# zsc/MOSS-TTSD

Measured on AMD Instinct MI355X. Metric: audio codec tokens/sec/node (decode, bf16, batch 32 @ 4k ctx), higher is better.
Workload: dtype bf16; 1 GPU; configs[2]: batch 32 synthetic dialogues/GPU, 4k-token KV context, top-k/top-p sampling on 8 channels, decode steps at full context; batch_per_gpu=32, context=4096, prompt=512, layers=28, hidden=2048, parallelism=dp1 (batch shard, no per-step collective)

## Files before the change

include/mtts.h:

```cpp
#ifndef MTTS_H
#define MTTS_H

#include <stdint.h>

#ifdef __cplusplus
extern "C" {
#endif

#define MTTS_OK 0
#define MTTS_EINVAL (-1)
#define MTTS_EHIP (-2)
#define MTTS_ENOMEM (-3)
#define MTTS_ESTATE (-4)

#define MTTS_CHANNELS 8

typedef struct MttsConfig {
    int32_t vocab_size;
    int32_t hidden_size;
    int32_t intermediate_size;
    int32_t num_hidden_layers;
    int32_t num_attention_heads;
    int32_t num_key_value_heads;
    int32_t head_dim;
// ... 13 lines not shown
#define MTTS_DTYPE_BF16 0
#define MTTS_DTYPE_F32 1
#define MTTS_DTYPE_F16 2

typedef struct MttsSamplerCfg {
    int32_t do_sample;
    int32_t top_k;
    float top_p;
    float one_minus_top_p;
    float temperature;
    float repetition_penalty;
} MttsSamplerCfg;

typedef struct MttsEngine MttsEngine;

const char* mtts_last_error(void);
int32_t mtts_version(void);

int32_t mtts_engine_create(const MttsConfig* cfg, int32_t device, MttsEngine** out);
int32_t mtts_engine_destroy(MttsEngine* e);

int32_t mtts_bind_weight(MttsEngine* e, const char* name, const void* dev_bf16,
                         int64_t rows, int64_t cols, void* stream);
int32_t mtts_bind_weight_lora(MttsEngine* e, const char* name, const void* dev_base, int64_t rows, int64_t cols,
                              const float* dev_lora_a, const float* dev_lora_b, int32_t r, float scaling, void* stream);
#define MTTS_MAX_ADAPTERS 16
#define MTTS_LORA_MAX_RANK 64
int32_t mtts_adapter_load(MttsEngine* e, int32_t adapter, const char* name, const float* dev_lora_a, const float* dev_lora_b,
                          int64_t rows, int64_t cols, int32_t r, float scaling, void* stream);
int32_t mtts_adapter_clear(MttsEngine* e, int32_t adapter);
int32_t mtts_set_row_adapters(MttsEngine* e, const int32_t* host_ids, int32_t n);
int32_t mtts_set_slot_adapter(MttsEngine* e, int32_t slot, int32_t adapter);
int32_t mtts_bind_rope(MttsEngine* e, const void* dev_cos_bf16, const void* dev_sin_bf16,
                       int32_t rows, void* stream);
int32_t mtts_weights_ready(MttsEngine* e);

int32_t mtts_generate(MttsEngine* e, const int64_t* host_input_ids, const uint8_t* host_attention_mask,
                      int32_t B, int32_t T, int32_t max_length,
                      const MttsSamplerCfg* sampler, uint64_t seed,
                      int64_t* host_out_ids, int32_t out_capacity, int32_t* out_len,
                      const int64_t* host_forced, int32_t forced_len, int64_t* host_decisions,
                      void* stream);

int32_t mtts_begin(MttsEngine* e, const int64_t* host_input_ids, const uint8_t* host_attention_mask,
                   int32_t B, int32_t T, int32_t max_length,
                   const MttsSamplerCfg* sampler, uint64_t seed, void* stream);
int32_t mtts_step(MttsEngine* e, int32_t n_steps, void* stream);
int32_t mtts_sync_state(MttsEngine* e, int32_t* steps_done, int32_t* all_finished, void* stream);
int32_t mtts_read_generated(MttsEngine* e, int64_t* host_gen, int32_t capacity_steps, int32_t* n_steps);
int32_t mtts_set_output_scores(MttsEngine* e, int32_t on);
int32_t mtts_read_scores(MttsEngine* e, float* host_lp, int32_t capacity_steps, int32_t* n_steps);
int32_t mtts_slot_read_scores(MttsEngine* e, int32_t slot, float* host_rows, int32_t capacity_steps, int32_t* n_steps);
int32_t mtts_score(MttsEngine* e, const int64_t* host_input_ids, const uint8_t* host_attention_mask,
                   const int64_t* host_labels, int32_t B, int32_t T, float* host_logp, void* stream);
#define MTTS_SCORE_MAX_TOPK 16
#define MTTS_SCORE_TOPK_ROWS 512
int32_t mtts_score_topk(MttsEngine* e, const int64_t* host_input_ids, const uint8_t* host_attention_mask,
                        const int64_t* host_labels, int32_t B, int32_t T, float* host_logp, int32_t k,
                        int32_t* host_top_ids, float* host_top_logp, void* stream);
int32_t mtts_read_logits(MttsEngine* e, uint16_t* host_logits0, uint16_t* host_logits17, void* stream);
int32_t mtts_read_logits_f32(MttsEngine* e, float* host_logits0, float* host_logits17, void* stream);
int32_t mtts_sched_open(MttsEngine* e, int32_t B, int32_t gen_cap, const MttsSamplerCfg* sampler, void* stream);
int32_t mtts_slot_submit(MttsEngine* e, int32_t slot, const int64_t* host_ids, int32_t T, int32_t max_length, uint64_t seed,
                         void* stream);
int32_t mtts_slot_submit_row(MttsEngine* e, int32_t slot, const int64_t* host_ids, int32_t T, int32_t max_length, uint64_t seed,
                             int32_t row_id, void* stream);
int32_t mtts_set_row_ids(MttsEngine* e, const int32_t* host_row_ids, int32_t n);
int32_t mtts_set_takes(MttsEngine* e, int32_t n);
int32_t mtts_slot_fork(MttsEngine* e, int32_t src_slot, int32_t dst_slot, uint64_t seed, int32_t row_id, void* stream);
int32_t mtts_slot_states(MttsEngine* e, int32_t* host_state, void* stream);
int32_t mtts_slot_read(MttsEngine* e, int32_t slot, int64_t* host_rows, int32_t capacity_steps, int32_t* n_steps);
int32_t mtts_read_seq_state(MttsEngine* e, int32_t* host_nas, int32_t* host_unfinished, int32_t* host_kv_len, void* stream);
int32_t mtts_slot_evict(MttsEngine* e, int32_t slot, void* stream);
int32_t mtts_kv_pool_state(MttsEngine* e, int32_t* total_pages, int32_t* free_pages, int32_t* max_pages_per_seq);
int32_t mtts_read_page_table(MttsEngine* e, int32_t* host_table, int32_t* host_n_pages);
int32_t mtts_set_forced_mode(MttsEngine* e, int32_t as_draw);
int32_t mtts_debug_read_device_page_table(MttsEngine* e, int32_t* host_table, void* stream);
int32_t mtts_export_codes(MttsEngine* e, int32_t first, int32_t n, int64_t* dev_codes, void* stream);
int32_t mtts_profile_enable(MttsEngine* e, int32_t on);
int32_t mtts_profile_read(MttsEngine* e, int32_t which, double* total_ms, int64_t* launches, int64_t* bytes);

int32_t mtts_debug_set_kv_len(MttsEngine* e, int32_t kv_len);
int32_t mtts_debug_kv_pack_stats(MttsEngine* e, int64_t* out6);
int32_t mtts_k_attn_bench(MttsEngine* e, int32_t phase, int32_t iters, float* avg_ms, int64_t* bytes_per_launch);
int32_t mtts_k_gemm_bench(int32_t N, int32_t K, int32_t epi, int32_t ksplit, int32_t waves, int32_t copies,
                          int32_t iters, float* avg_us);

int32_t mtts_k_gemm_bf16(const void* dev_w, const void* dev_x, void* dev_y,
                         int32_t M, int32_t N, int32_t K, int32_t ksplit, void* stream);
int64_t mtts_debug_gemm_depth_launches(void);
int64_t mtts_debug_attn_row_launches(void);
int32_t mtts_k_attn_section(const float* dev_slabs, int32_t ksplit, const void* dev_qnw, const void* dev_knw, const void* dev_cos,
                            const void* dev_sin, float eps, const void* dev_k, const void* dev_v, const int32_t* host_lens,
                            const int32_t* host_page_table, int32_t R, int32_t Lmax, int32_t nq, int32_t nkv, int32_t sealed,
                            int32_t path, void* dev_out, void* dev_kcache, void* dev_vcache, void* dev_kpack, void* dev_vpack,
                            void* stream);
int32_t mtts_k_attn_prefill(const float* dev_slabs, int32_t ksplit, const void* dev_qnw, const void* dev_knw, const void* dev_cos,
                            const void* dev_sin, float eps, const void* dev_k, const void* dev_v, const int32_t* host_lens,
                            const int32_t* host_cached, const int32_t* host_page_table, int32_t B, int32_t Lmax, int32_t nq,
                            int32_t nkv, void* dev_out, void* dev_q, void* dev_kcache, void* dev_vcache, void* stream);
int32_t mtts_k_gemm_swiglu_bf16(const void* dev_w, const void* dev_x, void* dev_y,
                                int32_t M, int32_t N, int32_t K, void* stream);
int32_t mtts_k_rmsnorm(const void* dev_x, const void* dev_w, void* dev_y,
                       int32_t rows, int32_t n, float eps, void* stream);
int32_t mtts_k_embed_norm(const int32_t* host_tokens, const int32_t* host_seq, const void* const* host_tables,
                          const int32_t* host_vocab, const void* dev_norm_w, int32_t R, int32_t H, float eps,
                          void* dev_x, void* dev_xn, void* stream);
int32_t mtts_k_resid_norm(const float* dev_slabs, int32_t ksplit, int32_t Npad, void* dev_x, const void* dev_norm_w,
                          const int32_t* host_seq, const int32_t* host_last, int32_t R, int32_t H, int32_t nseq, float eps,
                          void* dev_xn, void* dev_hlast, void* stream);
int32_t mtts_k_gemv_small(int32_t epi, int32_t pro, const void* dev_w, int32_t rows, int32_t N, int32_t K, int32_t want_ksplit,
                          const void* dev_x_in, const float* dev_slabs, int32_t slab_ksplit, const void* dev_norm_w, float eps,
                          void* dev_x_out, const float* dev_opart, const int32_t* host_seq, const int32_t* host_pos, int32_t nq,
                          int32_t nchunks_max, const void* dev_xrows, void* dev_y, int32_t* out_plan, void* stream);
int32_t mtts_k_gemm_tile(int32_t epi, const void* dev_w, const void* dev_x, void* dev_y, int32_t M, int32_t N, int32_t K,
                         int32_t ksplit, void* stream);
int32_t mtts_k_rope_kvwrite(const void* dev_qkv, const int32_t* host_pos, const void* dev_qnorm, const void* dev_knorm,
                            const void* dev_cos, const void* dev_sin, int32_t R, int32_t nq, int32_t nkv, float eps,
                            void* dev_q, void* dev_k, void* dev_v, void* stream);
int32_t mtts_k_paged_attn_decode(const void* dev_q, const void* dev_k, const void* dev_v, const int32_t* host_lens,
                                 const int32_t* host_page_table, int32_t R, int32_t Lmax, int32_t nq, int32_t nkv,
                                 void* dev_out, void* stream);
int32_t mtts_k_kv_seal(const void* dev_pages, int32_t npages, void* dev_sealed, int32_t as_k, void* stream);
int32_t mtts_k_head_ce(const void* dev_w, const void* dev_x, const int32_t* host_labels, int32_t M, int32_t N, int32_t K,
                       int32_t n_valid, int32_t segments, float* dev_logp, void* stream);
int32_t mtts_k_head_topk(const void* dev_w, const void* dev_x, int32_t M, int32_t N, int32_t K, int32_t n_valid,
                         int32_t segments, int32_t k, int32_t* dev_ids, float* dev_logp, void* stream);
int32_t mtts_k_lora_pack(const void* dev_base, int32_t rows, int32_t cols, const float* dev_lora_a, const float* dev_lora_b,
                         int32_t r, float scaling, int32_t rows_pad, int32_t row_mul, int32_t row_off, int32_t dtype,
                         void* dev_out, void* stream);
int32_t mtts_k_lora_delta(const void* dev_x, int32_t R, int32_t K, int32_t Npad, int32_t nseg, const int32_t* host_segs,
                          int32_t n_adapters, const void* const* host_a, const void* const* host_b, const int32_t* host_r,
                          const float* host_scaling, const int32_t* host_row_adapter, float* dev_slabs, int32_t ks, void* stream);
int32_t mtts_k_swiglu_slabs(const void* dev_w, const void* dev_x, const float* dev_delta, void* dev_y, float* dev_slab0_out,
                            int32_t M, int32_t N, int32_t K, void* stream);
int32_t mtts_k_sample(const void* dev_logits_bf16, int32_t rows, int32_t vocab,
                      const void* dev_history_bitmap, const MttsSamplerCfg* cfg,
                      int32_t mask_id, uint64_t seed, int32_t step, int32_t channel,
                      int32_t* dev_tokens, void* stream);
int32_t mtts_k_sample_scores(const void* dev_logits_bf16, int32_t rows, int32_t vocab,
                             const void* dev_history_bitmap, const MttsSamplerCfg* cfg,
                             int32_t mask_id, uint64_t seed, int32_t step, int32_t channel,
                             int32_t* dev_tokens, float* dev_logp, void* stream);

typedef struct MttsCodecConfig {
    int32_t nq, codebook_size, rvq_dim, quant_out_dim;
    int32_t adapter_layers, adapter_dim, adapter_heads, adapter_ffn, adapter_max_pos;
    int32_t up_stride;
    int32_t dec_layers, dec_dim, dec_heads, dec_ffn, dec_max_pos, mel_bins;
    int32_t voc_dim, voc_inter, voc_layers, n_fft, hop;
    int32_t mel_n_fft, mel_hop, mel_frames;
    int32_t enc_layers, enc_dim, enc_heads, enc_ffn, enc_max_pos;
    int32_t sem_adapter_layers, pre_rvq_layers, down_pool;
} MttsCodecConfig;

typedef struct MttsCodec MttsCodec;
const char* mtts_codec_last_error(void);
int32_t mtts_codec_create(const MttsCodecConfig* cfg, int32_t device, MttsCodec** out);
int32_t mtts_codec_destroy(MttsCodec* c);
int32_t mtts_codec_bind(MttsCodec* c, const char* role, const float* dev_f32, int64_t n, void* stream);
int32_t mtts_codec_detokenize(MttsCodec* c, const int64_t* dev_codes, const int32_t* host_lens, int32_t B, int32_t T,
                              float* dev_wav, void* stream);
int32_t mtts_codec_detokenize_async(MttsCodec* c, const int64_t* dev_codes, const int32_t* host_lens, int32_t B, int32_t T,
                                    float* dev_wav, void* stream);
int32_t mtts_codec_check(MttsCodec* c, void* stream);
int32_t mtts_codec_tokenize(MttsCodec* c, const float* dev_wav, const int32_t* host_lens, int32_t B, int32_t nsamp,
// ... 11 lines not shown
```

moss-ttsd_amd/csrc/attn.hip:

```cpp
#include "launch.h"
#include <algorithm>
#include <atomic>
#include <cstdlib>
#ifndef MTTS_PK_WAVES
#define MTTS_PK_WAVES 0
#endif
#if MTTS_PK_WAVES
#define PK_OCC(PK) __attribute__((amdgpu_waves_per_eu((PK) ? MTTS_PK_WAVES : 1, (PK) ? MTTS_PK_WAVES : 8)))
#else
#define PK_OCC(PK)
#endif

__device__ __forceinline__ uint32_t u4c(const u32x4_t& v, int c) { return c == 0 ? v.x : c == 1 ? v.y : c == 2 ? v.z : v.w; }
__device__ __forceinline__ void pk_unit(const u32x4_t* pk, int j, uint32_t w[4]) {
    const uint32_t L0 = u4c(pk[j >> 1], 2 * (j & 1)), L1 = u4c(pk[j >> 1], 2 * (j & 1) + 1);
    const uint32_t N = u4c(pk[8 + (j >> 2)], j & 3);
    const uint32_t lo = pk[12].x, hi = pk[12].y;
    const uint32_t HA = ((N & 0x08080808u) << 4) | __builtin_amdgcn_perm(hi, lo, N & 0x07070707u);
    const uint32_t HB = (N & 0x80808080u) | __builtin_amdgcn_perm(hi, lo, (N >> 4) & 0x07070707u);
    w[0] = __builtin_amdgcn_perm(HA, L0, 0x05010400u);
    w[1] = __builtin_amdgcn_perm(HA, L0, 0x07030602u);
    w[2] = __builtin_amdgcn_perm(HB, L1, 0x05010400u);
    w[3] = __builtin_amdgcn_perm(HB, L1, 0x07030602u);
}
// ... 109 lines not shown
                }
                out |= b << (16 * h);
            }
            w[c] = out;
        }
        v[j] = u32x4_t{w[0], w[1], w[2], w[3]};
    }
    return seal_encode(v, pk, ((uint32_t)s0 & 0xffu) | (((uint32_t)s1 & 0xffu) << 8), unfit);
}
__device__ bool seal_lane_v(const u32x4_t* __restrict__ raw, u32x4_t* __restrict__ pk, uint8_t* __restrict__ lds, int lane) {
    u32x4_t v[16];
#pragma unroll
    for (int j = 0; j < 16; ++j) v[j] = raw[j * 64];
    const int sub = lane >> 5;
    __builtin_amdgcn_wave_barrier();
    uint32_t* row = (uint32_t*)(lds + lane * 128);
#pragma unroll
    for (int it = 0; it < 16; ++it)
#pragma unroll
        for (int h = 0; h < 2; ++h) {
            uint32_t sum = 0u, cnt = 0u;
#pragma unroll
            for (int c = 0; c < 4; ++c) {
                const uint32_t e = (u4c(v[it], c) >> (7 + 16 * h)) & 0xffu;
                sum += e;
                cnt += e ? 1u : 0u;
            }
            row[2 * it + h] = sum | (cnt << 16);
        }
    __builtin_amdgcn_wave_barrier();
    int mean;
    {
        const int t = lane, st = (t >> 1) & 1, j = 2 * (t >> 2) + (t & 1);
        uint32_t tot = 0u, cn = 0u;
        for (int d = 0; d < 32; ++d) {
            const uint32_t w = ((const uint32_t*)(lds + (st * 32 + d) * 128))[j];
            tot += w & 0xffffu;
            cn += w >> 16;
        }
        mean = cn ? (int)((tot + cn / 2) / cn) : 0;
    }
    int* means = (int*)(lds + 8192);
    int8_t* sv = (int8_t*)(lds + 8192 + 256);
    means[lane] = mean;
    __builtin_amdgcn_wave_barrier();
    int ref = 255;
    for (int t = 0; t < 64; ++t) { const int m = means[t]; if (m > 0) ref = min(ref, m); }
    const int s_own = mean > 0 ? min((mean - ref) & ~1, 126) : 0;
    sv[lane] = (int8_t)s_own;
    __builtin_amdgcn_wave_barrier();
    bool unfit = false;
#pragma unroll
    for (int it = 0; it < 16; ++it) {
        const int s0 = sv[4 * it + 2 * sub], s1 = sv[4 * it + 2 * sub + 1];
        uint32_t w[4] = {v[it].x, v[it].y, v[it].z, v[it].w};
#pragma unroll
        for (int c = 0; c < 4; ++c) {
            uint32_t out = 0u;
#pragma unroll
            for (int h = 0; h < 2; ++h) {
                uint32_t b = (w[c] >> (16 * h)) & 0xffffu;
                const int sft = h ? s1 : s0;
                const int e = (int)((b >> 7) & 0xffu);
                if (e == 0) {
                    if ((b & 0x7fu) && sft) unfit = true;
                } else {
                    const int e2 = e - sft;
                    if (e == 255 ? sft != 0 : e2 < 1) unfit = true;
                    else b = (b - ((uint32_t)sft << 7)) & 0xffffu;
                }
                out |= b << (16 * h);
            }
            w[c] = out;
        }
        v[it] = u32x4_t{w[0], w[1], w[2], w[3]};
    }
    return seal_encode(v, pk, (uint32_t)s_own & 0xffu, unfit);
}
__device__ __forceinline__ void seal_count(bool fit, unsigned long long* __restrict__ cnt, int layer, int wave, int lane) {
    const bool all = !__any(!fit);
    if (cnt && lane == 0) atomicAdd(cnt + layer * 4 + wave * 2 + (all ? 0 : 1), 1ull);
}

__global__ __launch_bounds__(128) void kv_seal_scan_kernel(const u32x4_t* __restrict__ kcache, const u32x4_t* __restrict__ vcache,
                                                           u32x4_t* __restrict__ kpack, u32x4_t* __restrict__ vpack,
                                                           const int32_t* __restrict__ page_table, const RowMeta* __restrict__ meta, int R,
                                                           int max_pages, int total_pages, size_t raw_layer, size_t pk_layer,
                                                           unsigned long long* __restrict__ cnt) {
    __shared__ __attribute__((aligned(16))) uint8_t klds[8192 + 128];
    __shared__ __attribute__((aligned(16))) uint8_t vlds[8192 + 320];
    const int kvh = blockIdx.y, layer = blockIdx.z, wave = threadIdx.x >> 6, lane = threadIdx.x & 63;
    const int r = blockIdx.x * 64 + lane;
    RowMeta m{-1, 0, 0, 0};
    if (r < R) m = meta[r];
    unsigned long long todo = __ballot(m.seq >= 0 && (m.pos & 63) == 63);
    while (todo) {
        const int i = __ffsll((long long)todo) - 1;
        todo &= todo - 1;
        const int seq = __shfl(m.seq, i, 64), pos = __shfl(m.pos, i, 64);
        const int page = page_table[(size_t)seq * max_pages + (pos >> 6)];
        const size_t pi = (size_t)kvh * total_pages + page;
        const bool fit = wave ? seal_lane_v(vcache + layer * raw_layer + pi * (MTTS_PAGE * MTTS_HD / 8) + lane,
                                            vpack + layer * pk_layer + pi * (MTTS_PKU * 64) + lane, vlds, lane)
                              : seal_lane_k(kcache + layer * raw_layer + pi * (MTTS_PAGE * MTTS_HD / 8) + lane,
                                            kpack + layer * pk_layer + pi * (MTTS_PKU * 64) + lane, klds, lane);
        seal_count(fit, cnt, layer, wave, lane);
    }
}
__global__ __launch_bounds__(128) void kv_seal_all_kernel(const u32x4_t* __restrict__ kcache, const u32x4_t* __restrict__ vcache,
                                                          u32x4_t* __restrict__ kpack, u32x4_t* __restrict__ vpack, int total_pages,
                                                          size_t raw_layer, size_t pk_layer, unsigned long long* __restrict__ cnt) {
    __shared__ __attribute__((aligned(16))) uint8_t klds[8192 + 128];
    __shared__ __attribute__((aligned(16))) uint8_t vlds[8192 + 320];
    const int kvh = blockIdx.y, layer = blockIdx.z, wave = threadIdx.x >> 6, lane = threadIdx.x & 63;
    const size_t pi = (size_t)kvh * total_pages + blockIdx.x;
    const bool fit = wave ? seal_lane_v(vcache + layer * raw_layer + pi * (MTTS_PAGE * MTTS_HD / 8) + lane,
                                        vpack + layer * pk_layer + pi * (MTTS_PKU * 64) + lane, vlds, lane)
                          : seal_lane_k(kcache + layer * raw_layer + pi * (MTTS_PAGE * MTTS_HD / 8) + lane,
                                        kpack + layer * pk_layer + pi * (MTTS_PKU * 64) + lane, klds, lane);
    seal_count(fit, cnt, layer, wave, lane);
}
__global__ __launch_bounds__(64) void kv_seal_pages_kernel(const u32x4_t* __restrict__ raw, u32x4_t* __restrict__ pk, int as_k) {
    __shared__ __attribute__((aligned(16))) uint8_t klds[8192 + 320];
    const u32x4_t* src = raw + (size_t)blockIdx.x * (MTTS_PAGE * MTTS_HD / 8) + threadIdx.x;
    u32x4_t* dst = pk + (size_t)blockIdx.x * (MTTS_PKU * 64) + threadIdx.x;
    if (as_k == 1) seal_lane_k(src, dst, klds, threadIdx.x);
    else if (as_k == 2) seal_lane_v(src, dst, klds, threadIdx.x);
    else seal_lane(src, dst);
}
void launch_kv_seal_pages(const void* raw, void* pk, int npages, int as_k, hipStream_t st) {
    hipLaunchKernelGGL(kv_seal_pages_kernel, dim3(npages), dim3(64), 0, st, (const u32x4_t*)raw, (u32x4_t*)pk, as_k);
}
__global__ __launch_bounds__(64) void kv_pack_count_kernel(const u32x4_t* __restrict__ kpack, const u32x4_t* __restrict__ vpack,
                                                           const int32_t* __restrict__ page_table, const int32_t* __restrict__ complete,
                                                           int max_pages, int total_pages, size_t pk_layer, unsigned long long* __restrict__ out) {
    const int b = blockIdx.x, kvh = blockIdx.y, layer = blockIdx.z, lane = threadIdx.x;
    unsigned long long n = 0, dk = 0, dv = 0;
    for (int pg = 0; pg < complete[b]; ++pg) {
        const size_t pi = (size_t)kvh * total_pages + page_table[(size_t)b * max_pages + pg];
        const u32x4_t fk = kpack[layer * pk_layer + pi * (MTTS_PKU * 64) + 12 * 64 + lane];
        const u32x4_t fv = vpack[layer * pk_layer + pi * (MTTS_PKU * 64) + 12 * 64 + lane];
        n += 1;
        dk += __any(fk.w != 0u) ? 1 : 0;
        dv += __any(fv.w != 0u) ? 1 : 0;
    }
    if (lane == 0 && n) {
        atomicAdd(out + 0, n); atomicAdd(out + 1, dk); atomicAdd(out + 2, n); atomicAdd(out + 3, dv);
    }
}
void launch_kv_pack_count(const void* kpack, const void* vpack, const int32_t* page_table, const int32_t* complete, int B, int max_pages,
                          int total_pages, int nkv, int L, unsigned long long* out, hipStream_t st) {
    const size_t pk_layer = (size_t)total_pages * nkv * (MTTS_PKU * 64);
    hipLaunchKernelGGL(kv_pack_count_kernel, dim3(B, nkv, L), dim3(64), 0, st, (const u32x4_t*)kpack, (const u32x4_t*)vpack, page_table,
                       complete, max_pages, total_pages, pk_layer, out);
}
void launch_kv_seal_rows(const void* kcache, const void* vcache, void* kpack, void* vpack, const int32_t* page_table,
                         const RowMeta* meta, int R, int max_pages, int total_pages, int nkv, int L, unsigned long long* cnt, hipStream_t st) {
    const size_t raw_layer = (size_t)total_pages * nkv * (MTTS_PAGE * MTTS_HD / 8), pk_layer = (size_t)total_pages * nkv * (MTTS_PKU * 64);
    hipLaunchKernelGGL(kv_seal_scan_kernel, dim3((R + 63) / 64, nkv, L), dim3(128), 0, st, (const u32x4_t*)kcache, (const u32x4_t*)vcache,
                       (u32x4_t*)kpack, (u32x4_t*)vpack, page_table, meta, R, max_pages, total_pages, raw_layer, pk_layer, cnt);
}
void launch_kv_seal_all(const void* kcache, const void* vcache, void* kpack, void* vpack, int total_pages, int nkv, int L,
                        unsigned long long* cnt, hipStream_t st) {
    const size_t raw_layer = (size_t)total_pages * nkv * (MTTS_PAGE * MTTS_HD / 8), pk_layer = (size_t)total_pages * nkv * (MTTS_PKU * 64);
    hipLaunchKernelGGL(kv_seal_all_kernel, dim3(total_pages, nkv, L), dim3(128), 0, st, (const u32x4_t*)kcache, (const u32x4_t*)vcache,
                       (u32x4_t*)kpack, (u32x4_t*)vpack, total_pages, raw_layer, pk_layer, cnt);
}


__device__ __forceinline__ void fuse_reduce(const QkvFuse& f, int r, int col, int lane, float& a, float& b) {
    const size_t kstride = (size_t)MTTS_PFCAP * f.Npad;
    const float* p0 = f.partial + (size_t)r * f.Npad + col + lane;
    a = 0.f; b = 0.f;
    for (int k0 = 0; k0 < f.ksplit; k0 += 8) {
        float ta[8], tb[8];
#pragma unroll
        for (int j = 0; j < 8; ++j) {
            const float* pk = p0 + (size_t)min(k0 + j, f.ksplit - 1) * kstride;
            ta[j] = pk[0];
            tb[j] = pk[64];
        }
        if (k0 == 0) { a = ta[0]; b = tb[0]; }
#pragma unroll
        for (int j = 0; j < 8; ++j)
            if (k0 + j < f.ksplit && k0 + j > 0) { a += ta[j]; b += tb[j]; }
    }
    a = rbf(a);
    b = rbf(b);
}

__device__ __forceinline__ void fuse_reduce_request(const QkvFuse& f, int r, int col, int lane, float (&ta)[8], float (&tb)[8]) {
    const size_t kstride = (size_t)MTTS_PFCAP * f.Npad;
    const float* p0 = f.partial + (size_t)r * f.Npad + col + lane;
#pragma unroll
    for (int j = 0; j < 8; ++j) {
        const float* pk = p0 + (size_t)min(j, f.ksplit - 1) * kstride;
        ta[j] = pk[0];
        tb[j] = pk[64];
    }
}
__device__ __forceinline__ void fuse_reduce_sum(const QkvFuse& f, const float (&ta)[8], const float (&tb)[8], float& a, float& b) {
    a = ta[0]; b = tb[0];
#pragma unroll
    for (int j = 1; j < 8; ++j)
        if (j < f.ksplit) { a += ta[j]; b += tb[j]; }
    a = rbf(a);
    b = rbf(b);
}

struct FuseVec { float w0, w1, c, s; };
__device__ __forceinline__ FuseVec fuse_load_vec(const QkvFuse& f, const uint16_t* __restrict__ nw, int pos, int lane) {
    FuseVec v;
    v.w0 = bf2f(nw[lane]);
    v.w1 = bf2f(nw[lane + 64]);
    v.c = bf2f(f.rope_cos[(size_t)pos * 64 + lane]);
    v.s = bf2f(f.rope_sin[(size_t)pos * 64 + lane]);
    return v;
}
__device__ __forceinline__ void fuse_norm_rope(const QkvFuse& f, const FuseVec& v, float a, float b, float& o1, float& o2) {
    const float ss = wave_sum(a * a + b * b);
    const float inv = 1.0f / sqrtf(ss / (float)MTTS_HD + f.eps);
    a = rbf(v.w0 * rbf(a * inv));
    b = rbf(v.w1 * rbf(b * inv));
    o1 = rbf(rbf(a * v.c) + rbf(-b * v.s));
    o2 = rbf(rbf(b * v.c) + rbf(a * v.s));
}

template <int G, bool FUSED, bool PK>
__global__ __launch_bounds__(256) PK_OCC(PK) void attn_scores_kernel(
    const uint16_t* __restrict__ qbuf, u32x4_t* __restrict__ kcache, const int32_t* __restrict__ page_table,
    const RowMeta* __restrict__ meta, uint16_t* __restrict__ scores, float* __restrict__ stats, int max_pages,
    int total_pages, int nq, int nkv, float scale, QkvFuse f, const u32x4_t* __restrict__ kpack) {
    __shared__ __attribute__((aligned(16))) uint32_t qs[G][MTTS_HD / 2];
    __shared__ __attribute__((aligned(16))) uint16_t knew[MTTS_HD];
    __shared__ __attribute__((aligned(16))) uint32_t qw[PK ? 4 : 1][G][MTTS_HD / 2];
    const int r = blockIdx.z, kvh = blockIdx.y;
    const RowMeta m = meta[r];
    if (m.seq < 0) return;
    const int len = m.pos + 1;
    const int npages = (len + MTTS_PAGE - 1) / MTTS_PAGE;
    if ((int)blockIdx.x * 4 >= npages) return;
    const int wave = __builtin_amdgcn_readfirstlane(threadIdx.x >> 6), lane = threadIdx.x & 63;
    const int pg = blockIdx.x * 4 + wave;
// ... 1009 lines not shown
```

moss-ttsd_amd/csrc/engine.h:

```cpp
#pragma once
#include <hip/hip_runtime.h>

#include <algorithm>
#include <cstdarg>
#include <cstdio>
#include <cstdlib>
#include <cstring>
#include <memory>
#include <string>
#include <vector>

#include "launch.h"

#define MTTS_LOCAL __attribute__((visibility("hidden")))
extern MTTS_LOCAL thread_local char g_err[512];
MTTS_LOCAL int fail(int code, const char* fmt, ...) __attribute__((format(printf, 2, 3)));
#define HIPCHK(x)                                                                          \
    do {                                                                                   \
        hipError_t _e = (x);                                                               \
        if (_e != hipSuccess) return fail(MTTS_EHIP, "%s: %s (%s:%d)", #x, hipGetErrorString(_e), __FILE__, __LINE__); \
    } while (0)
#define TRY(x)             \
    do {                   \
        int _r = (x);      \
// ... 108 lines not shown
    uint16_t *rope_cos = nullptr, *rope_sin = nullptr;
    int rope_rows = 0;
    int emb_bound = 0, norm_bound = 0;
    const uint16_t** d_tables = nullptr;
    GemmPlan p_qkv, p_o, p_gu, p_d, p_h0, p_h17;
    float* partial = nullptr;
    float* partial2 = nullptr;
    void *x2 = nullptr, *act_rm = nullptr;
    int small_rows = SMALL_RP;
    int gemm_depth = 1;
    void *x = nullptr, *xn = nullptr, *attn_p = nullptr, *act_p = nullptr, *qbuf = nullptr, *hlast = nullptr, *xh = nullptr;
    void *logits0 = nullptr, *logits17 = nullptr, *join_logits0 = nullptr, *join_logits17 = nullptr;
    void* scores = nullptr;
    float *stats = nullptr, *opart = nullptr;
    void *kcache = nullptr, *vcache = nullptr;
    size_t layer_stride = 0;
    int total_pages = 0, max_pages = 0, nchunks_max = 0;
    int32_t* d_page_table = nullptr;
    std::vector<int32_t> h_page_table;
    std::vector<int32_t> free_pages;
    std::vector<int32_t> n_pages;
    std::vector<int32_t> page_owners;
    std::vector<char> slot_live;
    PageEdits pending_edits;
    int forced_draw = 0;
    std::vector<int32_t> next_row_ids;
    int next_takes = 1;
    int takes = 1;
    bool f32 = false;
    int h16 = 0;
    struct LayerF32 { float *wqkv = nullptr, *wo = nullptr, *wgu = nullptr, *wd = nullptr, *ln_in = nullptr, *ln_post = nullptr, *qn = nullptr, *kn = nullptr; };
    std::vector<LayerF32> lf;
    float* embf[8] = {nullptr};
    const float** d_tables_f = nullptr;
    float *final_norm_f = nullptr, *rope_cos_f = nullptr, *rope_sin_f = nullptr;
    float *kcache_f = nullptr, *vcache_f = nullptr;
    float *xf = nullptr, *xnf = nullptr, *qkvf = nullptr, *qbuf_f = nullptr, *attnf = nullptr, *yf = nullptr, *guf = nullptr,
          *actf = nullptr, *hlast_f = nullptr, *scores_f = nullptr;
    SeqState* d_seqs = nullptr;
    RowMeta* d_meta = nullptr;
    LoopState* d_ls = nullptr;
    LoopState* h_ls = nullptr;
    SeqState* h_seqs = nullptr;
    int32_t *d_decisions = nullptr, *d_cur = nullptr, *d_gen = nullptr, *d_declog = nullptr, *d_forced = nullptr,
            *d_tf = nullptr;
    uint32_t* d_bitmaps = nullptr;
    int bm_words = 0;
    MttsSamplerCfg* d_scfg = nullptr;
    SampleScratch sscr;
    int ch0_sampled = 0;
    float* d_lp = nullptr;
    int lp_cap = 0;
    int scores_next = 0;
    int scores_on = 0;
    bool run_open = false;
    int32_t* d_sc_labels = nullptr;
    float* d_sc_logp = nullptr;
    size_t sc_cap_rows = 0;
    float* sc_part = nullptr;
    float* sc_logits = nullptr;
    int32_t* d_sc_top_ids = nullptr;
    float* d_sc_top_logp = nullptr;
    size_t sc_top_cap = 0;
    uint32_t* sc_cand = nullptr;
    std::vector<LoraEnt> bank;
    LoraEnt* d_bank = nullptr;
    int bank_pairs[MTTS_MAX_ADAPTERS] = {0};
    int32_t* d_seq_adapter = nullptr;
    std::vector<int32_t> seq_adapter = std::vector<int32_t>(MTTS_RCAP, -1);
    std::vector<int32_t> next_slot_adapter = std::vector<int32_t>(MTTS_RCAP, -1);
    std::vector<int32_t> next_row_adapters;
    bool row_adapters_pending = false;
    int32_t* d_pf_tokens = nullptr;
    RowMeta* d_pf_meta = nullptr;
    size_t pf_cap_rows = 0;
    int gen_cap = 0;
    int B = 0, T = 0, base_length = 0, max_length = 0, max_steps = 0, steps_issued = 0;
    bool continuous = false;
    std::vector<int> join_step;
    std::vector<int> n_real;
    int max_real = 0;
    uint64_t seed = 0;
    bool began = false, has_forced = false;
    struct StepGraph { int B, pages, forced, ch0, scores, row, lora; hipGraphExec_t exec; };
    std::vector<StepGraph> graphs;
    hipStream_t cap_stream = nullptr;
    bool use_graphs = true;
    int kv_pack = 1;
    void *kpack = nullptr, *vpack = nullptr;
    size_t pk_layer_stride = 0;
    unsigned long long *d_seal_cnt = nullptr, *h_seal_cnt = nullptr;
    std::vector<char> pack_k_on, pack_v_on;
    int pack_min_work = 512;
    int fuse_qkv_max = 2560;
    int attn_row = 1;
    int n_cus = 0;
    int pf_mfma_pages = 0;
    bool prof = false;
    std::vector<std::pair<hipEvent_t, hipEvent_t>> ev[PROF_N];
    int64_t prof_bytes[PROF_N] = {0, 0, 0, 0, 0};
};

static inline bool attn_row_auto(int rows, int nkv, int pages_bound, int n_cus) {
    (void)pages_bound;
    return n_cus > 0 && rows * nkv >= n_cus;
}
static inline bool attn_row_shape(const MttsEngine* e, int pages_bound) {
    if (e->attn_row == 0 || e->f32) return false;
    return e->attn_row == 2 || attn_row_auto(e->B, e->nkv, pages_bound, e->n_cus);
}

static inline KvPack layer_pack(MttsEngine* e, int n, int pages_bound) {
    KvPack pk{nullptr, nullptr};
    if (e->B * pages_bound < e->pack_min_work) return pk;
    if (e->kpack && e->pack_k_on[n]) pk.k = (uint8_t*)e->kpack + e->pk_layer_stride * n;
    if (e->vpack && e->pack_v_on[n]) pk.v = (uint8_t*)e->vpack + e->pk_layer_stride * n;
    return pk;
}
```

moss-ttsd_amd/csrc/engine.hip:

```cpp
#include "engine.h"

#define FLUSH_STEPS 7
#define LINGER_STEPS 14
static inline int linger_bound(int B) { return 6 * B + 8; }

thread_local char g_err[512] = "";
int fail(int code, const char* fmt, ...) {
    va_list ap;
    va_start(ap, fmt);
    vsnprintf(g_err, sizeof(g_err), fmt, ap);
    va_end(ap);
    return code;
}

const char* mtts_last_error(void) { return g_err; }
int32_t mtts_version(void) { return 202; }

static void pool_reset(MttsEngine* e) {
    e->free_pages.resize(e->total_pages);
    for (int i = 0; i < e->total_pages; ++i) e->free_pages[i] = e->total_pages - 1 - i;
    if (const char* g = getenv("MTTS_PAGE_SHUFFLE")) {
        uint64_t x = 0x9E3779B97F4A7C15ull ^ (uint64_t)atoll(g);
        for (int i = e->total_pages - 1; i > 0; --i) {
            x = x * 6364136223846793005ull + 1442695040888963407ull;
// ... 73 lines not shown
    HIPCHK(hipMemcpy((void*)e->d_tables_f, e->embf, 8 * sizeof(void*), hipMemcpyHostToDevice));
    const size_t P = MTTS_PF32CAP;
    TRY(e->mem.get(&e->xf, P * H)); TRY(e->mem.get(&e->xnf, P * H)); TRY(e->mem.get(&e->yf, P * H));
    TRY(e->mem.get(&e->qkvf, P * e->qkv_rows)); TRY(e->mem.get(&e->qbuf_f, P * e->nq * D)); TRY(e->mem.get(&e->attnf, P * e->nq * D));
    TRY(e->mem.get(&e->guf, P * 2 * I)); TRY(e->mem.get(&e->actf, P * I));
    TRY(e->mem.get(&e->hlast_f, (size_t)MTTS_RCAP * H));
    TRY(e->mem.get((float**)&e->logits0, (size_t)MTTS_RCAP * e->V0_pad));
    TRY(e->mem.get((float**)&e->logits17, (size_t)MTTS_RCAP * 7 * e->Vs_pad));
    return 0;
}

static int forward_rows_f32(MttsEngine* e, const int32_t* d_tokens, const RowMeta* d_meta, int R, int heads, hipStream_t st) {
    const int H = e->H, I = e->I, nq = e->nq, nkv = e->nkv;
    const float eps = e->cfg.rms_norm_eps, scale = 1.0f / sqrtf((float)MTTS_HD);
    const int Lmax = e->max_pages * MTTS_PAGE, h16 = e->h16;
    const bool dec = heads == 1;
    launch_f32_embed_norm(d_tokens, d_meta, e->d_tables_f, e->lf[0].ln_in, e->xf, e->xnf, R, H, eps, h16, st);
    for (int n = 0; n < e->L; ++n) {
        auto& l = e->lf[n];
        float* kc = e->kcache_f + e->layer_stride * n;
        float* vc = e->vcache_f + e->layer_stride * n;
        launch_f32_linear(l.wqkv, e->xnf, e->qkvf, R, e->qkv_rows, H, e->qkv_rows, h16, dec, st);
        launch_f32_qkv_post(e->qkvf, e->qkv_rows, d_meta, l.qn, l.kn, e->rope_cos_f, e->rope_sin_f, e->qbuf_f, kc, vc,
                            e->d_page_table, e->max_pages, e->total_pages, R, nq, nkv, eps, h16, st);
        launch_f32_attn(e->qbuf_f, kc, vc, e->d_page_table, d_meta, e->scores_f, e->attnf, R, e->max_pages, e->total_pages, nq,
                        nkv, scale, Lmax, h16, st);
        launch_f32_linear(l.wo, e->attnf, e->yf, R, H, nq * MTTS_HD, H, h16, dec, st);
        launch_f32_resid_norm(e->yf, e->xf, l.ln_post, e->xnf, nullptr, d_meta, R, H, eps, h16, st);
        launch_f32_linear(l.wgu, e->xnf, e->guf, R, 2 * I, H, 2 * I, h16, dec, st);
        launch_f32_swiglu(e->guf, e->actf, R, I, h16, st);
        launch_f32_linear(l.wd, e->actf, e->yf, R, H, I, H, h16, dec, st);
        const bool lastl = n == e->L - 1;
        launch_f32_resid_norm(e->yf, e->xf, lastl ? e->final_norm_f : e->lf[n + 1].ln_in, e->xnf, lastl ? e->hlast_f : nullptr,
                              d_meta, R, H, eps, h16, st);
    }
    if (heads) {
        const float* xin = heads == 1 ? e->xnf : e->hlast_f;
        launch_f32_linear(e->embf[0], xin, (float*)e->logits0, e->B, e->V0, H, e->V0_pad, h16, true, st);
        for (int c = 1; c < 8; ++c)
            launch_f32_linear(e->embf[c], xin, (float*)e->logits17 + (size_t)(c - 1) * e->Vs_pad, e->B, e->Vs, H, 7 * e->Vs_pad, h16, true, st);
    }
    HIPCHK(hipGetLastError());
    return MTTS_OK;
}

static void drop_graphs(MttsEngine* e) {
    for (auto& g : e->graphs) hipGraphExecDestroy(g.exec);
    e->graphs.clear();
}

int32_t mtts_engine_create(const MttsConfig* c, int32_t device, MttsEngine** out) {
    if (!c || !out) return fail(MTTS_EINVAL, "null argument");
    if (c->head_dim != MTTS_HD) return fail(MTTS_EINVAL, "head_dim must be 128 (got %d)", c->head_dim);
    if (c->channels != 8) return fail(MTTS_EINVAL, "channels must be 8");
    if (c->hidden_size % 16 || c->intermediate_size % 16) return fail(MTTS_EINVAL, "hidden/intermediate must be multiples of 16");
    if (c->hidden_size > 8192) return fail(MTTS_EINVAL, "hidden_size > 8192 not built (resid_norm keeps a row in registers)");
    if (c->num_attention_heads % c->num_key_value_heads) return fail(MTTS_EINVAL, "bad GQA ratio");
    int G = c->num_attention_heads / c->num_key_value_heads;
    if (G != 1 && G != 2 && G != 4) return fail(MTTS_EINVAL, "GQA group %d not built (1,2,4)", G);
    if (c->max_batch < 1 || c->max_batch > MTTS_RCAP) return fail(MTTS_EINVAL, "max_batch must be 1..128");
    if (c->vocab_size <= 152694 || c->speech_vocab_size <= 1024)
        return fail(MTTS_EINVAL, "vocab too small for the reference's hard-coded mask ids 152694 / 1024");
    if (c->dtype != MTTS_DTYPE_BF16 && c->dtype != MTTS_DTYPE_F32 && c->dtype != MTTS_DTYPE_F16)
        return fail(MTTS_EINVAL, "dtype %d not built (bf16 = 0, fp32 = 1, fp16 = 2)", c->dtype);
    if (c->kv_pool_pages < 0) return fail(MTTS_EINVAL, "kv_pool_pages must be >= 0");
    HIPCHK(hipSetDevice(device));
    struct Destroy {
        void operator()(MttsEngine* p) const {
            const std::string keep = g_err;
            mtts_engine_destroy(p);
            snprintf(g_err, sizeof(g_err), "%s", keep.c_str());
        }
    };
    std::unique_ptr<MttsEngine, Destroy> holder(new MttsEngine());
    MttsEngine* e = holder.get();
    DevBufs& m = e->mem;
    e->cfg = *c;
    e->device = device;
    if (const char* g = getenv("MTTS_GRAPHS")) e->use_graphs = atoi(g) != 0;
    if (const char* g = getenv("MTTS_FUSE_QKV_MAX")) e->fuse_qkv_max = atoi(g);
    if (const char* g = getenv("MTTS_KV_PACK")) e->kv_pack = atoi(g);
    if (const char* g = getenv("MTTS_KV_PACK_MIN")) e->pack_min_work = atoi(g);
    if (const char* g = getenv("MTTS_PREFILL_MFMA_PAGES")) e->pf_mfma_pages = atoi(g);
    if (const char* g = getenv("MTTS_ATTN_ROW")) e->attn_row = std::min(std::max(atoi(g), 0), 2);
    HIPCHK(hipDeviceGetAttribute(&e->n_cus, hipDeviceAttributeMultiprocessorCount, device));
    if (e->attn_row && attn_row_prepare()) {
        if (e->attn_row == 2) return fail(MTTS_EINVAL, "attn_row_kernel: the dynamic LDS limit could not be raised");
        e->attn_row = 0;
    }
    if (const char* g = getenv("MTTS_SMALL_ROWS")) e->small_rows = std::min(std::max(atoi(g), 0), SMALL_RP);
    e->gemm_depth = gemm_depth_env();
    e->H = c->hidden_size; e->I = c->intermediate_size; e->L = c->num_hidden_layers;
    e->nq = c->num_attention_heads; e->nkv = c->num_key_value_heads;
    e->V0 = c->vocab_size; e->Vs = c->speech_vocab_size;
    e->V0_pad = round_up(e->V0, 32); e->Vs_pad = round_up(e->Vs, 32);
    e->qkv_rows = (e->nq + 2 * e->nkv) * MTTS_HD;
    e->layers.resize(e->L);
    const int H = e->H, I = e->I;
    e->f32 = c->dtype != MTTS_DTYPE_BF16;
    e->h16 = c->dtype == MTTS_DTYPE_F16;
    if (e->f32) TRY(create_f32(e));
    if (!e->f32) {
        for (auto& l : e->layers) {
            TRY(m.get((uint16_t**)&l.wqkv, (size_t)e->qkv_rows * H));
            TRY(m.get((uint16_t**)&l.wo, (size_t)H * e->nq * MTTS_HD));
            TRY(m.get((uint16_t**)&l.wgu, (size_t)2 * I * H));
            TRY(m.get((uint16_t**)&l.wd, (size_t)round_up(H, 32) * I));
            TRY(m.get((uint16_t**)&l.ln_in, (size_t)H));
            TRY(m.get((uint16_t**)&l.ln_post, (size_t)H));
            TRY(m.get((uint16_t**)&l.qn, (size_t)MTTS_HD));
            TRY(m.get((uint16_t**)&l.kn, (size_t)MTTS_HD));
        }
        TRY(m.get((uint16_t**)&e->emb[0], (size_t)e->V0 * H, false));
        for (int ch = 1; ch < 8; ++ch) TRY(m.get((uint16_t**)&e->emb[ch], (size_t)e->Vs * H, false));
        TRY(m.get((uint16_t**)&e->head0, (size_t)e->V0_pad * H));
        TRY(m.get((uint16_t**)&e->heads17, (size_t)7 * e->Vs_pad * H));
        TRY(m.get((uint16_t**)&e->final_norm, (size_t)H));
        TRY(m.get(&e->d_tables, 8));
        HIPCHK(hipMemcpy((void*)e->d_tables, e->emb, 8 * sizeof(void*), hipMemcpyHostToDevice));
    }
    e->p_qkv = mtts_plan_gemm(e->qkv_rows, H, 0);
    e->p_o = mtts_plan_gemm(round_up(H, 32), e->nq * MTTS_HD, 0);
    e->p_gu = mtts_plan_gemm(2 * I, H, 1);
    e->p_d = mtts_plan_gemm(round_up(H, 32), I, 0);
    e->p_h0 = mtts_plan_gemm(e->V0_pad, H, 1);
    e->p_h17 = mtts_plan_gemm(7 * e->Vs_pad, H, 1);
    for (GemmPlan* p : {&e->p_qkv, &e->p_o, &e->p_gu, &e->p_d, &e->p_h0, &e->p_h17}) p->depth = e->gemm_depth;
    size_t pmax = (size_t)8 * std::max(e->qkv_rows, round_up(H, 32));
    if (!e->f32) {
        TRY(m.get(&e->partial, pmax * MTTS_PFCAP));
        TRY(m.get(&e->partial2, (size_t)8 * round_up(H, 32) * MTTS_PFCAP));
        TRY(m.get((uint16_t**)&e->x2, (size_t)MTTS_MAXR * H));
        TRY(m.get((uint16_t**)&e->act_rm, (size_t)MTTS_MAXR * I));
        TRY(m.get((uint16_t**)&e->x, (size_t)MTTS_PFCAP * H));
        TRY(m.get((uint16_t**)&e->xn, (size_t)MTTS_PFCAP * H));
        TRY(m.get((uint16_t**)&e->xh, (size_t)MTTS_RCAP * H));
        TRY(m.get((uint16_t**)&e->hlast, (size_t)MTTS_RCAP * H));
        TRY(m.get((uint16_t**)&e->attn_p, (size_t)MTTS_PFCAP * e->nq * MTTS_HD));
        TRY(m.get((uint16_t**)&e->act_p, (size_t)MTTS_PFCAP * I));
        TRY(m.get((uint16_t**)&e->qbuf, (size_t)MTTS_PFCAP * e->nq * MTTS_HD));
        TRY(m.get((uint16_t**)&e->logits0, (size_t)MTTS_RCAP * e->V0_pad));
        TRY(m.get((uint16_t**)&e->logits17, (size_t)MTTS_RCAP * 7 * e->Vs_pad));
        TRY(m.get((uint16_t**)&e->join_logits0, (size_t)MTTS_MAXR * e->V0_pad));
        TRY(m.get((uint16_t**)&e->join_logits17, (size_t)MTTS_MAXR * 7 * e->Vs_pad));
    }
    e->max_pages = (c->max_seq_len + MTTS_PAGE - 1) / MTTS_PAGE + 1;
    e->total_pages = c->kv_pool_pages > 0 ? c->kv_pool_pages : e->max_pages * c->max_batch;
    e->nchunks_max = (e->max_pages + ATT_PB - 1) / ATT_PB;
    e->layer_stride = (size_t)e->total_pages * e->nkv * MTTS_PAGE * MTTS_HD;
    if (e->f32) {
        TRY(m.get(&e->kcache_f, e->layer_stride * e->L));
        TRY(m.get(&e->vcache_f, e->layer_stride * e->L));
        TRY(m.get(&e->scores_f, (size_t)MTTS_PF32CAP * e->nq * e->max_pages * MTTS_PAGE, false));
    } else {
        TRY(m.get((uint16_t**)&e->kcache, e->layer_stride * e->L));
        TRY(m.get((uint16_t**)&e->vcache, e->layer_stride * e->L));
        if (e->kv_pack) {
            e->pk_layer_stride = (size_t)e->total_pages * e->nkv * MTTS_PKU * 64 * 16;
            size_t free_b = 0, total_b = 0;
            const size_t need = 2 * e->pk_layer_stride * e->L;
            if (hipMemGetInfo(&free_b, &total_b) != hipSuccess || need + ((size_t)8 << 30) > free_b) {
                fprintf(stderr, "mtts: sealed KV pages off: %.1f GB needed, %.1f GB free (8 GB kept for the run)\n", need / 1e9, free_b / 1e9);
                e->kv_pack = 0;
            }
        }
        if (e->kv_pack) {
// ... 324 lines not shown
}
static void prof_end(MttsEngine* e, hipStream_t st, hipEvent_t a) {
    if (!e->prof) return;
    hipEventRecord(a, st);
}

static int pack_policy_reset(MttsEngine* e, hipStream_t st) {
    if (!e->d_seal_cnt) return 0;
    HIPCHK(hipMemsetAsync(e->d_seal_cnt, 0, (size_t)e->L * 4 * sizeof(unsigned long long), st));
    bool changed = false;
    for (int n = 0; n < e->L; ++n) { changed |= !e->pack_k_on[n] || !e->pack_v_on[n]; e->pack_k_on[n] = 1; e->pack_v_on[n] = 1; }
    if (changed) drop_graphs(e);
    return 0;
}
static int attend_layer(MttsEngine* e, int n, const RowMeta* d_meta, int R, int pages_bound, int ks_qkv, int nphases, bool prefill,
                        bool fused, bool sealed, hipStream_t st, int64_t kv_tokens_hint) {
    static const AttnPhase decode_ph[3] = {ATTN_SCORES, ATTN_PV, ATTN_COMBINE}, prefill_ph[3] = {ATTN_PF_SCORES, ATTN_PF_PV, ATTN_PF_COMBINE};
    Layer& l = e->layers[n];
    const float eps = e->cfg.rms_norm_eps, scale = 1.0f / sqrtf((float)MTTS_HD);
    uint16_t* kc = (uint16_t*)e->kcache + e->layer_stride * n;
    uint16_t* vc = (uint16_t*)e->vcache + e->layer_stride * n;
    const QkvFuse fz{e->partial, ks_qkv, e->qkv_rows, (const uint16_t*)l.qn, (const uint16_t*)l.kn, e->rope_cos, e->rope_sin, eps};
    const KvPack pk = layer_pack(e, n, pages_bound);
    const KvPack* pkp = (sealed && (pk.k || pk.v)) ? &pk : nullptr;
    if (!prefill && sealed && nphases == 3 && attn_row_shape(e, pages_bound) && attn_row_fits(e->nq / e->nkv, &fz, pkp, pages_bound)) {
        hipEvent_t ev = nullptr;
        prof_begin(e, PROF_SCORES, st, &ev);
        if (const int rc = launch_attn(e->qbuf, kc, vc, e->d_page_table, d_meta, e->scores, e->stats, e->opart, e->attn_p, R, pages_bound,
                                       e->max_pages, e->total_pages, e->nchunks_max, e->nq, e->nkv, scale, &fz, ATTN_ROW, st, pkp))
            return fail(MTTS_EINVAL, rc == -2 ? "the whole-row attention kernel does not take this launch" : "attention group size not built");
        prof_end(e, st, ev);
        if (e->prof) e->prof_bytes[PROF_SCORES] += 2 * kv_tokens_hint * e->nkv * MTTS_HD * 2;
        return 0;
    }
    if (!fused)
        launch_qkv_post(e->partial, ks_qkv, e->qkv_rows, d_meta, l.qn, l.kn, e->rope_cos, e->rope_sin, e->qbuf,
                        kc, vc, e->d_page_table, e->max_pages, e->total_pages, R, e->nq, e->nkv, eps, st);
    for (int i = 0; i < nphases; ++i) {
        hipEvent_t ev = nullptr;
        if (i < 2) prof_begin(e, i == 0 ? PROF_SCORES : PROF_PV, st, &ev);
        if (launch_attn(e->qbuf, kc, vc, e->d_page_table, d_meta, e->scores, e->stats, e->opart, e->attn_p, R,
                        pages_bound, e->max_pages, e->total_pages, e->nchunks_max, e->nq, e->nkv, scale,
                        fused ? &fz : nullptr, (prefill ? prefill_ph : decode_ph)[i], st, pkp))
            return fail(MTTS_EINVAL, "attention group size not built");
        if (i < 2) prof_end(e, st, ev);
    }
    if (e->prof) {
        e->prof_bytes[PROF_SCORES] += kv_tokens_hint * e->nkv * MTTS_HD * 2;
        e->prof_bytes[PROF_PV] += kv_tokens_hint * e->nkv * MTTS_HD * 2;
    }
    return 0;
}
static bool small_path_fits(MttsEngine* e) {
    const int H = e->H;
    if (H > 8192 || H % 8 || e->I % 8) return false;
    const int lim = 64 * 1024 - 33 * 1024;
    return mtts_small_lds_bytes(e->p_qkv, H, PRO_NORM) <= lim && mtts_small_lds_bytes(e->p_d, e->I, PRO_ROWS) <= lim &&
           mtts_small_lds_bytes(e->p_o, e->nq * MTTS_HD, PRO_COMBINE) <= lim;
}
static int forward_small(MttsEngine* e, const RowMeta* d_meta, int pages_bound, hipStream_t st, int64_t kv_tokens_hint) {
    const int H = e->H, I = e->I, nq = e->nq, nkv = e->nkv, Hp = round_up(H, 32), R = MTTS_MAXR;
    const float eps = e->cfg.rms_norm_eps;
    uint16_t* xa = (uint16_t*)e->x;
    uint16_t* xb = (uint16_t*)e->x2;
    SmallPro base{};
    base.rows = e->B; base.eps = eps; base.slab_npad = Hp;
    for (int n = 0; n < e->L; ++n) {
        Layer& l = e->layers[n];
        SmallPro pq = base;
        pq.x_in = xa; pq.x_out = xb; pq.slabs = e->partial2; pq.ksplit = n ? e->p_d.ksplit : 0; pq.norm_w = (const uint16_t*)l.ln_in;
        launch_gemv_small(EPI_PARTIAL, PRO_NORM, e->p_qkv, l.wqkv, H, e->qkv_rows, e->qkv_rows, e->partial, nullptr, pq, st);
        TRY(attend_layer(e, n, d_meta, R, pages_bound, e->p_qkv.ksplit, 2, false, e->B * pages_bound <= e->fuse_qkv_max, true, st,
                         kv_tokens_hint));
        SmallPro po = base;
        po.opart = e->opart; po.meta = d_meta; po.nchunks_max = e->nchunks_max; po.nq = nq; po.pages_per_chunk = ATT_PB;
        launch_gemv_small(EPI_PARTIAL, PRO_COMBINE, e->p_o, l.wo, nq * MTTS_HD, Hp, Hp, e->partial2, nullptr, po, st);
        SmallPro pg = base;
        pg.x_in = xb; pg.x_out = xa; pg.slabs = e->partial2; pg.ksplit = e->p_o.ksplit; pg.norm_w = (const uint16_t*)l.ln_post;
        launch_gemv_small(EPI_SILU_RM, PRO_NORM, e->p_gu, l.wgu, H, 2 * I, 2 * I, nullptr, (uint16_t*)e->act_rm, pg, st);
        SmallPro pd = base;
        pd.xrows = (const uint16_t*)e->act_rm;
        launch_gemv_small(EPI_PARTIAL, PRO_ROWS, e->p_d, l.wd, I, Hp, Hp, e->partial2, nullptr, pd, st);
    }
    if (e->kpack)
        launch_kv_seal_rows(e->kcache, e->vcache, e->kpack, e->vpack, e->d_page_table, d_meta, R, e->max_pages, e->total_pages, nkv, e->L, e->d_seal_cnt, st);
    SmallPro ph = base;
    ph.x_in = xa; ph.x_out = nullptr; ph.slabs = e->partial2; ph.ksplit = e->p_d.ksplit; ph.norm_w = (const uint16_t*)e->final_norm;
    launch_gemv_small(EPI_BF16, PRO_NORM, e->p_h0, e->head0, H, e->V0_pad, e->V0, nullptr, (uint16_t*)e->logits0, ph, st);
    launch_gemv_small(EPI_BF16, PRO_NORM, e->p_h17, e->heads17, H, 7 * e->Vs_pad, 7 * e->Vs_pad, nullptr, (uint16_t*)e->logits17, ph, st);
    HIPCHK(hipGetLastError());
    return MTTS_OK;
}

static int forward_rows(MttsEngine* e, const int32_t* d_tokens, const RowMeta* d_meta, int R, int pages_bound,
                        int heads, bool lora, hipStream_t st, int64_t kv_tokens_hint) {
    const int H = e->H, I = e->I, nq = e->nq, nkv = e->nkv;
    const float eps = e->cfg.rms_norm_eps;
    const int Hp = round_up(H, 32);
    const int mb = (R + 31) / 32;
    const bool tiled = heads != 1;
    if (e->f32) return forward_rows_f32(e, d_tokens, d_meta, heads == 1 ? e->B : R, heads, st);
    launch_embed_norm(d_tokens, d_meta, e->d_tables, e->layers[0].ln_in, e->x, e->xn, R, H, eps, st);
    if (heads == 1 && !lora && e->B <= e->small_rows && small_path_fits(e)) return forward_small(e, d_meta, pages_bound, st, kv_tokens_hint);
    if (lora && !e->d_bank) return fail(MTTS_ESTATE, "a pass with adapters on an engine without a bank");
    const int QD = nq * MTTS_HD, KD = nkv * MTTS_HD, EL = e->L * 7;
    const LoraJob j_qkv{3, e->qkv_rows, H, EL, {{0, QD, 1, 0}, {QD, KD, 1, 1}, {QD + KD, KD, 1, 2}}};
    const LoraJob j_o{1, Hp, QD, EL, {{0, H, 1, 3}}}, j_gu{2, 2 * I, H, EL, {{0, I, 2, 4}, {1, I, 2, 5}}}, j_d{1, Hp, I, EL, {{0, H, 1, 6}}};
    for (int n = 0; n < e->L; ++n) {
        Layer& l = e->layers[n];
        auto delta = [&](const LoraJob& job, const void* xp, int ks) {
            launch_lora_delta(xp, d_meta, e->d_seq_adapter, e->d_bank + (size_t)n * 7, job, e->partial + (size_t)ks * MTTS_PFCAP * job.Npad, R, st);
        };
        const int ex = lora ? 1 : 0;
        const int ks_qkv = tiled ? mtts_tile_ksplit(e->qkv_rows, H, 1024) : e->p_qkv.ksplit;
        const int ks_o = tiled ? mtts_tile_ksplit(Hp, nq * MTTS_HD, 1024) : e->p_o.ksplit;
        const int ks_d = tiled ? mtts_tile_ksplit(Hp, I, 1024) : e->p_d.ksplit;
        if (tiled) launch_gemm_tile(EPI_PARTIAL, R, ks_qkv, l.wqkv, e->xn, H, e->qkv_rows, e->qkv_rows, e->partial, nullptr, st);
        else launch_gemm(EPI_PARTIAL, mb, e->p_qkv, l.wqkv, e->xn, H, e->qkv_rows, e->qkv_rows, e->partial, nullptr, st);
        if (lora) delta(j_qkv, e->xn, ks_qkv);
        TRY(attend_layer(e, n, d_meta, R, pages_bound, ks_qkv + ex, 3, heads != 1 && pages_bound >= e->pf_mfma_pages,
                         heads == 1 && e->B * pages_bound <= e->fuse_qkv_max, heads == 1, st, kv_tokens_hint));
        if (tiled) launch_gemm_tile(EPI_PARTIAL, R, ks_o, l.wo, e->attn_p, nq * MTTS_HD, Hp, Hp, e->partial, nullptr, st);
        else launch_gemm(EPI_PARTIAL, mb, e->p_o, l.wo, e->attn_p, nq * MTTS_HD, Hp, Hp, e->partial, nullptr, st);
        if (lora) delta(j_o, e->attn_p, ks_o);
        launch_resid_norm(e->partial, ks_o + ex, Hp, e->x, l.ln_post, e->xn, nullptr, d_meta, R, H, eps, st);
        const int gu_epi = lora ? EPI_PARTIAL : EPI_SILU;
        float* gu_slab = lora ? e->partial : nullptr;
        if (tiled) launch_gemm_tile(gu_epi, R, 1, l.wgu, e->xn, H, 2 * I, 2 * I, gu_slab, (uint16_t*)e->act_p, st);
        else launch_gemm(gu_epi, mb, e->p_gu, l.wgu, e->xn, H, 2 * I, 2 * I, gu_slab, (uint16_t*)e->act_p, st);
        if (lora) {
            delta(j_gu, e->xn, 1);
            launch_swiglu_slabs(e->partial, e->partial + (size_t)MTTS_PFCAP * 2 * I, e->act_p, mb * 32, I, st);
        }
        if (tiled) launch_gemm_tile(EPI_PARTIAL, R, ks_d, l.wd, e->act_p, I, Hp, Hp, e->partial, nullptr, st);
        else launch_gemm(EPI_PARTIAL, mb, e->p_d, l.wd, e->act_p, I, Hp, Hp, e->partial, nullptr, st);
        if (lora) delta(j_d, e->act_p, ks_d);
        const bool lastl = (n == e->L - 1);
        const void* nw = lastl ? e->final_norm : e->layers[n + 1].ln_in;
        launch_resid_norm(e->partial, ks_d + ex, Hp, e->x, nw, e->xn, lastl ? e->hlast : nullptr, d_meta, R, H, eps, st);
    }
    if (e->kpack)
        launch_kv_seal_rows(e->kcache, e->vcache, e->kpack, e->vpack, e->d_page_table, d_meta, R, e->max_pages, e->total_pages, nkv, e->L, e->d_seal_cnt, st);
    if (heads) {
        const void* xin = e->xn;
        int hmb = mb;
        if (heads == 2) {
            hmb = (e->B + 31) / 32;
            launch_pack_rows(e->hlast, e->xh, e->B, H, hmb, st);
            xin = e->xh;
        }
        launch_gemm(EPI_BF16, hmb, e->p_h0, e->head0, xin, H, e->V0_pad, e->V0, nullptr, (uint16_t*)e->logits0, st);
        launch_gemm(EPI_BF16, hmb, e->p_h17, e->heads17, xin, H, 7 * e->Vs_pad, 7 * e->Vs_pad, nullptr, (uint16_t*)e->logits17, st);
    }
    HIPCHK(hipGetLastError());
    return MTTS_OK;
}

static int prefill_staged(MttsEngine* e, size_t Mpad, int pages_bound, int last_heads, bool lora, hipStream_t st) {
    const size_t pfcap = e->f32 ? MTTS_PF32CAP : MTTS_PFCAP;
    for (size_t off = 0; off < Mpad; off += pfcap) {
        const int rows = (int)std::min<size_t>(pfcap, Mpad - off);
        TRY(forward_rows(e, e->d_pf_tokens + off * 8, e->d_pf_meta + off, rows, pages_bound, off + rows >= Mpad ? last_heads : 0, lora, st, 0));
    }
    return 0;
}

static int ensure_gen_storage(MttsEngine* e, int steps) {
    if (steps <= e->gen_cap) return 0;
    e->mem.release(e->d_gen); e->mem.release(e->d_declog); e->mem.release(e->d_forced);
    drop_graphs(e);
    e->gen_cap = steps;
    const size_t n = (size_t)e->cfg.max_batch * steps * 8;
    TRY(e->mem.get(&e->d_gen, n));
    TRY(e->mem.get(&e->d_declog, n));
    TRY(e->mem.get(&e->d_forced, n, false));
    return 0;
}

static int start_scores(MttsEngine* e, hipStream_t st) {
    e->scores_on = e->scores_next;
    if (!e->scores_on) return 0;
    if (!e->sscr.lp) {
        drop_graphs(e);
        TRY(alloc_lp_scratch(e->mem, e->sscr, e->cfg.max_batch));
    }
    const size_t n = (size_t)e->cfg.max_batch * e->gen_cap * 8;
    if (!e->d_lp || e->lp_cap != e->gen_cap) {
        e->mem.release(e->d_lp);
        drop_graphs(e);
        TRY(e->mem.get(&e->d_lp, n, false));
        e->lp_cap = e->gen_cap;
    }
    HIPCHK(hipMemsetAsync(e->d_lp, 0xff, n * sizeof(float), st));
    return 0;
}

static int grow_prefill_staging(MttsEngine* e, size_t rows) {
    if (rows <= e->pf_cap_rows) return 0;
    e->mem.release(e->d_pf_tokens); e->mem.release(e->d_pf_meta);
    e->pf_cap_rows = 0;
    TRY(e->mem.get(&e->d_pf_tokens, rows * 8, false));
    TRY(e->mem.get(&e->d_pf_meta, rows, false));
    e->pf_cap_rows = rows;
    return 0;
}

static const SeqState IDLE_SEQ{-1, 0, 0, 0, 0, 0, 0, 0, 0};
static int reset_run_state(MttsEngine* e, const std::vector<SeqState>& seqs, bool continuous, const MttsSamplerCfg* sampler, hipStream_t st) {
    HIPCHK(hipMemcpyAsync(e->d_seqs, seqs.data(), seqs.size() * sizeof(SeqState), hipMemcpyHostToDevice, st));
    if (continuous) e->forced_draw = 0;
    LoopState ls{0, 0, continuous ? 1 : 0, e->B, 0, e->gen_cap, e->forced_draw, e->f32 ? 1 : 0};
    e->continuous = continuous;
    e->join_step.assign(MTTS_RCAP, 0);
    HIPCHK(hipMemcpyAsync(e->d_ls, &ls, sizeof(ls), hipMemcpyHostToDevice, st));
    *e->h_ls = ls;
    std::vector<RowMeta> dm(MTTS_RCAP, RowMeta{-1, 0, 0, 0});
    HIPCHK(hipMemcpyAsync(e->d_meta, dm.data(), dm.size() * sizeof(RowMeta), hipMemcpyHostToDevice, st));
    HIPCHK(hipMemcpyAsync(e->d_scfg, sampler, 8 * sizeof(MttsSamplerCfg), hipMemcpyHostToDevice, st));
    e->ch0_sampled = sampler[0].do_sample ? 1 : 0;
    HIPCHK(hipMemsetAsync(e->sscr.hist, 0, (size_t)e->cfg.max_batch * 2048 * 4, st));
    HIPCHK(hipMemsetAsync(e->sscr.cand_n, 0, (size_t)e->cfg.max_batch * 4, st));
    HIPCHK(hipMemsetAsync(e->sscr.overflow, 0, (size_t)e->cfg.max_batch * 4, st));
    HIPCHK(hipStreamSynchronize(st));
    return 0;
}

static int launch_fork_job(MttsEngine* e, ForkJob& job, bool state_rows, hipStream_t st) {
    const int ew = e->f32 ? 4 : 2;
    job.narr = 0;
    auto arr = [&](void* base, size_t stride, size_t bytes) {
        job.base[job.narr] = (uint8_t*)base; job.stride[job.narr] = (int64_t)stride; job.bytes[job.narr++] = (int64_t)bytes;
    };
    arr(e->logits0, (size_t)e->V0_pad * ew, (size_t)e->V0_pad * ew);
    arr(e->logits17, (size_t)7 * e->Vs_pad * ew, (size_t)7 * e->Vs_pad * ew);
    if (state_rows) {
// ... 82 lines not shown
    for (int b = 0; b < B; ++b) Mtot += (size_t)round_up(e->n_real[b * takes], MTTS_MAXR);
    size_t Mpad = (Mtot + MTTS_RCAP - 1) / MTTS_RCAP * MTTS_RCAP;
    std::vector<int32_t> toks(Mpad * 8, 0);
    std::vector<RowMeta> metas(Mpad, RowMeta{-1, 0, 0, 0});
    size_t r = 0;
    for (int b = 0; b < B; r = (r + MTTS_MAXR - 1) / MTTS_MAXR * MTTS_MAXR, ++b)
        for (int i = 0; i < e->n_real[b * takes]; ++i, ++r) {
            const int64_t* src = ids + ((size_t)b * T + pad[b] + i) * 8;
            for (int c = 0; c < 8; ++c) {
                int64_t t = src[c];
                int64_t V = c == 0 ? e->V0 : e->Vs;
                if (t < 0 || t >= V) return fail(MTTS_EINVAL, "token %lld out of range on channel %d", (long long)t, c);
                toks[r * 8 + c] = (int32_t)t;
            }
            metas[r] = RowMeta{b * takes, i, i == e->n_real[b * takes] - 1 ? 1 : 0, 0};
        }
    TRY(grow_prefill_staging(e, Mpad));
    HIPCHK(hipMemcpyAsync(e->d_pf_tokens, toks.data(), Mpad * 8 * 4, hipMemcpyHostToDevice, st));
    HIPCHK(hipMemcpyAsync(e->d_pf_meta, metas.data(), Mpad * sizeof(RowMeta), hipMemcpyHostToDevice, st));
    {
        std::vector<uint32_t> bm((size_t)MTTS_RCAP * 8 * e->bm_words, 0u);
        for (int rw = 0; rw < R; ++rw)
            for (int t = 0, b = rw / takes; t < base; ++t)
                for (int c = 0; c < 8; ++c) {
                    int64_t tk = ids[((size_t)b * T + t) * 8 + c];
                    if (tk >= 0 && tk < (int64_t)e->bm_words * 32) bm[((size_t)rw * 8 + c) * e->bm_words + (tk >> 5)] |= 1u << (tk & 31);
                }
        HIPCHK(hipMemcpyAsync(e->d_bitmaps, bm.data(), bm.size() * 4, hipMemcpyHostToDevice, st));
        std::vector<int32_t> tf((size_t)MTTS_RCAP * 7 * 8, 0);
        for (int rw = 0; rw < R; ++rw)
            for (int s = 0, b = rw / takes; s < 7; ++s)
                for (int c = 0; c < 8; ++c) {
                    int64_t tk = ids[((size_t)b * T + base + s) * 8 + c];
                    if (tk < 0 || tk >= (c == 0 ? e->V0 : e->Vs)) return fail(MTTS_EINVAL, "token %lld out of range on channel %d (delayed tail)", (long long)tk, c);
                    tf[((size_t)rw * 7 + s) * 8 + c] = (int32_t)tk;
                }
        HIPCHK(hipMemcpyAsync(e->d_tf, tf.data(), tf.size() * 4, hipMemcpyHostToDevice, st));
        std::vector<SeqState> ss(MTTS_RCAP, IDLE_SEQ);
        if (!e->next_row_ids.empty() && (int)e->next_row_ids.size() != R)
            return fail(MTTS_EINVAL, "mtts_set_row_ids gave %d ids, the batch has %d rows", (int)e->next_row_ids.size(), R);
        for (int b = 0; b < R; ++b)
            ss[b] = SeqState{-1, 1, e->n_real[b], 0, base, max_length, e->next_row_ids.empty() ? b : e->next_row_ids[b], 1, seed};
        e->next_row_ids.clear();
        for (int b = 0; b < MTTS_RCAP; ++b) e->seq_adapter[b] = (b < R && !row_adapters.empty()) ? row_adapters[b / takes] : -1;
        if (e->d_seq_adapter) HIPCHK(hipMemcpyAsync(e->d_seq_adapter, e->seq_adapter.data(), MTTS_RCAP * sizeof(int32_t), hipMemcpyHostToDevice, st));
        TRY(reset_run_state(e, ss, false, sampler, st));
    }
    TRY(prefill_staged(e, Mpad, (e->max_real + MTTS_PAGE - 1) / MTTS_PAGE, 2, lora, st));
    if (fork.nr) TRY(launch_fork_job(e, fork, false, st));
    e->began = true;
    e->run_open = true;
    return MTTS_OK;
}

int32_t mtts_set_takes(MttsEngine* e, int32_t n) {
    if (!e) return fail(MTTS_EINVAL, "null engine");
    if (n < 1 || n > MTTS_RCAP) return fail(MTTS_EINVAL, "takes must be 1..%d (got %d)", MTTS_RCAP, n);
    e->next_takes = n;
    return MTTS_OK;
}

int32_t mtts_begin(MttsEngine* e, const int64_t* ids, const uint8_t* mask, int32_t B, int32_t T, int32_t max_length,
                   const MttsSamplerCfg* sampler, uint64_t seed, void* stream) {
    if (!e) return fail(MTTS_EINVAL, "null argument");
    const int takes = e->next_takes;
    e->next_takes = 1;
    const std::vector<int32_t> row_adapters = take_row_adapters(e);
    return begin_run(e, ids, mask, B, T, max_length, sampler, seed, takes, row_adapters, stream);
}

static int step_body(MttsEngine* e, int pages_bound, hipStream_t st, int64_t kvtok) {
    launch_sample(e->logits0, e->logits17, e->V0, e->Vs, e->Vs_pad, e->d_bitmaps, e->bm_words, e->d_scfg, e->d_ls,
                  e->d_seqs, e->seed, e->d_decisions, &e->d_ls->error, e->B, e->sscr, e->ch0_sampled,
                  full_cap_for(e->V0), e->scores_on, st);
    launch_update(e->d_decisions, e->d_declog, e->has_forced ? e->d_forced : nullptr, e->d_tf, e->d_gen, e->d_cur,
                  e->d_seqs, e->d_meta, e->d_bitmaps, e->bm_words, e->d_ls, e->cfg.eos_token_id,
                  e->cfg.speech_pad_token, e->cfg.speech_range_lo, e->cfg.speech_range_hi,
                  e->scores_on ? e->sscr.lp : nullptr, e->scores_on ? e->d_lp : nullptr, st);
    return forward_rows(e, e->d_cur, e->d_meta, round_up(e->B, 32), pages_bound, 1, rows_carry_adapters(e), st, kvtok);
}

static int step_graph(MttsEngine* e, int pages, hipGraphExec_t* out) {
    const int forced = e->has_forced ? 1 : 0, row = attn_row_shape(e, pages) ? 1 : 0, lora = rows_carry_adapters(e) ? 1 : 0;
    for (auto& g : e->graphs)
        if (g.B == e->B && g.pages == pages && g.forced == forced && g.ch0 == e->ch0_sampled && g.scores == e->scores_on && g.row == row &&
            g.lora == lora) {
            *out = g.exec;
            return MTTS_OK;
        }
    if (e->graphs.size() >= 256) drop_graphs(e);
    if (!e->cap_stream) HIPCHK(hipStreamCreateWithFlags(&e->cap_stream, hipStreamNonBlocking));
    hipGraph_t g = nullptr;
    HIPCHK(hipStreamBeginCapture(e->cap_stream, hipStreamCaptureModeRelaxed));
    int rc = step_body(e, pages, e->cap_stream, 0);
    hipError_t ce = hipStreamEndCapture(e->cap_stream, &g);
    if (rc) { if (g) hipGraphDestroy(g); return rc; }
    HIPCHK(ce);
    hipGraphExec_t exec = nullptr;
    hipError_t ie = hipGraphInstantiate(&exec, g, nullptr, nullptr, 0);
    hipGraphDestroy(g);
    HIPCHK(ie);
    e->graphs.push_back({e->B, pages, forced, e->ch0_sampled, e->scores_on, row, lora, exec});
    *out = exec;
    return MTTS_OK;
}

static int issue_steps(MttsEngine* e, int n, hipStream_t st) {
    for (int i = 0; i < n; ++i) {
        if (e->steps_issued >= e->max_steps) break;
        int len_bound = 1;
        for (int b = 0; b < e->B; ++b) {
            if (!e->slot_live[b]) continue;
            const int len = e->n_real[b] + e->steps_issued + 1;
            len_bound = std::max(len_bound, len);
            TRY(pool_grow(e, b, (len + MTTS_PAGE - 1) / MTTS_PAGE, st));
        }
        TRY(pool_flush(e, st));
        const int pages_bound = (len_bound + MTTS_PAGE - 1) / MTTS_PAGE;
        if (e->use_graphs && !e->prof) {
            hipGraphExec_t exec = nullptr;
            TRY(step_graph(e, std::min(round_up(pages_bound, ATT_PB), e->max_pages), &exec));
            HIPCHK(hipGraphLaunch(exec, st));
        } else {
            hipEvent_t ev = nullptr;
            prof_begin(e, PROF_STEP, st, &ev);
            int64_t kvtok = 0;
            for (int b = 0; b < e->B; ++b) if (e->slot_live[b]) kvtok += e->n_real[b] + e->steps_issued + 1;
            TRY(step_body(e, pages_bound, st, kvtok));
            prof_end(e, st, ev);
        }
        e->steps_issued++;
    }
    return MTTS_OK;
}

int32_t mtts_step(MttsEngine* e, int32_t n_steps, void* stream) {
    if (!e || !e->began) return fail(MTTS_ESTATE, "mtts_begin has not run");
    HIPCHK(hipSetDevice(e->device));
    return issue_steps(e, n_steps, S(stream));
}

int32_t mtts_sync_state(MttsEngine* e, int32_t* steps_done, int32_t* all_finished, void* stream) {
    if (!e || !e->began) return fail(MTTS_ESTATE, "mtts_begin has not run");
    HIPCHK(hipSetDevice(e->device));
    HIPCHK(hipMemcpyAsync(e->h_ls, e->d_ls, sizeof(LoopState), hipMemcpyDeviceToHost, S(stream)));
    if (!e->continuous) HIPCHK(hipMemcpyAsync(e->h_seqs, e->d_seqs, e->B * sizeof(SeqState), hipMemcpyDeviceToHost, S(stream)));
    if (e->d_seal_cnt) HIPCHK(hipMemcpyAsync(e->h_seal_cnt, e->d_seal_cnt, (size_t)e->L * 4 * sizeof(unsigned long long), hipMemcpyDeviceToHost, S(stream)));
    HIPCHK(hipStreamSynchronize(S(stream)));
    if (e->d_seal_cnt && e->kv_pack == 1) {
        bool changed = false;
        for (int n = 0; n < e->L; ++n) {
            const unsigned long long* c = e->h_seal_cnt + (size_t)n * 4;
            const bool k_on = c[0] + c[1] < 16 || c[1] * 8 <= c[0] + c[1], v_on = c[2] + c[3] < 16 || c[3] * 8 <= c[2] + c[3];
            changed |= (k_on != (bool)e->pack_k_on[n]) || (v_on != (bool)e->pack_v_on[n]);
            e->pack_k_on[n] = k_on; e->pack_v_on[n] = v_on;
        }
        if (changed) drop_graphs(e);
    }
    if (e->h_ls->error) return fail(MTTS_EINVAL, "device sampler error %d: more than 4096 candidate tokens (set top_k so that the k-th score's radix bin holds <= 4096 tokens)", e->h_ls->error);
    if (!e->continuous) {
        const SeqState* ss = e->h_seqs;
        for (int b = 0; b < e->B; ++b)
            if (e->slot_live[b] && ss[b].step > 0 && !ss[b].unfinished && ss[b].active != 2) { e->slot_live[b] = 0; pool_release(e, b); }
    }
    if (steps_done) *steps_done = e->h_ls->step;
    if (all_finished) *all_finished = e->h_ls->done;
    if (e->h_ls->done && !e->continuous) e->run_open = false;
    return MTTS_OK;
}

template <typename Src, typename Dst>
static int read_slots(MttsEngine* e, const Src* d_src, int slot0, int nslots, int steps, Dst* host) {
    std::vector<Src> tmp((size_t)std::max(steps, 1) * 8);
    for (int b = 0; b < nslots; ++b) {
        if (steps) HIPCHK(hipMemcpy(tmp.data(), d_src + (size_t)(slot0 + b) * e->gen_cap * 8, (size_t)steps * 8 * sizeof(Src), hipMemcpyDeviceToHost));
        for (int s = 0; s < steps; ++s)
            for (int c = 0; c < 8; ++c) host[((size_t)s * nslots + b) * 8 + c] = tmp[(size_t)s * 8 + c];
    }
    return MTTS_OK;
}
template <typename Src, typename Dst>
static int read_rows(MttsEngine* e, const Src* d_src, Dst* host, int capacity_steps, int* n_steps) {
    const int steps = e->h_ls->step;
    if (steps > capacity_steps) return fail(MTTS_EINVAL, "output buffer holds %d steps, need %d", capacity_steps, steps);
    TRY(read_slots(e, d_src, 0, e->B, steps, host));
    if (n_steps) *n_steps = steps;
    return MTTS_OK;
}
template <typename Src, typename Dst>
static int slot_read(MttsEngine* e, const Src* d_src, int slot, Dst* host_rows, int capacity_steps, int* n_steps) {
    HIPCHK(hipSetDevice(e->device));
    HIPCHK(hipDeviceSynchronize());
    SeqState cur;
    HIPCHK(hipMemcpy(&cur, e->d_seqs + slot, sizeof(cur), hipMemcpyDeviceToHost));
    if (cur.step > capacity_steps) return fail(MTTS_EINVAL, "buffer holds %d steps, need %d", capacity_steps, cur.step);
    TRY(read_slots(e, d_src, slot, 1, cur.step, host_rows));
    if (n_steps) *n_steps = cur.step;
    return MTTS_OK;
}
template <typename T>
// ... 355 lines not shown
    e->B = B; e->steps_issued = 0; e->has_forced = false; e->continuous = true;
    e->max_steps = 1 << 30;
    e->n_real.assign(B, 0);
    e->max_real = 0;
    HIPCHK(hipStreamSynchronize(st));
    for (int b = 0; b < e->cfg.max_batch; ++b) { pool_release(e, b); e->slot_live[b] = 0; }
    e->pending_edits.n = 0;
    TRY(pack_policy_reset(e, st));
    std::fill(e->seq_adapter.begin(), e->seq_adapter.end(), -1);
    if (e->d_seq_adapter) HIPCHK(hipMemsetAsync(e->d_seq_adapter, 0xff, MTTS_RCAP * sizeof(int32_t), st));
    TRY(reset_run_state(e, std::vector<SeqState>(MTTS_RCAP, IDLE_SEQ), true, sampler, st));
    e->began = true;
    e->run_open = true;
    return MTTS_OK;
}

int32_t mtts_slot_submit(MttsEngine* e, int32_t slot, const int64_t* ids, int32_t T, int32_t max_length, uint64_t seed,
                         void* stream) {
    return mtts_slot_submit_row(e, slot, ids, T, max_length, seed, 0, stream);
}

int32_t mtts_set_row_ids(MttsEngine* e, const int32_t* host_row_ids, int32_t n) {
    if (!e || (n > 0 && !host_row_ids) || n < 0 || n > MTTS_RCAP) return fail(MTTS_EINVAL, "set_row_ids: bad argument");
    e->next_row_ids.assign(host_row_ids, host_row_ids + n);
    return MTTS_OK;
}

int32_t mtts_slot_submit_row(MttsEngine* e, int32_t slot, const int64_t* ids, int32_t T, int32_t max_length, uint64_t seed,
                             int32_t row_id, void* stream) {
    if (!e || !e->began || !e->continuous || !ids) return fail(MTTS_ESTATE, "mtts_sched_open has not run");
    HIPCHK(hipSetDevice(e->device));
    hipStream_t st = S(stream);
    if (slot < 0 || slot >= e->B) return fail(MTTS_EINVAL, "slot %d out of range", slot);
    const int adapter = e->next_slot_adapter[slot];
    e->next_slot_adapter[slot] = -1;
    TRY(adapter_id_check(e, adapter, "slot", slot));
    if (T < 8) return fail(MTTS_EINVAL, "T must be >= 8");
    const int base = T - 7, n = base;
    if (max_length <= base) return fail(MTTS_EINVAL, "max_length leaves no room to generate");
    const int max_new = max_length - base + FLUSH_STEPS;
    if (max_new > e->gen_cap) return fail(MTTS_EINVAL, "dialogue may run %d steps, slot storage holds %d", max_new, e->gen_cap);
    if ((n + max_new + MTTS_PAGE - 1) / MTTS_PAGE > e->max_pages) return fail(MTTS_ENOMEM, "dialogue needs more KV pages than a sequence may hold");
    if (n + max_new > e->rope_rows) return fail(MTTS_EINVAL, "rope table too short");
    HIPCHK(hipStreamSynchronize(st));
    {
        SeqState cur;
        HIPCHK(hipMemcpy(&cur, e->d_seqs + slot, sizeof(cur), hipMemcpyDeviceToHost));
        if (cur.active) return fail(MTTS_ESTATE, "slot %d is occupied", slot);
    }
    if (e->slot_live[slot]) { e->slot_live[slot] = 0; pool_release(e, slot); }
    if ((int)e->free_pages.size() < (n + 1 + MTTS_PAGE - 1) / MTTS_PAGE)
        return fail(MTTS_ENOMEM, "KV page pool: %d pages free, the prompt needs %d", (int)e->free_pages.size(), (n + 1 + MTTS_PAGE - 1) / MTTS_PAGE);
    TRY(pool_grow(e, slot, (n + MTTS_PAGE - 1) / MTTS_PAGE, st));
    TRY(pool_flush(e, st));
    const size_t Mpad = ((size_t)n + MTTS_RCAP - 1) / MTTS_RCAP * MTTS_RCAP;
    std::vector<int32_t> toks(Mpad * 8, 0);
    std::vector<RowMeta> metas(Mpad, RowMeta{-1, 0, 0, 0});
    std::vector<uint32_t> bm((size_t)8 * e->bm_words, 0u);
    std::vector<int32_t> tf(7 * 8, 0);
    for (int i = 0; i < T; ++i)
        for (int c = 0; c < 8; ++c) {
            int64_t t = ids[(size_t)i * 8 + c];
            if (t < 0 || t >= (c == 0 ? e->V0 : e->Vs)) return fail(MTTS_EINVAL, "token %lld out of range on channel %d", (long long)t, c);
            if (i < n) { toks[(size_t)i * 8 + c] = (int32_t)t; bm[(size_t)c * e->bm_words + (t >> 5)] |= 1u << (t & 31); }
            else tf[(i - n) * 8 + c] = (int32_t)t;
        }
    for (int i = 0; i < n; ++i) metas[i] = RowMeta{slot, i, i == n - 1 ? 1 : 0, 0};
    TRY(grow_prefill_staging(e, Mpad));
    HIPCHK(hipMemcpy(e->d_pf_tokens, toks.data(), Mpad * 8 * 4, hipMemcpyHostToDevice));
    HIPCHK(hipMemcpy(e->d_pf_meta, metas.data(), Mpad * sizeof(RowMeta), hipMemcpyHostToDevice));
    HIPCHK(hipMemcpy(e->d_bitmaps + (size_t)slot * 8 * e->bm_words, bm.data(), bm.size() * 4, hipMemcpyHostToDevice));
    HIPCHK(hipMemcpy(e->d_tf + (size_t)slot * 7 * 8, tf.data(), tf.size() * 4, hipMemcpyHostToDevice));
    TRY(set_seq_adapter(e, slot, adapter, st));
    TRY(prefill_staged(e, Mpad, (n + MTTS_PAGE - 1) / MTTS_PAGE, 0, adapter >= 0, st));
    if (e->f32) {
        const float* xin = e->hlast_f + (size_t)slot * e->H;
        launch_f32_linear(e->embf[0], xin, (float*)e->logits0 + (size_t)slot * e->V0_pad, 1, e->V0, e->H, e->V0_pad, e->h16, true, st);
        for (int c = 1; c < 8; ++c)
            launch_f32_linear(e->embf[c], xin, (float*)e->logits17 + (size_t)slot * 7 * e->Vs_pad + (size_t)(c - 1) * e->Vs_pad, 1, e->Vs,
                              e->H, 7 * e->Vs_pad, e->h16, true, st);
    } else {
    HIPCHK(hipMemsetAsync(e->xh, 0, (size_t)MTTS_MAXR * e->H * 2, st));
    launch_pack_rows((const uint16_t*)e->hlast + (size_t)slot * e->H, e->xh, 1, e->H, 1, st);
    launch_gemm(EPI_BF16, 1, e->p_h0, e->head0, e->xh, e->H, e->V0_pad, e->V0, nullptr, (uint16_t*)e->join_logits0, st);
    launch_gemm(EPI_BF16, 1, e->p_h17, e->heads17, e->xh, e->H, 7 * e->Vs_pad, 7 * e->Vs_pad, nullptr, (uint16_t*)e->join_logits17, st);
    HIPCHK(hipMemcpyAsync((uint16_t*)e->logits0 + (size_t)slot * e->V0_pad, e->join_logits0, (size_t)e->V0 * 2, hipMemcpyDeviceToDevice, st));
    HIPCHK(hipMemcpyAsync((uint16_t*)e->logits17 + (size_t)slot * 7 * e->Vs_pad, e->join_logits17, (size_t)7 * e->Vs_pad * 2, hipMemcpyDeviceToDevice, st));
    }
    SeqState ns{-1, 1, n, 0, base, max_length, row_id, 1, seed};
    HIPCHK(hipMemcpyAsync(e->d_seqs + slot, &ns, sizeof(ns), hipMemcpyHostToDevice, st));
    int32_t zero = 0;
    HIPCHK(hipMemcpyAsync(&e->d_ls->done, &zero, 4, hipMemcpyHostToDevice, st));
    HIPCHK(hipStreamSynchronize(st));
    e->n_real[slot] = n - e->steps_issued;
    e->join_step[slot] = e->steps_issued;
    e->slot_live[slot] = 1;
    return MTTS_OK;
}

int32_t mtts_slot_fork(MttsEngine* e, int32_t src, int32_t dst, uint64_t seed, int32_t row_id, void* stream) {
    if (!e || !e->began || !e->continuous) return fail(MTTS_ESTATE, "mtts_sched_open has not run");
    if (src < 0 || src >= e->B || dst < 0 || dst >= e->B || src == dst) return fail(MTTS_EINVAL, "fork: slots %d -> %d out of range", src, dst);
    HIPCHK(hipSetDevice(e->device));
    hipStream_t st = S(stream);
    if (!e->slot_live[src] || e->join_step[src] != e->steps_issued)
        return fail(MTTS_ESTATE, "fork: slot %d holds no dialogue submitted since the last step", src);
    HIPCHK(hipMemcpyAsync(e->h_seqs, e->d_seqs, (size_t)e->B * sizeof(SeqState), hipMemcpyDeviceToHost, st));
    HIPCHK(hipStreamSynchronize(st));
    if (!e->h_seqs[src].active || e->h_seqs[src].step) return fail(MTTS_ESTATE, "fork: slot %d has stepped", src);
    if (e->h_seqs[dst].active) return fail(MTTS_ESTATE, "fork: slot %d is occupied", dst);
    if (e->slot_live[dst]) { e->slot_live[dst] = 0; pool_release(e, dst); }
    const int len = e->n_real[src] + e->steps_issued, full = len / MTTS_PAGE, tail = len % MTTS_PAGE != 0;
    if ((int)e->free_pages.size() < tail)
        return fail(MTTS_ENOMEM, "KV page pool: no free page for the take's copy of the last prompt page");
    ForkJob job;
    job.np = 0; job.nr = 1;
    job.rsrc[0] = src; job.rdst[0] = dst;
    int rc = pool_share(e, src, dst, full, st);
    if (!rc && tail) {
        rc = pool_grow(e, dst, full + 1, st);
        job.psrc[0] = e->h_page_table[(size_t)src * e->max_pages + full];
        job.pdst[0] = e->h_page_table[(size_t)dst * e->max_pages + full];
        job.np = 1;
    }
    if (!rc) rc = pool_flush(e, st);
    if (!rc) rc = launch_fork_job(e, job, true, st);
    if (rc) { pool_release(e, dst); return rc; }
    SeqState ns = e->h_seqs[src];
    ns.row_id = row_id; ns.seed = seed;
    e->h_seqs[dst] = ns;
    TRY(set_seq_adapter(e, dst, e->seq_adapter[src], st));
    HIPCHK(hipMemcpyAsync(e->d_seqs + dst, e->h_seqs + dst, sizeof(SeqState), hipMemcpyHostToDevice, st));
    HIPCHK(hipStreamSynchronize(st));
    e->n_real[dst] = e->n_real[src];
    e->join_step[dst] = e->steps_issued;
    e->slot_live[dst] = 1;
    return MTTS_OK;
}

int32_t mtts_slot_states(MttsEngine* e, int32_t* host_state, void* stream) {
    if (!e || !e->began || !host_state) return fail(MTTS_ESTATE, "engine not started");
    HIPCHK(hipSetDevice(e->device));
    std::vector<SeqState> ss(MTTS_RCAP);
    HIPCHK(hipMemcpyAsync(ss.data(), e->d_seqs, ss.size() * sizeof(SeqState), hipMemcpyDeviceToHost, S(stream)));
    HIPCHK(hipStreamSynchronize(S(stream)));
    for (int b = 0; b < e->B; ++b) {
        host_state[b * 4 + 0] = ss[b].active; host_state[b * 4 + 1] = ss[b].unfinished;
        host_state[b * 4 + 2] = ss[b].step; host_state[b * 4 + 3] = ss[b].kv_len;
        if (e->continuous && e->slot_live[b] && !ss[b].active) { e->slot_live[b] = 0; pool_release(e, b); e->seq_adapter[b] = -1; }
    }
    return MTTS_OK;
}

int32_t mtts_slot_evict(MttsEngine* e, int32_t slot, void* stream) {
    if (!e || !e->began || !e->continuous) return fail(MTTS_ESTATE, "mtts_sched_open has not run");
    if (slot < 0 || slot >= e->B) return fail(MTTS_EINVAL, "slot %d out of range", slot);
    HIPCHK(hipSetDevice(e->device));
    HIPCHK(hipStreamSynchronize(S(stream)));
    SeqState cur;
    HIPCHK(hipMemcpy(&cur, e->d_seqs + slot, sizeof(cur), hipMemcpyDeviceToHost));
    cur.active = 0; cur.unfinished = 0;
    HIPCHK(hipMemcpy(e->d_seqs + slot, &cur, sizeof(cur), hipMemcpyHostToDevice));
    RowMeta idle{-1, 0, 0, 0};
    HIPCHK(hipMemcpy(e->d_meta + slot, &idle, sizeof(idle), hipMemcpyHostToDevice));
    if (e->slot_live[slot]) { e->slot_live[slot] = 0; pool_release(e, slot); }
    e->seq_adapter[slot] = -1;
    return MTTS_OK;
}
// ... 80 lines not shown
```

moss-ttsd_amd/csrc/gemm.hip:

```cpp
#include "launch.h"


template <int WAVES, int EPI, int MB>
__global__ __launch_bounds__(WAVES * 64) void gemm_skinny_kernel(
    const u32x4_t* __restrict__ Wp, const u32x4_t* __restrict__ Xp, int KT, int kt_per_split,
    int kt_per_wave, float* __restrict__ partial, uint16_t* __restrict__ out, int Npad, int n_valid) {
    __shared__ float red[WAVES][16][64];
    const int nt = blockIdx.x, ks = blockIdx.y;
    const int wave = threadIdx.x >> 6, lane = threadIdx.x & 63;
    int kt0 = ks * kt_per_split + wave * kt_per_wave;
    int kt1 = min(min(kt0 + kt_per_wave, (ks + 1) * kt_per_split), KT);
    f32x16_t acc[MB];
#pragma unroll
    for (int mb = 0; mb < MB; ++mb)
#pragma unroll
        for (int i = 0; i < 16; ++i) acc[mb][i] = 0.f;
    const u32x4_t* wp = Wp + ((size_t)nt * KT + kt0) * 64 + lane;
    const u32x4_t* xp = Xp + (size_t)kt0 * 64 + lane;
    const size_t xtile = (size_t)KT * 64;
    constexpr int U = (MB == 1) ? 8 : 4;
    int n = kt1 - kt0;
    int i = 0;
    for (; i + U <= n; i += U) {
        u32x4_t a[U], b[U][MB];
#pragma unroll
        for (int u = 0; u < U; ++u) a[u] = __builtin_nontemporal_load(wp + (size_t)(i + u) * 64);
#pragma unroll
        for (int u = 0; u < U; ++u)
#pragma unroll
            for (int mb = 0; mb < MB; ++mb) b[u][mb] = xp[(size_t)(i + u) * 64 + mb * xtile];
#pragma unroll
        for (int u = 0; u < U; ++u)
#pragma unroll
            for (int mb = 0; mb < MB; ++mb)
                acc[mb] = __builtin_amdgcn_mfma_f32_32x32x16_bf16(*(bf16x8_t*)&a[u], *(bf16x8_t*)&b[u][mb], acc[mb], 0, 0, 0);
    }
    for (; i < n; ++i) {
        u32x4_t a = __builtin_nontemporal_load(wp + (size_t)i * 64);
#pragma unroll
        for (int mb = 0; mb < MB; ++mb) {
            u32x4_t b = xp[(size_t)i * 64 + mb * xtile];
            acc[mb] = __builtin_amdgcn_mfma_f32_32x32x16_bf16(*(bf16x8_t*)&a, *(bf16x8_t*)&b, acc[mb], 0, 0, 0);
        }
    }
    const int l2 = threadIdx.x & 63;
#pragma unroll
    for (int mb = 0; mb < MB; ++mb) {
        if (mb) __syncthreads();
#pragma unroll
        for (int r = 0; r < 16; ++r) red[wave][r][lane] = acc[mb][r];
        __syncthreads();
        for (int q = threadIdx.x >> 6; q < 4; q += WAVES) {
            float v[4];
#pragma unroll
            for (int j = 0; j < 4; ++j) {
                float s = red[0][4 * q + j][l2];
#pragma unroll
                for (int w = 1; w < WAVES; ++w) s += red[w][4 * q + j][l2];
                v[j] = s;
            }
            const int row = mb * 32 + (l2 & 31);
            const int nl = 8 * q + 4 * (l2 >> 5);
            const int n0 = nt * 32 + nl;
            if (EPI == EPI_PARTIAL) {
                float4 o = make_float4(v[0], v[1], v[2], v[3]);
                *(float4*)(partial + ((size_t)ks * MTTS_PFCAP + row) * Npad + n0) = o;
            } else if (EPI == EPI_BF16) {
                uint16_t* o = out + (size_t)row * Npad + n0;
                if (n0 + 3 < n_valid) *(u32x2_t*)o = u32x2_t{pack2(v[0], v[1]), pack2(v[2], v[3])};
                else {
#pragma unroll
                    for (int j = 0; j < 4; ++j)
                        if (n0 + j < n_valid) o[j] = f2bf(v[j]);
                }
            } else {
#pragma unroll
                for (int j = 0; j < 2; ++j) {
                    float g = rbf(v[2 * j]), u = rbf(v[2 * j + 1]);
                    float a = rbf(g / (1.0f + expf(-g)));
                    int idx = (n0 >> 1) + j;
                    out[xpack_off(row, idx, Npad >> 1)] = f2bf(a * u);
                }
            }
        }
    }
}

template <int EPI>
__device__ __forceinline__ void skinny_store(const float (&v)[4], int row, int n0, int ks, float* __restrict__ partial,
                                             uint16_t* __restrict__ out, int Npad, int n_valid) {
    if (EPI == EPI_PARTIAL) {
        *(float4*)(partial + ((size_t)ks * MTTS_PFCAP + row) * Npad + n0) = make_float4(v[0], v[1], v[2], v[3]);
    } else if (EPI == EPI_BF16) {
        uint16_t* o = out + (size_t)row * Npad + n0;
        if (n0 + 3 < n_valid) *(u32x2_t*)o = u32x2_t{pack2(v[0], v[1]), pack2(v[2], v[3])};
        else {
#pragma unroll
            for (int j = 0; j < 4; ++j)
                if (n0 + j < n_valid) o[j] = f2bf(v[j]);
        }
    } else {
#pragma unroll
        for (int j = 0; j < 2; ++j) {
            float g = rbf(v[2 * j]), u = rbf(v[2 * j + 1]);
            float a = rbf(g / (1.0f + expf(-g)));
            out[xpack_off(row, (n0 >> 1) + j, Npad >> 1)] = f2bf(a * u);
        }
    }
}

template <int WAVES, int KTW, int EPI>
__global__ __launch_bounds__(WAVES * 64) void gemm_depth_kernel(
    const u32x4_t* __restrict__ Wp, const u32x4_t* __restrict__ Xp, int KT, float* __restrict__ partial,
    uint16_t* __restrict__ out, int Npad, int n_valid) {
    __shared__ float red[WAVES][16][64];
    const int nt = blockIdx.x, ks = blockIdx.y;
    const int wave = threadIdx.x >> 6, lane = threadIdx.x & 63;
    const int kt0 = (ks * WAVES + wave) * KTW;
    const u32x4_t* wp = Wp + ((size_t)nt * KT + kt0) * 64 + lane;
    const u32x4_t* xp = Xp + (size_t)kt0 * 64 + lane;
    u32x4_t a[KTW], b[KTW];
#pragma unroll
    for (int u = 0; u < KTW; ++u) b[u] = xp[(size_t)u * 64];
    __builtin_amdgcn_sched_barrier(0);
#pragma unroll
    for (int u = 0; u < KTW; ++u) {
        a[u] = __builtin_nontemporal_load(wp + (size_t)u * 64);
        __builtin_amdgcn_sched_barrier(0);
    }
    f32x16_t acc;
#pragma unroll
    for (int i = 0; i < 16; ++i) acc[i] = 0.f;
#pragma unroll
    for (int u = 0; u < KTW; ++u)
        acc = __builtin_amdgcn_mfma_f32_32x32x16_bf16(*(bf16x8_t*)&a[u], *(bf16x8_t*)&b[u], acc, 0, 0, 0);
#pragma unroll
    for (int r = 0; r < 16; ++r) red[wave][r][lane] = acc[r];
    __syncthreads();
    for (int q = wave; q < 4; q += WAVES) {
        float v[4];
#pragma unroll
        for (int j = 0; j < 4; ++j) {
            float s = red[0][4 * q + j][lane];
#pragma unroll
            for (int w = 1; w < WAVES; ++w) s += red[w][4 * q + j][lane];
            v[j] = s;
        }
        skinny_store<EPI>(v, lane & 31, nt * 32 + 8 * q + 4 * (lane >> 5), ks, partial, out, Npad, n_valid);
    }
}

template <int WAVES, int KTW>
__global__ __launch_bounds__(WAVES * 64) void gemm_gateup48_kernel(
    const u32x4_t* __restrict__ Wp, const u32x4_t* __restrict__ Xp, int KT, uint16_t* __restrict__ out, int Npad) {
    __shared__ float red[WAVES][24][64];
    const int p = blockIdx.x >> 1, o = blockIdx.x & 1;
    const int tf = 3 * p + 2 * o, th = 3 * p + 1;
    const int wave = threadIdx.x >> 6, lane = threadIdx.x & 63;
    const int kt0 = wave * KTW;
    const int hl = (((lane >> 4) & 1) == o) ? lane : (lane ^ 16);
    const u32x4_t* wp = Wp + ((size_t)tf * KT + kt0) * 64 + lane;
    const u32x4_t* hp = Wp + ((size_t)th * KT + kt0) * 64 + hl;
    const u32x4_t* xp = Xp + (size_t)kt0 * 64 + lane;
    u32x4_t a[KTW], h[KTW], b[KTW];
#pragma unroll
// ... 334 lines not shown
    int KT = K / 16, ntiles = Npad / 32;
    int ks = want_ksplit;
    if (ks <= 0) {
        ks = 1;
        while (ntiles * ks < 256 && ks < 8 && KT / (ks * 2) >= 16) ks *= 2;
    }
    p.ksplit = ks;
    p.kt_per_split = (KT + ks - 1) / ks;
    int w = 8;
    while (w > 1 && p.kt_per_split / w < 4) w >>= 1;
    p.waves = w;
    p.kt_per_wave = (p.kt_per_split + w - 1) / w;
    p.depth = 1;
    return p;
}

template <int EPI, int MB>
static void launch_gemm_epi(const GemmPlan& p, const void* Wp, const void* Xp, int K, int Npad, int n_valid,
                            float* partial, uint16_t* out, hipStream_t st) {
    dim3 grid(Npad / 32, p.ksplit);
    int KT = K / 16;
#define MTTS_GEMM_CASE(WV)                                                                            \
    case WV:                                                                                          \
        hipLaunchKernelGGL((gemm_skinny_kernel<WV, EPI, MB>), grid, dim3(WV * 64), 0, st,             \
                           (const u32x4_t*)Wp, (const u32x4_t*)Xp, KT, p.kt_per_split, p.kt_per_wave, \
                           partial, out, Npad, n_valid);                                              \
        break;
    switch (p.waves) {
        MTTS_GEMM_CASE(8)
        MTTS_GEMM_CASE(4)
        MTTS_GEMM_CASE(2)
        MTTS_GEMM_CASE(1)
    }
#undef MTTS_GEMM_CASE
}

template <int EPI>
static void launch_gemm_mb(int mb, const GemmPlan& p, const void* Wp, const void* Xp, int K, int Npad, int n_valid,
                           float* partial, uint16_t* out, hipStream_t st) {
    if (mb <= 1) launch_gemm_epi<EPI, 1>(p, Wp, Xp, K, Npad, n_valid, partial, out, st);
    else if (mb == 2) launch_gemm_epi<EPI, 2>(p, Wp, Xp, K, Npad, n_valid, partial, out, st);
    else launch_gemm_epi<EPI, 4>(p, Wp, Xp, K, Npad, n_valid, partial, out, st);
}

static long long g_depth_launches = 0;
long long mtts_gemm_depth_launches() { return g_depth_launches; }
static bool launch_gemm_depth(int epi, int mb, const GemmPlan& p, const void* Wp, const void* Xp, int K, int Npad,
                              int n_valid, float* partial, uint16_t* out, hipStream_t st) {
    const int KT = K / 16;
    if (!p.depth || mb > 1 || p.waves != 8 || K % 16 || KT != p.ksplit * 8 * p.kt_per_wave || p.kt_per_split != 8 * p.kt_per_wave)
        return false;
    if (epi == EPI_PARTIAL) {
        dim3 grid(Npad / 32, p.ksplit);
#define MTTS_DEPTH_CASE(KTW)                                                                                        \
    case KTW:                                                                                                       \
        hipLaunchKernelGGL((gemm_depth_kernel<8, KTW, EPI_PARTIAL>), grid, dim3(512), 0, st, (const u32x4_t*)Wp,    \
                           (const u32x4_t*)Xp, KT, partial, out, Npad, n_valid);                                    \
        ++g_depth_launches;                                                                                         \
        return true;
        switch (p.kt_per_wave) {
            MTTS_DEPTH_CASE(4)
            MTTS_DEPTH_CASE(12)
        }
#undef MTTS_DEPTH_CASE
        return false;
    }
    if (epi == EPI_SILU && p.ksplit == 1 && p.kt_per_wave == 16 && Npad % 96 == 0 && n_valid == Npad) {
        hipLaunchKernelGGL((gemm_gateup48_kernel<8, 16>), dim3(Npad / 48), dim3(512), 0, st, (const u32x4_t*)Wp,
                           (const u32x4_t*)Xp, KT, out, Npad);
        ++g_depth_launches;
        return true;
    }
    return false;
}

void launch_gemm(int epi, int mb, const GemmPlan& p, const void* Wp, const void* Xp, int K, int Npad, int n_valid,
                 float* partial, uint16_t* out, hipStream_t st) {
    if (launch_gemm_depth(epi, mb, p, Wp, Xp, K, Npad, n_valid, partial, out, st)) return;
    if (epi == EPI_PARTIAL) launch_gemm_mb<EPI_PARTIAL>(mb, p, Wp, Xp, K, Npad, n_valid, partial, out, st);
    else if (epi == EPI_BF16) launch_gemm_mb<EPI_BF16>(mb, p, Wp, Xp, K, Npad, n_valid, partial, out, st);
    else launch_gemm_mb<EPI_SILU>(mb, p, Wp, Xp, K, Npad, n_valid, partial, out, st);
}


int mtts_small_lds_bytes(const GemmPlan& p, int K, int pro) {
    const int kts = pro == PRO_NORM ? K / 16 : p.kt_per_split;
    return kts * 2 * SMALL_RP * 16;
}
template <int EPI, int PRO>
static void launch_small_epi(const GemmPlan& p0, const void* Wp, int K, int Npad, int n_valid, float* partial, uint16_t* out,
                             const SmallPro& pr, hipStream_t st) {
    GemmPlan p = p0;
    if (p.waves < 4) { p.waves = 4; p.kt_per_wave = (p.kt_per_split + 3) / 4; }
    dim3 grid(Npad / 32, p.ksplit);
    const int KT = K / 16;
    const size_t lds = (size_t)mtts_small_lds_bytes(p, K, PRO);
    if (p.waves == 8)
        hipLaunchKernelGGL((gemv_small_kernel<8, EPI, PRO>), grid, dim3(512), lds, st, (const u32x4_t*)Wp, KT, p.kt_per_split,
                           p.kt_per_wave, partial, out, Npad, n_valid, pr);
    else
        hipLaunchKernelGGL((gemv_small_kernel<4, EPI, PRO>), grid, dim3(256), lds, st, (const u32x4_t*)Wp, KT, p.kt_per_split,
                           p.kt_per_wave, partial, out, Npad, n_valid, pr);
}
void launch_gemv_small(int epi, int pro, const GemmPlan& p, const void* Wp, int K, int Npad, int n_valid, float* partial,
                       uint16_t* out, const SmallPro& pr, hipStream_t st) {
    if (epi == EPI_PARTIAL && pro == PRO_NORM) launch_small_epi<EPI_PARTIAL, PRO_NORM>(p, Wp, K, Npad, n_valid, partial, out, pr, st);
    else if (epi == EPI_PARTIAL && pro == PRO_COMBINE) launch_small_epi<EPI_PARTIAL, PRO_COMBINE>(p, Wp, K, Npad, n_valid, partial, out, pr, st);
    else if (epi == EPI_PARTIAL && pro == PRO_ROWS) launch_small_epi<EPI_PARTIAL, PRO_ROWS>(p, Wp, K, Npad, n_valid, partial, out, pr, st);
    else if (epi == EPI_SILU_RM && pro == PRO_NORM) launch_small_epi<EPI_SILU_RM, PRO_NORM>(p, Wp, K, Npad, n_valid, partial, out, pr, st);
    else if (epi == EPI_BF16 && pro == PRO_NORM) launch_small_epi<EPI_BF16, PRO_NORM>(p, Wp, K, Npad, n_valid, partial, out, pr, st);
}

int mtts_tile_ksplit(int Npad, int K, int R) {
    int blocks = ((Npad + 127) / 128) * ((R + 127) / 128), ks = 1;
    while (blocks * ks < 512 && ks < 8 && (K / 16) / (ks * 2) >= 16) ks *= 2;
    return ks;
}
void launch_gemm_tile(int epi, int R, int ksplit, const void* Wp, const void* Xp, int K, int Npad, int n_valid,
                      float* partial, uint16_t* out, hipStream_t st) {
    const int KT = K / 16, ntiles = Npad / 32, rtiles = (R + 31) / 32;
    const int kps = (KT + ksplit - 1) / ksplit;
    dim3 grid((ntiles + 3) / 4, (rtiles + 3) / 4, ksplit);
#define MTTS_TILE_CASE(E)                                                                                     \
    hipLaunchKernelGGL((gemm_tile_kernel<E>), grid, dim3(256), 0, st, (const u32x4_t*)Wp, (const u32x4_t*)Xp, \
                       KT, kps, ntiles, rtiles, partial, out, Npad, n_valid)
    if (epi == EPI_PARTIAL) MTTS_TILE_CASE(EPI_PARTIAL);
    else if (epi == EPI_BF16) MTTS_TILE_CASE(EPI_BF16);
    else MTTS_TILE_CASE(EPI_SILU);
#undef MTTS_TILE_CASE
}

GemmPlan mtts_plan_gemm(int Npad, int K, int want_ksplit) { return plan_gemm(Npad, K, want_ksplit); }
GemmPlan mtts_plan_gemm_forced(int Npad, int K, int ksplit, int waves) {
    GemmPlan p;
    int KT = K / 16;
    p.ksplit = ksplit;
    p.kt_per_split = (KT + ksplit - 1) / ksplit;
    p.waves = waves;
    p.kt_per_wave = (p.kt_per_split + waves - 1) / waves;
    p.depth = 1;
    return p;
}

void launch_pack_weight(const void* src, void* dst, int rows, int cols, int rows_pad, int row_mul, int row_off, hipStream_t st) {
    size_t total = (size_t)rows_pad * cols / 8;
    int blocks = (int)((total + 255) / 256);
    if (blocks > 4096) blocks = 4096;
    hipLaunchKernelGGL(pack_weight_kernel, dim3(blocks), dim3(256), 0, st, (const uint16_t*)src, (uint16_t*)dst, rows,
                       cols, rows_pad, row_mul, row_off);
}
void launch_pack_rows(const void* src, void* dst, int R, int K, int tiles, hipStream_t st) {
    int total = (K / 16) * 64 * tiles;
    hipLaunchKernelGGL(pack_rows_kernel, dim3((total + 255) / 256), dim3(256), 0, st, (const uint16_t*)src,
                       (uint16_t*)dst, R, K, tiles);
}
void launch_reduce_partial_bf16(const float* partial, void* out, int ksplit, int Npad, int n_valid, int R, hipStream_t st) {
    int total = R * n_valid;
    hipLaunchKernelGGL(reduce_partial_bf16_kernel, dim3((total + 255) / 256), dim3(256), 0, st, partial,
                       (uint16_t*)out, ksplit, Npad, n_valid, R);
}
```

moss-ttsd_amd/csrc/hooks.hip:

```cpp
#include "engine.h"

int32_t mtts_k_gemm_bf16(const void* w, const void* x, void* y, int32_t M, int32_t N, int32_t K, int32_t ksplit, void* stream) {
    if (!w || !x || !y || M < 1 || M > MTTS_PFCAP || K % 16 || N < 1) return fail(MTTS_EINVAL, "gemm: need 1<=M<=MTTS_PFCAP, K%%16==0");
    hipStream_t st = S(stream);
    int Npad = round_up(N, 32);
    void *wp = nullptr, *xp = nullptr;
    float* part = nullptr;
    GemmPlan p = mtts_plan_gemm(Npad, K, ksplit);
    p.depth = gemm_depth_env();
    DevBufs hb;
    TRY(hb.get((uint16_t**)&wp, (size_t)Npad * K));
    const bool tiled = M > MTTS_RCAP;
    const int ks = tiled ? (ksplit > 0 ? ksplit : mtts_tile_ksplit(Npad, K, M)) : p.ksplit;
    TRY(hb.get((uint16_t**)&xp, (size_t)MTTS_PFCAP * K));
    TRY(hb.get(&part, (size_t)ks * MTTS_PFCAP * Npad));
    launch_pack_weight(w, wp, N, K, Npad, 1, 0, st);
    const int tiles = (M + 31) / 32;
    launch_pack_rows(x, xp, M, K, tiles == 3 ? 4 : tiles, st);
    if (tiled) launch_gemm_tile(EPI_PARTIAL, M, ks, wp, xp, K, Npad, Npad, part, nullptr, st);
    else launch_gemm(EPI_PARTIAL, tiles, p, wp, xp, K, Npad, Npad, part, nullptr, st);
    launch_reduce_partial_bf16(part, y, ks, Npad, N, M, st);
    HIPCHK(hipGetLastError());
    HIPCHK(hipStreamSynchronize(st));
    return MTTS_OK;
// ... 576 lines not shown
    std::vector<char> seen(total_pages, 0);
    for (size_t i = 0; i < hpt.size(); ++i) {
        hpt[i] = host_page_table ? host_page_table[i] : (int32_t)i;
        if (hpt[i] < 0 || hpt[i] >= total_pages || seen[hpt[i]]) return fail(MTTS_EINVAL, "page table must be a permutation of 0..%d", total_pages - 1);
        seen[hpt[i]] = 1;
    }
    const int R = round_up((int)M, MTTS_RCAP);
    std::vector<RowMeta> hm(R, RowMeta{-1, 0, 0, 0});
    {
        int r = 0;
        for (int b = 0; b < B; r = round_up(r, MTTS_MAXR), ++b)
            for (int i = host_cached[b]; i < host_lens[b]; ++i, ++r) hm[r] = RowMeta{b, i, i == host_lens[b] - 1 ? 1 : 0, 0};
    }
    hipStream_t st = S(stream);
    RowMeta* meta = nullptr; int32_t *pt = nullptr, *lens = nullptr; uint16_t *kc = nullptr, *vc = nullptr, *qbuf = nullptr, *scores = nullptr, *outp = nullptr;
    float *stats = nullptr, *opart = nullptr, *slabs = nullptr;
    const size_t cache_n = (size_t)total_pages * nkv * MTTS_PAGE * MTTS_HD;
    const size_t q_n = (size_t)R * nq * MTTS_HD, sc_n = (size_t)R * nq * max_pages * MTTS_PAGE, st_n = (size_t)R * nq * max_pages * 2;
    const size_t op_n = (size_t)R * nq * nch_pf * MTTS_HD, sl_n = (size_t)ksplit * MTTS_PFCAP * Npad;
    DevBufs hb;
    TRY(hb.get(&meta, (size_t)R, false)); TRY(hb.get(&pt, hpt.size(), false)); TRY(hb.get(&lens, (size_t)B, false));
    TRY(hb.get(&kc, cache_n)); TRY(hb.get(&vc, cache_n));
    TRY(hb.get(&qbuf, q_n, false)); TRY(hb.get(&scores, sc_n, false)); TRY(hb.get(&stats, st_n, false)); TRY(hb.get(&opart, op_n, false));
    TRY(hb.get(&outp, q_n, false)); TRY(hb.get(&slabs, sl_n, false));
    HIPCHK(hipMemsetAsync(qbuf, 0xff, q_n * 2, st)); HIPCHK(hipMemsetAsync(scores, 0xff, sc_n * 2, st));
    HIPCHK(hipMemsetAsync(stats, 0xff, st_n * 4, st)); HIPCHK(hipMemsetAsync(opart, 0xff, op_n * 4, st));
    HIPCHK(hipMemsetAsync(outp, 0xff, q_n * 2, st)); HIPCHK(hipMemsetAsync(slabs, 0xff, sl_n * 4, st));
    std::vector<int32_t> full(B, Lmax);
    HIPCHK(hipMemcpyAsync(meta, hm.data(), hm.size() * sizeof(RowMeta), hipMemcpyHostToDevice, st));
    HIPCHK(hipMemcpyAsync(pt, hpt.data(), hpt.size() * 4, hipMemcpyHostToDevice, st));
    HIPCHK(hipMemcpyAsync(lens, full.data(), (size_t)B * 4, hipMemcpyHostToDevice, st));
    for (int k = 0; k < ksplit; ++k)
        HIPCHK(hipMemcpyAsync(slabs + (size_t)k * MTTS_PFCAP * Npad, dev_slabs + (size_t)k * M * Npad, (size_t)M * Npad * 4, hipMemcpyDeviceToDevice, st));
    launch_pack_kv_pages(dev_k, dev_v, kc, vc, pt, lens, B, Lmax, nkv, max_pages, total_pages, st);
    const float scale = 1.0f / sqrtf((float)MTTS_HD);
    launch_qkv_post(slabs, ksplit, Npad, meta, dev_qnw, dev_knw, dev_cos, dev_sin, qbuf, kc, vc, pt, max_pages, total_pages, R, nq, nkv, eps, st);
    static const AttnPhase prefill_ph[3] = {ATTN_PF_SCORES, ATTN_PF_PV, ATTN_PF_COMBINE};
    for (int i = 0; i < 3; ++i)
        if (launch_attn(qbuf, kc, vc, pt, meta, scores, stats, opart, outp, R, pages_bound, max_pages, total_pages, nch, nq, nkv, scale,
                        nullptr, prefill_ph[i], st, nullptr))
            return fail(MTTS_EINVAL, "attention group size not built (1, 2, 4)");
    launch_unpack_rows(outp, dev_out, (int)M, nq * MTTS_HD, st);
    HIPCHK(hipGetLastError());
    HIPCHK(hipMemcpyAsync(dev_q, qbuf, (size_t)M * nq * MTTS_HD * 2, hipMemcpyDeviceToDevice, st));
    HIPCHK(hipMemcpyAsync(dev_kcache, kc, cache_n * 2, hipMemcpyDeviceToDevice, st));
    HIPCHK(hipMemcpyAsync(dev_vcache, vc, cache_n * 2, hipMemcpyDeviceToDevice, st));
    HIPCHK(hipStreamSynchronize(st));
    return MTTS_OK;
}

int32_t mtts_k_kv_seal(const void* dev_pages, int32_t npages, void* dev_sealed, int32_t as_k, void* stream) {
    if (!dev_pages || !dev_sealed || npages < 1) return fail(MTTS_EINVAL, "kv_seal: bad argument");
    launch_kv_seal_pages(dev_pages, dev_sealed, npages, as_k, S(stream));
    HIPCHK(hipGetLastError());
    HIPCHK(hipStreamSynchronize(S(stream)));
    return MTTS_OK;
}

int32_t mtts_debug_kv_pack_stats(MttsEngine* e, int64_t* out6) {
    if (!e || !out6) return fail(MTTS_EINVAL, "null argument");
    if (!e->kpack) return fail(MTTS_ESTATE, "the engine keeps no sealed pages (fp32 / fp16 engine, or MTTS_KV_PACK=0)");
    HIPCHK(hipSetDevice(e->device));
    HIPCHK(hipDeviceSynchronize());
    std::vector<SeqState> ss(MTTS_RCAP);
    HIPCHK(hipMemcpy(ss.data(), e->d_seqs, ss.size() * sizeof(SeqState), hipMemcpyDeviceToHost));
    std::vector<int32_t> complete(e->B, 0);
    for (int b = 0; b < e->B; ++b)
        if (e->slot_live[b]) complete[b] = std::min(ss[b].kv_len >> 6, e->n_pages[b]);
    DevBufs hb;
    int32_t* dc = nullptr; unsigned long long* dout = nullptr;
    TRY(hb.get(&dc, e->B)); TRY(hb.get(&dout, 4));
    HIPCHK(hipMemcpy(dc, complete.data(), e->B * 4, hipMemcpyHostToDevice));
    HIPCHK(hipMemset(dout, 0, 32));
    launch_kv_pack_count(e->kpack, e->vpack, e->d_page_table, dc, e->B, e->max_pages, e->total_pages, e->nkv, e->L, dout, nullptr);
    HIPCHK(hipGetLastError());
    unsigned long long h[4];
    HIPCHK(hipMemcpy(h, dout, 32, hipMemcpyDeviceToHost));
    for (int i = 0; i < 4; ++i) out6[i] = (int64_t)h[i];
    out6[4] = out6[5] = 0;
    for (int n = 0; n < e->L; ++n) { out6[4] += e->pack_k_on[n]; out6[5] += e->pack_v_on[n]; }
    return MTTS_OK;
}

int32_t mtts_debug_set_kv_len(MttsEngine* e, int32_t kv_len) {
    if (!e || !e->began) return fail(MTTS_ESTATE, "mtts_begin has not run");
    if (e->f32) return fail(MTTS_EINVAL, "measurement hook of the bf16 engine");
    HIPCHK(hipSetDevice(e->device));
    HIPCHK(hipDeviceSynchronize());
    const int cap = std::min(e->max_pages * MTTS_PAGE, e->rope_rows);
    const int limit = cap - MTTS_PAGE;
    if (kv_len < 1 || kv_len > limit) return fail(MTTS_EINVAL, "kv_len %d outside 1..%d", kv_len, limit);
    e->max_steps = std::min(e->max_steps, e->steps_issued + cap - kv_len);
    std::vector<SeqState> ss(MTTS_RCAP);
    HIPCHK(hipMemcpy(ss.data(), e->d_seqs, ss.size() * sizeof(SeqState), hipMemcpyDeviceToHost));
    for (int b = 0; b < e->B; ++b) { ss[b].kv_len = kv_len; e->n_real[b] = kv_len - e->steps_issued; }
    e->max_real = kv_len - e->steps_issued;
    HIPCHK(hipMemcpy(e->d_seqs, ss.data(), ss.size() * sizeof(SeqState), hipMemcpyHostToDevice));
    launch_fill_random_bf16(e->kcache, e->layer_stride * e->L, 0x1234u, nullptr);
    launch_fill_random_bf16(e->vcache, e->layer_stride * e->L, 0x9876u, nullptr);
    if (e->kpack) launch_kv_seal_all(e->kcache, e->vcache, e->kpack, e->vpack, e->total_pages, e->nkv, e->L, nullptr, nullptr);
    HIPCHK(hipDeviceSynchronize());
    return MTTS_OK;
}

int32_t mtts_k_attn_bench(MttsEngine* e, int32_t phase, int32_t iters, float* avg_ms, int64_t* bytes_per_launch) {
    if (!e || !e->began || phase < ATTN_ALL || phase > ATTN_ROW || iters < 1 || !avg_ms) return fail(MTTS_EINVAL, "attn_bench: bad argument");
    if (e->f32) return fail(MTTS_EINVAL, "measurement hook of the bf16 engine");
    HIPCHK(hipSetDevice(e->device));
    HIPCHK(hipDeviceSynchronize());
    const float scale = 1.0f / sqrtf((float)MTTS_HD);
    const int R = round_up(e->B, 32);
    const int len_bound = e->max_real + e->steps_issued + 1;
    const int pages_bound = (len_bound + MTTS_PAGE - 1) / MTTS_PAGE;
    if (phase == ATTN_ROW) {
        if (attn_row_prepare()) return fail(MTTS_EINVAL, "attn_row_kernel: the dynamic LDS limit could not be raised");
        const QkvFuse f0{e->partial, e->p_qkv.ksplit, e->qkv_rows, nullptr, nullptr, nullptr, nullptr, 0.f};
        for (int n = 0; n < e->L; ++n) {
            const KvPack pk = layer_pack(e, n, pages_bound);
            if (!attn_row_fits(e->nq / e->nkv, &f0, (pk.k || pk.v) ? &pk : nullptr, pages_bound))
                return fail(MTTS_EINVAL, "attn_bench: the whole-row kernel does not take this shape");
        }
    }
    hipEvent_t e0, e1;
    hipEventCreate(&e0); hipEventCreate(&e1);
    auto run = [&](int n) {
        for (int i = 0; i < n; ++i) {
            const int layer = i % e->L;
            uint16_t* kc = (uint16_t*)e->kcache + e->layer_stride * layer;
            uint16_t* vc = (uint16_t*)e->vcache + e->layer_stride * layer;
            const QkvFuse fz{e->partial, e->p_qkv.ksplit, e->qkv_rows, (const uint16_t*)e->layers[layer].qn,
                             (const uint16_t*)e->layers[layer].kn, e->rope_cos, e->rope_sin, e->cfg.rms_norm_eps};
            const KvPack pk = layer_pack(e, layer, pages_bound);
            launch_attn(e->qbuf, kc, vc, e->d_page_table, e->d_meta, e->scores, e->stats, e->opart, e->attn_p, R, pages_bound,
                        e->max_pages, e->total_pages, e->nchunks_max, e->nq, e->nkv, scale, (phase == ATTN_ROW || e->B * pages_bound <= e->fuse_qkv_max) ? &fz : nullptr, (AttnPhase)phase, nullptr,
                        (pk.k || pk.v) ? &pk : nullptr);
        }
    };
    run(e->L);
    hipEventRecord(e0, nullptr);
    run(iters);
    hipEventRecord(e1, nullptr);
    HIPCHK(hipEventSynchronize(e1));
    float ms = 0;
    hipEventElapsedTime(&ms, e0, e1);
    *avg_ms = ms / iters;
    if (bytes_per_launch) {
        std::vector<RowMeta> m(MTTS_RCAP);
        HIPCHK(hipMemcpy(m.data(), e->d_meta, m.size() * sizeof(RowMeta), hipMemcpyDeviceToHost));
        int64_t tok = 0;
        for (int b = 0; b < R; ++b) if (m[b].seq >= 0) tok += m[b].pos + 1;
        *bytes_per_launch = phase == ATTN_COMBINE ? 0 : tok * e->nkv * MTTS_HD * 2 * ((phase == ATTN_ALL || phase == ATTN_ROW) ? 2 : 1);
    }
    hipEventDestroy(e0); hipEventDestroy(e1);
    return MTTS_OK;
}

int32_t mtts_k_gemm_bench(int32_t N, int32_t K, int32_t epi, int32_t ksplit, int32_t waves, int32_t copies,
                                     int32_t iters, float* avg_us) {
    if (N % 32 || K % 16 || copies < 1 || iters < 1 || !avg_us) return fail(MTTS_EINVAL, "gemm_bench: bad argument");
    const int tile_rows = waves < 0 ? -waves : 0;
    if (tile_rows > MTTS_PFCAP) return fail(MTTS_EINVAL, "gemm_bench: at most MTTS_PFCAP rows");
    GemmPlan p = (ksplit > 0 && waves > 0) ? mtts_plan_gemm_forced(N, K, ksplit, waves) : mtts_plan_gemm(N, K, tile_rows ? std::max(ksplit, 1) : ksplit);
    if (tile_rows) p.ksplit = std::max(ksplit, 1);
    p.depth = gemm_depth_env();
    DevBufs hb;
    std::vector<uint16_t*> w(copies, nullptr);
// ... 26 lines not shown
```

moss-ttsd_amd/csrc/launch.h:

```cpp
#pragma once
#include <type_traits>

#include "../../include/mtts.h"
#include "common.h"

enum { EPI_PARTIAL = 0, EPI_BF16 = 1, EPI_SILU = 2,
       EPI_SILU_RM = 3 };
struct GemmPlan {
    int waves, ksplit, kt_per_split, kt_per_wave;
    int depth;
};
GemmPlan mtts_plan_gemm(int Npad, int K, int want_ksplit);
GemmPlan mtts_plan_gemm_forced(int Npad, int K, int ksplit, int waves);
void launch_gemm(int epi, int mb, const GemmPlan& p, const void* Wp, const void* Xp, int K, int Npad, int n_valid,
                 float* partial, uint16_t* out, hipStream_t st);
int mtts_tile_ksplit(int Npad, int K, int R);
void launch_gemm_tile(int epi, int R, int ksplit, const void* Wp, const void* Xp, int K, int Npad, int n_valid,
                      float* partial, uint16_t* out, hipStream_t st);
int mtts_small_lds_bytes(const GemmPlan& p, int K, int pro);
void launch_gemv_small(int epi, int pro, const GemmPlan& p, const void* Wp, int K, int Npad, int n_valid, float* partial,
                       uint16_t* out, const SmallPro& pr, hipStream_t st);
long long mtts_gemm_depth_launches();
void launch_pack_weight(const void* src, void* dst, int rows, int cols, int rows_pad, int row_mul, int row_off, hipStream_t st);
void launch_pack_rows(const void* src, void* dst, int R, int K, int tiles, hipStream_t st);
void launch_reduce_partial_bf16(const float* partial, void* out, int ksplit, int Npad, int n_valid, int R, hipStream_t st);

struct PageEdits { int32_t n; int32_t idx[31]; int32_t val[31]; };
static_assert(sizeof(PageEdits) == 252, "PageEdits is a kernel argument: one 32-bit count + 31 (index, value) pairs");
void launch_embed_norm(const int32_t* tokens, const RowMeta* meta, const uint16_t* const* tables, const void* norm_w,
                       void* x, void* xn_packed, int R, int H, float eps, hipStream_t st);
void launch_resid_norm(const float* partial, int ksplit, int Npad, void* x, const void* norm_w, void* xn_packed,
                       void* hlast, const RowMeta* meta, int R, int H, float eps, hipStream_t st);
void launch_qkv_post(const float* partial, int ksplit, int Npad, const RowMeta* meta, const void* qnw, const void* knw,
                     const void* cosb, const void* sinb, void* qbuf, void* kcache, void* vcache,
                     const int32_t* page_table, int max_pages, int total_pages, int R, int nq, int nkv, float eps,
                     hipStream_t st);
void launch_rmsnorm_rows(const void* x, const void* w, void* y, int rows, int n, float eps, hipStream_t st);
void launch_fill_random_bf16(void* p, size_t n, uint32_t seed, hipStream_t st);
void launch_set_pages(int32_t* table, const PageEdits& ed, hipStream_t st);
void launch_fork(void* kc, void* vc, size_t layer_bytes, size_t head_bytes, int blk_bytes, int L, int nkv, const ForkJob& job,
                 hipStream_t st);
void launch_pack_kv_pages(const void* K, const void* V, void* kcache, void* vcache, const int32_t* page_table, const int32_t* lens,
                          int S, int Lmax, int nkv, int max_pages, int total_pages, hipStream_t st);
void launch_bf16_to_f32(const void* a, float* b, size_t n, hipStream_t st);
void launch_unpack_rows(const void* packed, void* out, int R, int K, hipStream_t st);

enum AttnPhase { ATTN_ALL = 0, ATTN_SCORES = 1, ATTN_PV = 2, ATTN_COMBINE = 3,
                 ATTN_ROW = 4,
                 ATTN_PF_SCORES = 11, ATTN_PF_PV = 12, ATTN_PF_COMBINE = 13 };
int launch_attn(const void* qbuf, void* kcache, void* vcache, const int32_t* page_table,
                const RowMeta* meta, void* scores, float* stats, float* opart, void* out_packed, int R,
                int pages_bound, int max_pages, int total_pages, int nchunks_max, int nq, int nkv, float scale,
                const QkvFuse* fuse, AttnPhase phase, hipStream_t st, const KvPack* pack = nullptr);
bool attn_row_fits(int G, const QkvFuse* fuse, const KvPack* pack, int pages_bound);
int attn_row_prepare();
int attn_row_lds_limit();
long long mtts_attn_row_launches();
void launch_kv_seal_rows(const void* kcache, const void* vcache, void* kpack, void* vpack, const int32_t* page_table,
                         const RowMeta* meta, int R, int max_pages, int total_pages, int nkv, int L, unsigned long long* cnt, hipStream_t st);
void launch_kv_seal_all(const void* kcache, const void* vcache, void* kpack, void* vpack, int total_pages, int nkv, int L,
                        unsigned long long* cnt, hipStream_t st);
void launch_kv_seal_pages(const void* raw, void* pk, int npages, int as_k, hipStream_t st);
void launch_kv_pack_count(const void* kpack, const void* vpack, const int32_t* page_table, const int32_t* complete, int B, int max_pages,
                          int total_pages, int nkv, int L, unsigned long long* out, hipStream_t st);

struct SeqState {
    int32_t nas;
    int32_t unfinished;
    int32_t kv_len;
    int32_t step;
    int32_t base_length;
    int32_t max_length;
    int32_t row_id;
    int32_t active;
    uint64_t seed;
};

struct LoopState {
    int32_t step;
    int32_t done;
    int32_t continuous;
    int32_t B;
    int32_t error;
    int32_t gen_cap;
    int32_t forced_draw;
    int32_t logits_f32;
};
static_assert(sizeof(SeqState) == 40 && std::is_trivially_copyable<SeqState>::value, "SeqState layout");
static_assert(sizeof(LoopState) == 32 && std::is_trivially_copyable<LoopState>::value, "LoopState layout");

#define SAMP_CAND 4096
#define SAMP_NS 32
struct SampleScratch {
    uint32_t* hist = nullptr;
    float* slice_val = nullptr;
    int32_t* slice_idx = nullptr;
    float* cand_val = nullptr;
    int32_t* cand_idx = nullptr;
// ... 70 lines not shown
```

moss-ttsd_amd/csrc/sampler.hip:

```cpp
#include "launch.h"

__device__ __forceinline__ void philox4x32_10(uint32_t c0, uint32_t c1, uint32_t c2, uint32_t c3, uint32_t k0,
                                              uint32_t k1, uint32_t* out) {
#pragma unroll
    for (int i = 0; i < 10; ++i) {
        uint64_t p0 = (uint64_t)0xD2511F53u * c0;
        uint64_t p1 = (uint64_t)0xCD9E8D57u * c2;
        uint32_t n0 = (uint32_t)(p1 >> 32) ^ c1 ^ k0;
        uint32_t n1 = (uint32_t)p1;
        uint32_t n2 = (uint32_t)(p0 >> 32) ^ c3 ^ k1;
        uint32_t n3 = (uint32_t)p0;
        c0 = n0; c1 = n1; c2 = n2; c3 = n3;
        k0 += 0x9E3779B9u;
        k1 += 0xBB67AE85u;
    }
    out[0] = c0; out[1] = c1; out[2] = c2; out[3] = c3;
}

__device__ __forceinline__ uint32_t fkey(float f) {
    uint32_t u = __float_as_uint(f);
    return (u & 0x80000000u) ? ~u : (u | 0x80000000u);
}

struct LogitsPtr { const void* p; int f32; };
__device__ __forceinline__ float proc_score(LogitsPtr logits, int i, int mask_id,
                                            const uint32_t* __restrict__ bitmap, float penalty, float temperature) {
    if (i == mask_id) return -INFINITY;
    float s = logits.f32 ? ((const float*)logits.p)[i] : bf2f(((const uint16_t*)logits.p)[i]);
    if (penalty > 0.f && (bitmap[i >> 5] >> (i & 31)) & 1u) s = (s < 0.f) ? s * penalty : s / penalty;
    if (temperature > 0.f) s = s / temperature;
    return s;
}

#define SAMP_T 256

struct SampleCtx {
    LogitsPtr lg;
    const uint32_t* bm;
    int V, mask_id, step, c;
    float penalty, temp;
    uint64_t seed;
    uint32_t row_id;
};

__device__ __forceinline__ bool sample_ctx(SampleCtx& x, int b, int c_in, const uint16_t* logits0,
                                           const uint16_t* logits17, int V0, int Vs, int Vs_pad,
                                           const uint32_t* bitmaps, int bm_words, const MttsSamplerCfg* cfgs,
                                           const LoopState* ls, const SeqState* seqs, int single_vocab, int single_mask,
                                           int single_step, int single_channel) {
    if (single_vocab > 0) {
        x.c = single_channel; x.step = single_step; x.V = single_vocab; x.mask_id = single_mask;
        x.seed = 0; x.row_id = (uint32_t)b;
        x.lg = LogitsPtr{logits0 + (size_t)b * x.V, 0};
        x.bm = bitmaps ? bitmaps + (size_t)b * bm_words : nullptr;
    } else {
        if (ls->done) return false;
        const SeqState sq = seqs[b];
        if (!sq.active || !(sq.unfinished || sq.active == 2)) return false;
        x.c = c_in; x.step = sq.step;
        x.seed = sq.seed; x.row_id = (uint32_t)sq.row_id;
        x.V = (x.c == 0) ? V0 : Vs;
        {
            const size_t off = (x.c == 0) ? (size_t)b * ((V0 + 31) & ~31) : ((size_t)b * 7 + (x.c - 1)) * Vs_pad;
            const char* base = (const char*)((x.c == 0) ? logits0 : logits17);
            x.lg = LogitsPtr{base + off * (ls->logits_f32 ? 4 : 2), ls->logits_f32};
        }
        x.mask_id = -1;
        if (x.c != 0 && x.step >= x.c) x.mask_id = 1024;
        if (x.c == 0 && x.step <= 6) x.mask_id = 152694;
        x.bm = bitmaps ? bitmaps + ((size_t)b * 8 + x.c) * bm_words : nullptr;
    }
    const MttsSamplerCfg cfg = cfgs[x.c];
    x.penalty = (x.bm && cfg.repetition_penalty > 0.f) ? cfg.repetition_penalty : 0.f;
    x.temp = cfg.temperature;
    return true;
}

__device__ __forceinline__ void argmax_merge(float& bv, int& bi, float ov, int oi) {
    if (ov > bv || (ov == bv && oi < bi)) { bv = ov; bi = oi; }
}

__device__ __forceinline__ void block_argmax(float& bv, int& bi, float* shf, int* shi) {
#pragma unroll
    for (int o = 32; o > 0; o >>= 1) argmax_merge(bv, bi, __shfl_xor(bv, o, 64), __shfl_xor(bi, o, 64));
    const int wid = threadIdx.x >> 6, nw = blockDim.x >> 6;
    __syncthreads();
    if ((threadIdx.x & 63) == 0) { shf[wid] = bv; shi[wid] = bi; }
    __syncthreads();
    bv = shf[0]; bi = shi[0];
    for (int w = 1; w < nw; ++w) argmax_merge(bv, bi, shf[w], shi[w]);
    __syncthreads();
}

template <int NT>
__device__ __forceinline__ double block_excl_scan(double v, double* sh, double& total) {
    const int lane = threadIdx.x & 63, wid = threadIdx.x >> 6;
    double inc = v;
#pragma unroll
    for (int o = 1; o < 64; o <<= 1) {
        double t = __shfl_up(inc, o, 64);
        if (lane >= o) inc += t;
    }
    __syncthreads();
    if (lane == 63) sh[wid] = inc;
    __syncthreads();
    double base = 0.0, tot = 0.0;
    for (int w = 0; w < NT / 64; ++w) { if (w < wid) base += sh[w]; tot += sh[w]; }
    total = tot;
    __syncthreads();
    return base + inc - v;
}

template <bool LP>
__global__ __launch_bounds__(SAMP_T) void sample_scan_kernel(
    const uint16_t* __restrict__ logits0, int V0, const uint32_t* __restrict__ bitmaps, int bm_words,
    const MttsSamplerCfg* __restrict__ cfgs, const LoopState* __restrict__ ls, const SeqState* __restrict__ seqs,
    SampleScratch sc, int single_vocab,
    int single_mask, int single_step, int single_channel) {
    __shared__ uint32_t hist[2048];
    __shared__ float shf[SAMP_T / 64];
    __shared__ int shi[SAMP_T / 64];
    __shared__ double shd[SAMP_T / 64];
    const int b = blockIdx.y, slice = blockIdx.x, tid = threadIdx.x;
    SampleCtx x;
    if (!sample_ctx(x, b, 0, logits0, nullptr, V0, 0, 0, bitmaps, bm_words, cfgs, ls, seqs, single_vocab, single_mask,
                    single_step, single_channel)) return;
    const MttsSamplerCfg cfg = cfgs[x.c];
    const bool want_hist = cfg.do_sample && cfg.top_k > 0 && cfg.top_k < x.V;
    for (int i = tid; i < 2048; i += SAMP_T) hist[i] = 0;
    __syncthreads();
    const int per = (x.V + SAMP_NS - 1) / SAMP_NS;
    const int i0 = slice * per, i1 = min(x.V, i0 + per);
    float bv = -INFINITY;
    int bi = 0x7fffffff;
    for (int i = i0 + tid; i < i1; i += SAMP_T) {
        float s = proc_score(x.lg, i, x.mask_id, x.bm, x.penalty, x.temp);
        argmax_merge(bv, bi, s, i);
        if (want_hist) atomicAdd(&hist[fkey(s) >> 21], 1u);
    }
    block_argmax(bv, bi, shf, shi);
    if (tid == 0) { sc.slice_val[b * SAMP_NS + slice] = bv; sc.slice_idx[b * SAMP_NS + slice] = bi; }
    if (LP && !cfg.do_sample) {
        float loc = 0.f;
        if (bv > -INFINITY)
            for (int i = i0 + tid; i < i1; i += SAMP_T) {
                const float s = proc_score(x.lg, i, x.mask_id, x.bm, x.penalty, x.temp);
                if (s > -INFINITY) loc += expf(s - bv);
            }
        double tot;
        (void)block_excl_scan<SAMP_T>((double)loc, shd, tot);
        if (tid == 0) sc.slice_sum[b * SAMP_NS + slice] = (float)tot;
    }
    if (want_hist)
        for (int i = tid; i < 2048; i += SAMP_T)
            if (hist[i]) atomicAdd(&sc.hist[(size_t)b * 2048 + i], hist[i]);
}

#define SAMP_FT 1024
#define NUC_BINS 2048
#define NUC_SCALE 35184372088832.0
typedef unsigned long long u64;

struct NucSel {
    uint32_t kmin;
    uint32_t kp;
    int idp;
};
__device__ __forceinline__ float unfkey(uint32_t k) { return __uint_as_float((k & 0x80000000u) ? (k & 0x7fffffffu) : ~k); }
__device__ __forceinline__ bool nuc_in(const NucSel& z, uint32_t key, int id) {
    return key > 0x007fffffu  && key >= z.kmin && (key > z.kp || (key == z.kp && id >= z.idp));
}
__device__ __forceinline__ int nuc_bin(uint32_t key, float lo) {
    const int b = (int)((unfkey(key) - lo) * ((float)(NUC_BINS - 1) / 32.0f));
    return min(max(b, 0), NUC_BINS - 1);
}

__device__ __forceinline__ u64 nuc_q(uint32_t key, float smax) { return (u64)((double)expf(unfkey(key) - smax) * NUC_SCALE); }

__device__ __forceinline__ void nuc_pass_a(const SampleCtx& x, float smax, float lo, uint32_t* __restrict__ keys,
                                           uint16_t* __restrict__ bins, unsigned int* cnt, u64* mass, int i0, int i1, int step) {
    for (int i = i0; i < i1; i += step) {
        const float s = proc_score(x.lg, i, x.mask_id, x.bm, x.penalty, x.temp) + 0.0f;
        const uint32_t key = fkey(s);
        keys[i] = key;
        if (s > -INFINITY) {
            const int d = nuc_bin(key, lo);
            bins[i] = (uint16_t)d;
            atomicAdd(&cnt[d], 1u);
            atomicAdd(&mass[d], nuc_q(key, smax));
        } else bins[i] = 0xffffu;
    }
}


__device__ __forceinline__ int topk_bin(const uint32_t* hist, uint32_t k, uint32_t* wsum, int* sh_b0) {
    const int tid = threadIdx.x, lane = tid & 63, wid = tid >> 6;
    const uint32_t* h = hist + tid * 8;
    uint32_t cnt[8], mine = 0;
#pragma unroll
    for (int j = 0; j < 8; ++j) { cnt[j] = h[j]; mine += cnt[j]; }
    uint32_t suf = mine;
#pragma unroll
    for (int o = 1; o < 64; o <<= 1) {
        uint32_t t = __shfl_down(suf, o, 64);
        if (lane + o < 64) suf += t;
    }
    if (lane == 0) wsum[wid] = suf;
    if (tid == 0) *sh_b0 = 0;
    __syncthreads();
    uint32_t above_waves = 0;
    for (int w = wid + 1; w < SAMP_T / 64; ++w) above_waves += wsum[w];
    const uint32_t above = above_waves + suf - mine;
    if (above < k && above + mine >= k) {
        uint32_t run = above;
        for (int j = 7; j >= 0; --j) {
            run += cnt[j];
            if (run >= k) { *sh_b0 = tid * 8 + j; break; }
        }
    }
    __syncthreads();
    return *sh_b0;
}

__global__ __launch_bounds__(SAMP_T) void sample_collect_kernel(
    const uint16_t* __restrict__ logits0, int V0, const uint32_t* __restrict__ bitmaps, int bm_words,
    const MttsSamplerCfg* __restrict__ cfgs, const LoopState* __restrict__ ls, const SeqState* __restrict__ seqs,
    SampleScratch sc, int full_cap, int single_vocab,
    int single_mask, int single_step, int single_channel) {
    __shared__ uint32_t wsum[SAMP_T / 64];
    __shared__ int sh_b0;
    const int b = blockIdx.y, slice = blockIdx.x, tid = threadIdx.x, lane = tid & 63, wid = tid >> 6;
    SampleCtx x;
    if (!sample_ctx(x, b, 0, logits0, nullptr, V0, 0, 0, bitmaps, bm_words, cfgs, ls, seqs, single_vocab, single_mask,
                    single_step, single_channel)) return;
    const MttsSamplerCfg cfg = cfgs[x.c];
    if (!cfg.do_sample) return;
    if (!(cfg.top_k > 0 && cfg.top_k < x.V) || cfg.top_k > SAMP_CAND) {
        __shared__ unsigned int a_cnt[2048];
        __shared__ unsigned long long a_mass[2048];
        float smax = sc.slice_val[b * SAMP_NS + (lane & (SAMP_NS - 1))];
        smax = wave_max(smax);
        for (int i = tid; i < 2048; i += SAMP_T) { a_cnt[i] = 0; a_mass[i] = 0; }
        __syncthreads();
        const int per = (x.V + SAMP_NS - 1) / SAMP_NS;
        const int i0 = slice * per, i1 = min(x.V, i0 + per);
        nuc_pass_a(x, smax, smax - 32.0f, (uint32_t*)(sc.full_idx + (size_t)b * full_cap), (uint16_t*)(sc.full_val + (size_t)b * full_cap),
                   a_cnt, a_mass, i0 + tid, i1, SAMP_T);
        __syncthreads();
        for (int i = tid; i < 2048; i += SAMP_T)
            if (a_cnt[i]) { atomicAdd(&sc.nuc_cnt[(size_t)b * 2048 + i], a_cnt[i]); atomicAdd(&sc.nuc_mass[(size_t)b * 2048 + i], a_mass[i]); }
        if (slice == 0 && tid == 0) { sc.cand_n[b] = SAMP_CAND + 1; sc.overflow[b] = 2; }
        return;
    }
    const int b0 = topk_bin(sc.hist + (size_t)b * 2048, (uint32_t)cfg.top_k, wsum, &sh_b0);
    const uint32_t ninf_key = fkey(-INFINITY);
    const int per = (x.V + SAMP_NS - 1) / SAMP_NS;
    const int i0 = slice * per, i1 = min(x.V, i0 + per);
    for (int i = i0 + tid; i < i1; i += SAMP_T) {
        float s = proc_score(x.lg, i, x.mask_id, x.bm, x.penalty, x.temp);
        uint32_t key = fkey(s);
        if ((int)(key >> 21) >= b0 && key > ninf_key) {
            uint32_t slot = atomicAdd(&sc.cand_n[b], 1u);
            if (slot < SAMP_CAND) { sc.cand_val[(size_t)b * SAMP_CAND + slot] = s; sc.cand_idx[(size_t)b * SAMP_CAND + slot] = i; }
        }
    }
}

template <int NT>
__device__ int finish_sample(float* __restrict__ cval, int* __restrict__ cidx, int n, const MttsSamplerCfg& cfg, float smax,
                             uint32_t step, uint32_t b, uint32_t c, uint64_t seed, double* shd, int* sh_i, float* lp) {
    const int tid = threadIdx.x;
    int P = 1;
    while (P < n) P <<= 1;
    for (int i = n + tid; i < P; i += NT) { cval[i] = INFINITY; cidx[i] = 0x7fffffff; }
    __syncthreads();
    for (int kk = 2; kk <= P; kk <<= 1) {
        for (int j = kk >> 1; j > 0; j >>= 1) {
            for (int t = tid; t < P; t += NT) {
                int ixj = t ^ j;
                if (ixj > t) {
                    bool up = ((t & kk) == 0);
                    float a = cval[t], bb = cval[ixj];
                    int ai = cidx[t], bi2 = cidx[ixj];
                    bool gt = (a > bb) || (a == bb && ai > bi2);
                    if (gt == up) { cval[t] = bb; cval[ixj] = a; cidx[t] = bi2; cidx[ixj] = ai; }
                }
            }
            __syncthreads();
        }
    }
    int f0 = 0;
    if (cfg.top_k > 0 && cfg.top_k < n) {
        const float thr = cval[n - cfg.top_k];
        int cnt = 0;
        for (int i = tid; i < n; i += NT) cnt += (cval[i] < thr) ? 1 : 0;
        double tot;
        (void)block_excl_scan<NT>((double)cnt, shd, tot);
        f0 = (int)tot;
    }
    const int m = n - f0;
    const int per = (m + NT - 1) / NT;
    int first_keep = f0;
    if (cfg.top_p > 0.f && cfg.top_p < 1.0f) {
        const int a0 = f0 + tid * per, a1 = min(n, a0 + per);
        double loc = 0.0;
        for (int i = a0; i < a1; ++i) loc += (double)expf(cval[i] - smax);
        double tot;
        double base = block_excl_scan<NT>(loc, shd, tot);
        int drop = 0;
        double run = base;
        for (int i = a0; i < a1; ++i) {
            run += (double)expf(cval[i] - smax);
            if (i < n - 1 && (float)(run / tot) <= cfg.one_minus_top_p) drop++;
        }
        double dtot;
        (void)block_excl_scan<NT>((double)drop, shd, dtot);
        first_keep = f0 + (int)dtot;
    }
    const int nk = n - first_keep;
    const int perk = (nk + NT - 1) / NT;
    const int r0 = tid * perk, r1 = min(nk, r0 + perk);
    double loc = 0.0;
    for (int r = r0; r < r1; ++r) loc += (double)expf(cval[n - 1 - r] - smax);
    double tot;
    double base = block_excl_scan<NT>(loc, shd, tot);
    uint32_t rnd[4];
    philox4x32_10(step, b, c, 0u, (uint32_t)seed, (uint32_t)(seed >> 32), rnd);
    const double u = (double)((float)(rnd[0] >> 8) * (1.0f / 16777216.0f));
    const double target = u * tot;
    if (tid == 0) sh_i[1] = 0x7fffffff;
    __syncthreads();
    double run = base;
    for (int r = r0; r < r1; ++r) {
        run += (double)expf(cval[n - 1 - r] - smax);
        if (run > target) { atomicMin(&sh_i[1], r); break; }
    }
    __syncthreads();
    int r = sh_i[1];
    if (r >= nk) r = nk - 1;
    if (lp && tid == 0) *lp = (float)((double)(cval[n - 1 - r] - smax) - log(tot));
    return cidx[n - 1 - r];
}

template <bool LP>
__global__ __launch_bounds__(SAMP_T) void sample_final_kernel(
    const uint16_t* __restrict__ logits0, const uint16_t* __restrict__ logits17, int V0, int Vs, int Vs_pad,
    const uint32_t* __restrict__ bitmaps, int bm_words, const MttsSamplerCfg* __restrict__ cfgs,
    const LoopState* __restrict__ ls, const SeqState* __restrict__ seqs, uint64_t seed, int32_t* __restrict__ decisions,
// ... 370 lines not shown
                const bool take = s.unfinished != 0 || (linger && ls->forced_draw == 2);
#pragma unroll
                for (int c = 0; c < 8; ++c) {
                    dec_log[slot + c] = tok[c];
                    const int f = forced[slot + c];
                    if (f >= 0 && take) tok[c] = f;
                }
            }
            const bool speech = tok[0] >= sp_lo && tok[0] < sp_hi;
            if ((s.unfinished || linger) && !speech && s.nas < 0) s.nas = 7;
            if (step < 7) {
#pragma unroll
                for (int c = 0; c < 8; ++c)
                    if (c >= step + 1) tok[c] = tf_tail[(b * 7 + step) * 8 + c];
            }
            if (s.nas > 0 && s.nas < 7) {
                tok[0] = eos;
#pragma unroll
                for (int c = 1; c < 8; ++c)
                    if (s.nas < 8 - c) tok[c] = spad;
            }
            if (!s.unfinished) {
                tok[0] = eos;
#pragma unroll
                for (int c = 1; c < 8; ++c) tok[c] = spad;
            }
            if (lp_out) {
                const bool flush = s.nas > 0 && s.nas < 7;
#pragma unroll
                for (int c = 0; c < 8; ++c) {
                    const bool used = s.unfinished && !(step < 7 && c >= step + 1) && !(flush && (c == 0 || s.nas < 8 - c));
                    lp_out[slot + c] = used ? lp_in[b * 8 + c] : __uint_as_float(0x7fc00000u);
                }
            }
            if (dec_log && !as_draw) {
#pragma unroll
                for (int c = 0; c < 8; ++c) dec_log[slot + c] = tok[c];
            }
            if (forced && !as_draw) {
#pragma unroll
                for (int c = 0; c < 8; ++c) {
                    int f = forced[slot + c];
                    if (f >= 0) tok[c] = f;
                }
            }
#pragma unroll
            for (int c = 0; c < 8; ++c) {
                gen[slot + c] = tok[c];
                cur_tokens[b * 8 + c] = tok[c];
                uint32_t* bm = bitmaps + ((size_t)b * 8 + c) * bm_words;
                bm[tok[c] >> 5] |= 1u << (tok[c] & 31);
            }
            if (s.nas > 0) s.nas -= 1;
            const int new_len = s.base_length + step + 1;
            const bool stopping = (new_len >= s.max_length) || (tok[0] == eos) || (s.nas == 0);
            s.unfinished = (s.unfinished && !stopping) ? 1 : 0;
            if (s.nas > 0) s.unfinished = 1;
            s.step = step + 1;
            if (ls->continuous) {
                if (!s.unfinished) s.active = 0;
            } else {
                s.active = (!s.unfinished && s.nas < 0) ? 2 : 1;
            }
            meta[b].seq = (s.unfinished || s.active == 2) ? b : -1;
            meta[b].pos = s.kv_len;
            meta[b].last = 1;
            s.kv_len += 1;
            seqs[b] = s;
            if (s.unfinished) atomicOr(&any_unfinished, 1);
        }
    }
    __syncthreads();
    if (b == 0) {
        ls->step = ls->step + 1;
        if (!any_unfinished) ls->done = 1;
    }
}

static SampleScratch g_dummy_scratch;
void launch_sample(const void* logits0, const void* logits17, int V0, int Vs, int Vs_pad, const uint32_t* bitmaps, int bm_words,
                   const MttsSamplerCfg* cfgs, const LoopState* ls, const SeqState* seqs, uint64_t seed, int32_t* decisions,
                   int32_t* err, int B, const SampleScratch& sc, int ch0_sampled, int full_cap, int emit_lp, hipStream_t st) {
    const int big0 = V0 > SAMP_CAND ? 1 : 0;
    if (big0) {
        hipLaunchKernelGGL(emit_lp ? sample_scan_kernel<true> : sample_scan_kernel<false>, dim3(SAMP_NS, B), dim3(SAMP_T), 0, st,
                           (const uint16_t*)logits0, V0, bitmaps, bm_words, cfgs, ls, seqs, sc, 0, 0, 0, 0);
        if (ch0_sampled)
            hipLaunchKernelGGL(sample_collect_kernel, dim3(SAMP_NS, B), dim3(SAMP_T), 0, st, (const uint16_t*)logits0, V0,
                               bitmaps, bm_words, cfgs, ls, seqs, sc, full_cap, 0, 0, 0, 0);
    }
    hipLaunchKernelGGL(emit_lp ? sample_final_kernel<true> : sample_final_kernel<false>, dim3(8, B), dim3(SAMP_T), 0, st,
                       (const uint16_t*)logits0, (const uint16_t*)logits17, V0, Vs, Vs_pad, bitmaps, bm_words, cfgs, ls, seqs, seed,
                       decisions, err, sc, big0, 0, 0, 0, 0);
    if (big0 && ch0_sampled)
        hipLaunchKernelGGL(sample_full_kernel, dim3(B), dim3(SAMP_FT), 0, st, (const uint16_t*)logits0, V0, bitmaps,
                           bm_words, cfgs, ls, seqs, seed, decisions, sc, full_cap, emit_lp, 0, 0, 0, 0);
}
void launch_sample_single(const void* logits, int rows, int vocab, const uint32_t* bitmap, int bm_words,
                          const MttsSamplerCfg* cfgs8, int mask_id, uint64_t seed, int step, int channel,
                          int32_t* decisions, int32_t* err, const SampleScratch& sc, int full_cap, int emit_lp, hipStream_t st) {
    if (vocab > SAMP_CAND) {
        hipLaunchKernelGGL(emit_lp ? sample_scan_kernel<true> : sample_scan_kernel<false>, dim3(SAMP_NS, rows), dim3(SAMP_T), 0, st,
                           (const uint16_t*)logits, vocab, bitmap, bm_words, cfgs8, (const LoopState*)nullptr,
                           (const SeqState*)nullptr, sc, vocab, mask_id, step, channel);
        hipLaunchKernelGGL(sample_collect_kernel, dim3(SAMP_NS, rows), dim3(SAMP_T), 0, st, (const uint16_t*)logits, vocab,
                           bitmap, bm_words, cfgs8, (const LoopState*)nullptr, (const SeqState*)nullptr, sc, full_cap, vocab, mask_id, step, channel);
    }
    hipLaunchKernelGGL(emit_lp ? sample_final_kernel<true> : sample_final_kernel<false>, dim3(1, rows), dim3(SAMP_T), 0, st,
                       (const uint16_t*)logits, (const uint16_t*)nullptr, vocab, vocab, vocab, bitmap, bm_words, cfgs8,
                       (const LoopState*)nullptr, (const SeqState*)nullptr, seed, decisions, err, sc, 1, vocab, mask_id, step, channel);
    if (vocab > SAMP_CAND)
        hipLaunchKernelGGL(sample_full_kernel, dim3(rows), dim3(SAMP_FT), 0, st, (const uint16_t*)logits, vocab, bitmap,
                           bm_words, cfgs8, (const LoopState*)nullptr, (const SeqState*)nullptr, seed, decisions, sc, full_cap, emit_lp,
                           vocab, mask_id, step, channel);
}
void launch_update(const int32_t* decisions, int32_t* dec_log, const int32_t* forced, const int32_t* tf_tail,
                   int32_t* gen, int32_t* cur_tokens, SeqState* seqs, RowMeta* meta, uint32_t* bitmaps, int bm_words,
                   LoopState* ls, int eos, int spad, int sp_lo, int sp_hi, const float* lp_in, float* lp_out, hipStream_t st) {
    hipLaunchKernelGGL(update_kernel, dim3(1), dim3(MTTS_RCAP), 0, st, decisions, dec_log, forced, tf_tail, gen,
                       cur_tokens, seqs, meta, bitmaps, bm_words, ls, eos, spad, sp_lo, sp_hi, lp_in, lp_out);
}

__global__ void export_codes_kernel(const int32_t* __restrict__ gen, int64_t* __restrict__ codes, int B, int first, int n,
                                    int speech_offset, int clamp_hi, int cap) {
    const int i = blockIdx.x * blockDim.x + threadIdx.x;
    if (i >= 8 * B * n) return;
    const int t = i % n, b = (i / n) % B, c = i / (n * B);
    int v = gen[((size_t)b * cap + (first + t + c)) * 8 + c];
    if (c == 0) v -= speech_offset;
    v = min(max(v, 0), clamp_hi);
    codes[i] = v;
}
void launch_export_codes(const int32_t* gen, int64_t* codes, int B, int first, int n, int speech_offset, int clamp_hi,
                         int cap, hipStream_t st) {
    int total = 8 * B * n;
    hipLaunchKernelGGL(export_codes_kernel, dim3((total + 255) / 256), dim3(256), 0, st, gen, codes, B, first, n,
                       speech_offset, clamp_hi, cap);
}
```

moss-ttsd_amd/mtts/capi.py:

```python
from __future__ import annotations

import ctypes as C
import os

_HERE = os.path.dirname(os.path.abspath(__file__))
LIB_PATH = os.path.join(os.path.dirname(_HERE), "lib", "libmtts.so")


class MttsConfig(C.Structure):
    _fields_ = [(n, C.c_int32) for n in (
        "vocab_size", "hidden_size", "intermediate_size", "num_hidden_layers", "num_attention_heads",
        "num_key_value_heads", "head_dim", "channels", "speech_vocab_size", "speech_pad_token",
        "speech_range_lo", "speech_range_hi", "eos_token_id", "max_position")] + [
        ("rms_norm_eps", C.c_float), ("max_batch", C.c_int32), ("max_seq_len", C.c_int32), ("kv_pool_pages", C.c_int32), ("dtype", C.c_int32)]


class MttsSamplerCfg(C.Structure):
    _fields_ = [("do_sample", C.c_int32), ("top_k", C.c_int32), ("top_p", C.c_float),
                ("one_minus_top_p", C.c_float), ("temperature", C.c_float), ("repetition_penalty", C.c_float)]


class MttsCodecConfig(C.Structure):
    _fields_ = [(n, C.c_int32) for n in (
        "nq", "codebook_size", "rvq_dim", "quant_out_dim",
        "adapter_layers", "adapter_dim", "adapter_heads", "adapter_ffn", "adapter_max_pos", "up_stride",
        "dec_layers", "dec_dim", "dec_heads", "dec_ffn", "dec_max_pos", "mel_bins",
        "voc_dim", "voc_inter", "voc_layers", "n_fft", "hop",
        "mel_n_fft", "mel_hop", "mel_frames", "enc_layers", "enc_dim", "enc_heads", "enc_ffn", "enc_max_pos",
        "sem_adapter_layers", "pre_rvq_layers", "down_pool")]


class MttsError(RuntimeError):
    def __init__(self, msg, code=0):
        super().__init__(msg)
        self.code = code


EINVAL = -1
ENOMEM = -3
ESTATE = -4


_lib = None

_SIGS = {
    "mtts_last_error": (C.c_char_p, []),
    "mtts_version": (C.c_int32, []),
    "mtts_engine_create": (C.c_int32, [C.POINTER(MttsConfig), C.c_int32, C.POINTER(C.c_void_p)]),
    "mtts_engine_destroy": (C.c_int32, [C.c_void_p]),
    "mtts_bind_weight": (C.c_int32, [C.c_void_p, C.c_char_p, C.c_void_p, C.c_int64, C.c_int64, C.c_void_p]),
    "mtts_bind_weight_lora": (C.c_int32, [C.c_void_p, C.c_char_p, C.c_void_p, C.c_int64, C.c_int64, C.c_void_p, C.c_void_p,
                                          C.c_int32, C.c_float, C.c_void_p]),
    "mtts_k_lora_pack": (C.c_int32, [C.c_void_p, C.c_int32, C.c_int32, C.c_void_p, C.c_void_p, C.c_int32, C.c_float,
                                     C.c_int32, C.c_int32, C.c_int32, C.c_int32, C.c_void_p, C.c_void_p]),
    "mtts_adapter_load": (C.c_int32, [C.c_void_p, C.c_int32, C.c_char_p, C.c_void_p, C.c_void_p, C.c_int64, C.c_int64, C.c_int32,
                                      C.c_float, C.c_void_p]),
    "mtts_adapter_clear": (C.c_int32, [C.c_void_p, C.c_int32]),
    "mtts_set_row_adapters": (C.c_int32, [C.c_void_p, C.c_void_p, C.c_int32]),
    "mtts_set_slot_adapter": (C.c_int32, [C.c_void_p, C.c_int32, C.c_int32]),
    "mtts_k_lora_delta": (C.c_int32, [C.c_void_p, C.c_int32, C.c_int32, C.c_int32, C.c_int32, C.c_void_p, C.c_int32] +
                          [C.c_void_p] * 6 + [C.c_int32, C.c_void_p]),
    "mtts_k_swiglu_slabs": (C.c_int32, [C.c_void_p] * 5 + [C.c_int32] * 3 + [C.c_void_p]),
    "mtts_bind_rope": (C.c_int32, [C.c_void_p, C.c_void_p, C.c_void_p, C.c_int32, C.c_void_p]),
    "mtts_weights_ready": (C.c_int32, [C.c_void_p]),
    "mtts_generate": (C.c_int32, [C.c_void_p, C.c_void_p, C.c_void_p, C.c_int32, C.c_int32, C.c_int32,
                                  C.POINTER(MttsSamplerCfg), C.c_uint64, C.c_void_p, C.c_int32,
                                  C.POINTER(C.c_int32), C.c_void_p, C.c_int32, C.c_void_p, C.c_void_p]),
    "mtts_begin": (C.c_int32, [C.c_void_p, C.c_void_p, C.c_void_p, C.c_int32, C.c_int32, C.c_int32,
                               C.POINTER(MttsSamplerCfg), C.c_uint64, C.c_void_p]),
    "mtts_step": (C.c_int32, [C.c_void_p, C.c_int32, C.c_void_p]),
    "mtts_sync_state": (C.c_int32, [C.c_void_p, C.POINTER(C.c_int32), C.POINTER(C.c_int32), C.c_void_p]),
    "mtts_read_generated": (C.c_int32, [C.c_void_p, C.c_void_p, C.c_int32, C.POINTER(C.c_int32)]),
    "mtts_set_output_scores": (C.c_int32, [C.c_void_p, C.c_int32]),
    "mtts_read_scores": (C.c_int32, [C.c_void_p, C.c_void_p, C.c_int32, C.POINTER(C.c_int32)]),
    "mtts_slot_read_scores": (C.c_int32, [C.c_void_p, C.c_int32, C.c_void_p, C.c_int32, C.POINTER(C.c_int32)]),
    "mtts_score": (C.c_int32, [C.c_void_p, C.c_void_p, C.c_void_p, C.c_void_p, C.c_int32, C.c_int32, C.c_void_p, C.c_void_p]),
    "mtts_score_topk": (C.c_int32, [C.c_void_p, C.c_void_p, C.c_void_p, C.c_void_p, C.c_int32, C.c_int32, C.c_void_p, C.c_int32,
                                    C.c_void_p, C.c_void_p, C.c_void_p]),
    "mtts_read_logits": (C.c_int32, [C.c_void_p, C.c_void_p, C.c_void_p, C.c_void_p]),
    "mtts_read_logits_f32": (C.c_int32, [C.c_void_p, C.c_void_p, C.c_void_p, C.c_void_p]),
    "mtts_sched_open": (C.c_int32, [C.c_void_p, C.c_int32, C.c_int32, C.POINTER(MttsSamplerCfg), C.c_void_p]),
    "mtts_slot_submit": (C.c_int32, [C.c_void_p, C.c_int32, C.c_void_p, C.c_int32, C.c_int32, C.c_uint64, C.c_void_p]),
    "mtts_slot_submit_row": (C.c_int32, [C.c_void_p, C.c_int32, C.c_void_p, C.c_int32, C.c_int32, C.c_uint64, C.c_int32, C.c_void_p]),
    "mtts_set_row_ids": (C.c_int32, [C.c_void_p, C.c_void_p, C.c_int32]),
    "mtts_set_takes": (C.c_int32, [C.c_void_p, C.c_int32]),
    "mtts_slot_fork": (C.c_int32, [C.c_void_p, C.c_int32, C.c_int32, C.c_uint64, C.c_int32, C.c_void_p]),
    "mtts_slot_states": (C.c_int32, [C.c_void_p, C.c_void_p, C.c_void_p]),
    "mtts_slot_read": (C.c_int32, [C.c_void_p, C.c_int32, C.c_void_p, C.c_int32, C.POINTER(C.c_int32)]),
    "mtts_read_seq_state": (C.c_int32, [C.c_void_p, C.c_void_p, C.c_void_p, C.c_void_p, C.c_void_p]),
    "mtts_slot_evict": (C.c_int32, [C.c_void_p, C.c_int32, C.c_void_p]),
    "mtts_kv_pool_state": (C.c_int32, [C.c_void_p, C.POINTER(C.c_int32), C.POINTER(C.c_int32), C.POINTER(C.c_int32)]),
    "mtts_read_page_table": (C.c_int32, [C.c_void_p, C.c_void_p, C.c_void_p]),
    "mtts_set_forced_mode": (C.c_int32, [C.c_void_p, C.c_int32]),
    "mtts_debug_read_device_page_table": (C.c_int32, [C.c_void_p, C.c_void_p, C.c_void_p]),
    "mtts_export_codes": (C.c_int32, [C.c_void_p, C.c_int32, C.c_int32, C.c_void_p, C.c_void_p]),
    "mtts_profile_enable": (C.c_int32, [C.c_void_p, C.c_int32]),
    "mtts_profile_read": (C.c_int32, [C.c_void_p, C.c_int32, C.POINTER(C.c_double), C.POINTER(C.c_int64),
                                      C.POINTER(C.c_int64)]),
    "mtts_debug_set_kv_len": (C.c_int32, [C.c_void_p, C.c_int32]),
    "mtts_debug_kv_pack_stats": (C.c_int32, [C.c_void_p, C.c_void_p]),
    "mtts_k_kv_seal": (C.c_int32, [C.c_void_p, C.c_int32, C.c_void_p, C.c_int32, C.c_void_p]),
    "mtts_k_attn_bench": (C.c_int32, [C.c_void_p, C.c_int32, C.c_int32, C.POINTER(C.c_float), C.POINTER(C.c_int64)]),
    "mtts_k_gemm_bench": (C.c_int32, [C.c_int32] * 7 + [C.POINTER(C.c_float)]),
    "mtts_k_gemm_bf16": (C.c_int32, [C.c_void_p, C.c_void_p, C.c_void_p, C.c_int32, C.c_int32, C.c_int32,
                                     C.c_int32, C.c_void_p]),
    "mtts_debug_gemm_depth_launches": (C.c_int64, []),
    "mtts_debug_attn_row_launches": (C.c_int64, []),
    "mtts_k_attn_section": (C.c_int32, [C.c_void_p, C.c_int32] + [C.c_void_p] * 4 + [C.c_float] + [C.c_void_p] * 4 +
                            [C.c_int32] * 6 + [C.c_void_p] * 6),
    "mtts_k_attn_prefill": (C.c_int32, [C.c_void_p, C.c_int32] + [C.c_void_p] * 4 + [C.c_float] + [C.c_void_p] * 5 +
                            [C.c_int32] * 4 + [C.c_void_p] * 5),
    "mtts_k_gemm_swiglu_bf16": (C.c_int32, [C.c_void_p, C.c_void_p, C.c_void_p, C.c_int32, C.c_int32, C.c_int32, C.c_void_p]),
    "mtts_k_rmsnorm": (C.c_int32, [C.c_void_p, C.c_void_p, C.c_void_p, C.c_int32, C.c_int32, C.c_float, C.c_void_p]),
    "mtts_k_embed_norm": (C.c_int32, [C.c_void_p] * 5 + [C.c_int32, C.c_int32, C.c_float] + [C.c_void_p] * 3),
    "mtts_k_resid_norm": (C.c_int32, [C.c_void_p, C.c_int32, C.c_int32] + [C.c_void_p] * 4 + [C.c_int32] * 3 + [C.c_float] +
                          [C.c_void_p] * 3),
    "mtts_k_gemv_small": (C.c_int32, [C.c_int32, C.c_int32, C.c_void_p] + [C.c_int32] * 4 + [C.c_void_p, C.c_void_p, C.c_int32,
                                      C.c_void_p, C.c_float] + [C.c_void_p] * 4 + [C.c_int32, C.c_int32] + [C.c_void_p] * 4),
    "mtts_k_gemm_tile": (C.c_int32, [C.c_int32] + [C.c_void_p] * 3 + [C.c_int32] * 4 + [C.c_void_p]),
    "mtts_k_rope_kvwrite": (C.c_int32, [C.c_void_p] * 6 + [C.c_int32, C.c_int32, C.c_int32, C.c_float] + [C.c_void_p] * 4),
    "mtts_k_paged_attn_decode": (C.c_int32, [C.c_void_p] * 5 + [C.c_int32] * 4 + [C.c_void_p, C.c_void_p]),
    "mtts_k_head_ce": (C.c_int32, [C.c_void_p, C.c_void_p, C.c_void_p] + [C.c_int32] * 5 + [C.c_void_p, C.c_void_p]),
    "mtts_k_head_topk": (C.c_int32, [C.c_void_p, C.c_void_p] + [C.c_int32] * 6 + [C.c_void_p, C.c_void_p, C.c_void_p]),
    "mtts_k_sample": (C.c_int32, [C.c_void_p, C.c_int32, C.c_int32, C.c_void_p, C.POINTER(MttsSamplerCfg),
                                  C.c_int32, C.c_uint64, C.c_int32, C.c_int32, C.c_void_p, C.c_void_p]),
    "mtts_k_sample_scores": (C.c_int32, [C.c_void_p, C.c_int32, C.c_int32, C.c_void_p, C.POINTER(MttsSamplerCfg),
                                         C.c_int32, C.c_uint64, C.c_int32, C.c_int32, C.c_void_p, C.c_void_p, C.c_void_p]),
    "mtts_codec_last_error": (C.c_char_p, []),
    "mtts_codec_create": (C.c_int32, [C.POINTER(MttsCodecConfig), C.c_int32, C.POINTER(C.c_void_p)]),
    "mtts_codec_destroy": (C.c_int32, [C.c_void_p]),
    "mtts_codec_bind": (C.c_int32, [C.c_void_p, C.c_char_p, C.c_void_p, C.c_int64, C.c_void_p]),
    "mtts_codec_detokenize": (C.c_int32, [C.c_void_p, C.c_void_p, C.c_void_p, C.c_int32, C.c_int32, C.c_void_p, C.c_void_p]),
    "mtts_codec_detokenize_async": (C.c_int32, [C.c_void_p, C.c_void_p, C.c_void_p, C.c_int32, C.c_int32, C.c_void_p, C.c_void_p]),
    "mtts_codec_check": (C.c_int32, [C.c_void_p, C.c_void_p]),
    "mtts_codec_tokenize": (C.c_int32, [C.c_void_p, C.c_void_p, C.c_void_p, C.c_int32, C.c_int32, C.c_void_p, C.c_void_p, C.c_void_p]),
    "mtts_k_gemm_f32": (C.c_int32, [C.c_void_p, C.c_void_p, C.c_void_p, C.c_void_p, C.c_int32, C.c_int32, C.c_int32,
                                    C.c_int32, C.c_void_p]),
    "mtts_k_gemm_planes_bench": (C.c_int32, [C.c_int32, C.c_int32, C.c_int32, C.c_int32, C.c_int32, C.c_int32,
                                             C.POINTER(C.c_float), C.POINTER(C.c_int32)]),
}


def exported_symbols():
    return sorted(_SIGS)


def lib():
    global _lib
    if _lib is None:
        if not os.path.exists(LIB_PATH):
            raise MttsError(f"{LIB_PATH} is missing: build it with `python moss-ttsd_amd/build.py` "
                            "(hipcc --offload-arch=gfx950); there is no CPU fallback")
        L = C.CDLL(LIB_PATH)
        for name, (res, args) in _SIGS.items():
            fn = getattr(L, name)
            fn.restype = res
            fn.argtypes = args
        _lib = L
    return _lib


def check(rc):
    if rc != 0:
        raise MttsError(f"libmtts error {rc}: {lib().mtts_last_error().decode()}", rc)
```

moss-ttsd_amd/mtts/engine.py:

```python
from __future__ import annotations

import ctypes as C

import numpy as np
import torch

from . import capi


def sampler_cfgs(layers=None, do_samples=None):
    arr = (capi.MttsSamplerCfg * 8)()
    for i in range(8):
        lc = (layers[i] if layers and i < len(layers) else {}) or {}
        s = arr[i]
        s.do_sample = 1 if (do_samples and do_samples[i]) else 0
        s.top_k = int(lc.get("top_k") or 0)
        tp = lc.get("top_p")
        s.top_p = float(tp) if tp is not None else 0.0
        s.one_minus_top_p = float(np.float32(1.0 - tp)) if tp is not None else 0.0
        t = lc.get("temperature")
        s.temperature = float(t) if t is not None else 0.0
        rp = lc.get("repetition_penalty")
        s.repetition_penalty = float(rp) if rp is not None else 0.0
    return arr
# ... 209 lines not shown
    def read_logits(self):
        V0, Vs = self.cfg["vocab_size"], self.cfg["speech_vocab_size"]
        if self.dtype != "bf16":
            l0 = np.zeros((self._B, V0), dtype=np.float32)
            l17 = np.zeros((7, self._B, Vs), dtype=np.float32)
            capi.check(self.lib.mtts_read_logits_f32(self._h, l0.ctypes.data, l17.ctypes.data, None))
            return l0, l17
        l0 = np.zeros((self._B, V0), dtype=np.uint16)
        l17 = np.zeros((7, self._B, Vs), dtype=np.uint16)
        capi.check(self.lib.mtts_read_logits(self._h, l0.ctypes.data, l17.ctypes.data, None))
        f = lambda u: (u.astype(np.uint32) << 16).view(np.float32)
        return f(l0), f(l17)

    def sched_open(self, slots, gen_cap, layers=None, do_samples=None, output_scores=False):
        self._B = int(slots)
        self.set_output_scores(output_scores)
        capi.check(self.lib.mtts_sched_open(self._h, int(slots), int(gen_cap), sampler_cfgs(layers, do_samples), None))

    def submit(self, slot, ids, max_length, seed=0, row_id=0, adapter=None):
        ids = np.ascontiguousarray(ids, dtype=np.int64)
        assert ids.ndim == 2 and ids.shape[1] == 8
        if adapter is not None and int(adapter) >= 0:
            capi.check(self.lib.mtts_set_slot_adapter(self._h, int(slot), int(adapter)))
        capi.check(self.lib.mtts_slot_submit_row(self._h, int(slot), ids.ctypes.data, ids.shape[0], int(max_length),
                                                 C.c_uint64(seed), int(row_id), None))

    def fork(self, src, dst, seed=0, row_id=0):
        capi.check(self.lib.mtts_slot_fork(self._h, int(src), int(dst), C.c_uint64(seed), int(row_id), None))

    def slot_states(self):
        st = np.zeros((self._B, 4), dtype=np.int32)
        capi.check(self.lib.mtts_slot_states(self._h, st.ctypes.data, None))
        return st

    def slot_read(self, slot, capacity):
        buf = np.zeros((int(capacity), 8), dtype=np.int64)
        n = C.c_int32(0)
        capi.check(self.lib.mtts_slot_read(self._h, int(slot), buf.ctypes.data, int(capacity), C.byref(n)))
        return buf[:n.value].copy()

    def slot_read_scores(self, slot, capacity):
        buf = np.zeros((max(int(capacity), 1), 8), dtype=np.float32)
        n = C.c_int32(0)
        capi.check(self.lib.mtts_slot_read_scores(self._h, int(slot), buf.ctypes.data, buf.shape[0], C.byref(n)))
        return buf[:n.value].copy()

    def evict(self, slot):
        capi.check(self.lib.mtts_slot_evict(self._h, int(slot), None))

    def kv_pool_state(self):
        a, b, c = C.c_int32(0), C.c_int32(0), C.c_int32(0)
        capi.check(self.lib.mtts_kv_pool_state(self._h, C.byref(a), C.byref(b), C.byref(c)))
        return a.value, b.value, c.value

    def page_table(self, max_batch):
        _, _, mp = self.kv_pool_state()
        t = np.zeros((int(max_batch), mp), dtype=np.int32)
        n = np.zeros(int(max_batch), dtype=np.int32)
        capi.check(self.lib.mtts_read_page_table(self._h, t.ctypes.data, n.ctypes.data))
        return t, n

    def device_page_table(self, max_batch):
        _, _, mp = self.kv_pool_state()
        t = np.zeros((int(max_batch), mp), dtype=np.int32)
        capi.check(self.lib.mtts_debug_read_device_page_table(self._h, t.ctypes.data, None))
        return t

    def seq_state(self):
        a, u, k = (np.zeros(self._B, dtype=np.int32) for _ in range(3))
        capi.check(self.lib.mtts_read_seq_state(self._h, a.ctypes.data, u.ctypes.data, k.ctypes.data, None))
        return a, u, k

    def export_codes(self, first, n, stream=None):
        out = torch.empty(8, self._B, n, dtype=torch.int64, device=self.device)
        sp = C.c_void_p(stream.cuda_stream) if stream is not None else None
        capi.check(self.lib.mtts_export_codes(self._h, int(first), int(n), out.data_ptr(), sp))
        return out

    def kv_pack_stats(self):
        o = np.zeros(6, dtype=np.int64)
        capi.check(self.lib.mtts_debug_kv_pack_stats(self._h, o.ctypes.data))
        return dict(zip(("k_pages", "k_unsealed", "v_pages", "v_unsealed", "k_layers_on", "v_layers_on"), (int(x) for x in o)))

    def debug_set_kv_len(self, n):
        capi.check(self.lib.mtts_debug_set_kv_len(self._h, int(n)))

    def attn_bench(self, phase, iters=112):
        ms, by = C.c_float(0), C.c_int64(0)
        capi.check(self.lib.mtts_k_attn_bench(self._h, int(phase), int(iters), C.byref(ms), C.byref(by)))
        return ms.value, by.value

    def profile(self, on=True):
        capi.check(self.lib.mtts_profile_enable(self._h, 1 if on else 0))

    def profile_read(self, which):
        ms, n, by = C.c_double(0), C.c_int64(0), C.c_int64(0)
        capi.check(self.lib.mtts_profile_read(self._h, which, C.byref(ms), C.byref(n), C.byref(by)))
        return ms.value, n.value, by.value
```

Before: 81830 codec_tokens/s.

## Skip KV seal on non-page-completing steps, fuse head GEMMs, vectorize sampler

Several independent changes land together. Decode steps where no live row finishes a KV page now skip the seal-scan kernel, and step graphs are keyed on that flag. The two output-head GEMMs (channel 0 and channels 1-7) are merged into one launch when their plans match. The sampler scan/collect kernels get a vectorized slice walk, and collect uses a wave-level prefix sum in place of per-element atomics. The seal kernel also takes fewer rows per block to spread work wider. The cost is extra cached graph variants, more kernel template instantiations and some debug hooks.

Result: no change. 82220 codec_tokens/s (median of 6 runs) (+0.5%).

```diff
diff --git a/include/mtts.h b/include/mtts.h
--- a/include/mtts.h
+++ b/include/mtts.h
@@ -119,6 +119,8 @@
 
 int32_t mtts_debug_set_kv_len(MttsEngine* e, int32_t kv_len);
 int32_t mtts_debug_kv_pack_stats(MttsEngine* e, int64_t* out6);
+int32_t mtts_debug_step_counts(MttsEngine* e, int64_t* out2);
+int32_t mtts_debug_read_kv_pack(MttsEngine* e, int32_t which, void* host_out, int64_t cap_bytes, int64_t* bytes);
 int32_t mtts_k_attn_bench(MttsEngine* e, int32_t phase, int32_t iters, float* avg_ms, int64_t* bytes_per_launch);
 int32_t mtts_k_gemm_bench(int32_t N, int32_t K, int32_t epi, int32_t ksplit, int32_t waves, int32_t copies,
                           int32_t iters, float* avg_us);
diff --git a/moss-ttsd_amd/csrc/attn.hip b/moss-ttsd_amd/csrc/attn.hip
--- a/moss-ttsd_amd/csrc/attn.hip
+++ b/moss-ttsd_amd/csrc/attn.hip
@@ -215,17 +215,20 @@
     if (cnt && lane == 0) atomicAdd(cnt + layer * 4 + wave * 2 + (all ? 0 : 1), 1ull);
 }
 
+#ifndef SEAL_RPB
+#define SEAL_RPB 16
+#endif
 __global__ __launch_bounds__(128) void kv_seal_scan_kernel(const u32x4_t* __restrict__ kcache, const u32x4_t* __restrict__ vcache,
                                                            u32x4_t* __restrict__ kpack, u32x4_t* __restrict__ vpack,
                                                            const int32_t* __restrict__ page_table, const RowMeta* __restrict__ meta, int R,
-                                                           int max_pages, int total_pages, size_t raw_layer, size_t pk_layer,
+                                                           int rpb, int max_pages, int total_pages, size_t raw_layer, size_t pk_layer,
                                                            unsigned long long* __restrict__ cnt) {
     __shared__ __attribute__((aligned(16))) uint8_t klds[8192 + 128];
     __shared__ __attribute__((aligned(16))) uint8_t vlds[8192 + 320];
     const int kvh = blockIdx.y, layer = blockIdx.z, wave = threadIdx.x >> 6, lane = threadIdx.x & 63;
-    const int r = blockIdx.x * 64 + lane;
+    const int r = blockIdx.x * rpb + lane;
     RowMeta m{-1, 0, 0, 0};
-    if (r < R) m = meta[r];
+    if (lane < rpb && r < R) m = meta[r];
     unsigned long long todo = __ballot(m.seq >= 0 && (m.pos & 63) == 63);
     while (todo) {
         const int i = __ffsll((long long)todo) - 1;
@@ -290,8 +293,10 @@
 void launch_kv_seal_rows(const void* kcache, const void* vcache, void* kpack, void* vpack, const int32_t* page_table,
                          const RowMeta* meta, int R, int max_pages, int total_pages, int nkv, int L, unsigned long long* cnt, hipStream_t st) {
     const size_t raw_layer = (size_t)total_pages * nkv * (MTTS_PAGE * MTTS_HD / 8), pk_layer = (size_t)total_pages * nkv * (MTTS_PKU * 64);
-    hipLaunchKernelGGL(kv_seal_scan_kernel, dim3((R + 63) / 64, nkv, L), dim3(128), 0, st, (const u32x4_t*)kcache, (const u32x4_t*)vcache,
-                       (u32x4_t*)kpack, (u32x4_t*)vpack, page_table, meta, R, max_pages, total_pages, raw_layer, pk_layer, cnt);
+    int rpb = SEAL_RPB;
+    if (const char* g = getenv("MTTS_SEAL_RPB")) rpb = std::min(std::max(atoi(g), 1), 64);
+    hipLaunchKernelGGL(kv_seal_scan_kernel, dim3((R + rpb - 1) / rpb, nkv, L), dim3(128), 0, st, (const u32x4_t*)kcache, (const u32x4_t*)vcache,
+                       (u32x4_t*)kpack, (u32x4_t*)vpack, page_table, meta, R, rpb, max_pages, total_pages, raw_layer, pk_layer, cnt);
 }
 void launch_kv_seal_all(const void* kcache, const void* vcache, void* kpack, void* vpack, int total_pages, int nkv, int L,
                         unsigned long long* cnt, hipStream_t st) {
diff --git a/moss-ttsd_amd/csrc/engine.h b/moss-ttsd_amd/csrc/engine.h
--- a/moss-ttsd_amd/csrc/engine.h
+++ b/moss-ttsd_amd/csrc/engine.h
@@ -214,7 +214,7 @@
     int max_real = 0;
     uint64_t seed = 0;
     bool began = false, has_forced = false;
-    struct StepGraph { int B, pages, forced, ch0, scores, row, lora; hipGraphExec_t exec; };
+    struct StepGraph { int B, pages, forced, ch0, scores, row, lora, noseal; hipGraphExec_t exec; };
     std::vector<StepGraph> graphs;
     hipStream_t cap_stream = nullptr;
     bool use_graphs = true;
@@ -222,6 +222,9 @@
     void *kpack = nullptr, *vpack = nullptr;
     size_t pk_layer_stride = 0;
     unsigned long long *d_seal_cnt = nullptr, *h_seal_cnt = nullptr;
+    bool step_noseal = true;
+    bool skip_seal = false;
+    long long steps_sealing = 0, steps_noseal = 0;
     std::vector<char> pack_k_on, pack_v_on;
     int pack_min_work = 512;
     int fuse_qkv_max = 2560;
diff --git a/moss-ttsd_amd/csrc/engine.hip b/moss-ttsd_amd/csrc/engine.hip
--- a/moss-ttsd_amd/csrc/engine.hip
+++ b/moss-ttsd_amd/csrc/engine.hip
@@ -179,6 +179,7 @@
     if (const char* g = getenv("MTTS_KV_PACK")) e->kv_pack = atoi(g);
     if (const char* g = getenv("MTTS_KV_PACK_MIN")) e->pack_min_work = atoi(g);
     if (const char* g = getenv("MTTS_PREFILL_MFMA_PAGES")) e->pf_mfma_pages = atoi(g);
+    if (const char* g = getenv("MTTS_STEP_NOSEAL")) e->step_noseal = atoi(g) != 0;
     if (const char* g = getenv("MTTS_ATTN_ROW")) e->attn_row = std::min(std::max(atoi(g), 0), 2);
     HIPCHK(hipDeviceGetAttribute(&e->n_cus, hipDeviceAttributeMultiprocessorCount, device));
     if (e->attn_row && attn_row_prepare()) {
@@ -669,7 +670,7 @@
         pd.xrows = (const uint16_t*)e->act_rm;
         launch_gemv_small(EPI_PARTIAL, PRO_ROWS, e->p_d, l.wd, I, Hp, Hp, e->partial2, nullptr, pd, st);
     }
-    if (e->kpack)
+    if (e->kpack && !e->skip_seal)
         launch_kv_seal_rows(e->kcache, e->vcache, e->kpack, e->vpack, e->d_page_table, d_meta, R, e->max_pages, e->total_pages, nkv, e->L, e->d_seal_cnt, st);
     SmallPro ph = base;
     ph.x_in = xa; ph.x_out = nullptr; ph.slabs = e->partial2; ph.ksplit = e->p_d.ksplit; ph.norm_w = (const uint16_t*)e->final_norm;
@@ -726,7 +727,7 @@
         const void* nw = lastl ? e->final_norm : e->layers[n + 1].ln_in;
         launch_resid_norm(e->partial, ks_d + ex, Hp, e->x, nw, e->xn, lastl ? e->hlast : nullptr, d_meta, R, H, eps, st);
     }
-    if (e->kpack)
+    if (e->kpack && !e->skip_seal)
         launch_kv_seal_rows(e->kcache, e->vcache, e->kpack, e->vpack, e->d_page_table, d_meta, R, e->max_pages, e->total_pages, nkv, e->L, e->d_seal_cnt, st);
     if (heads) {
         const void* xin = e->xn;
@@ -736,8 +737,8 @@
             launch_pack_rows(e->hlast, e->xh, e->B, H, hmb, st);
             xin = e->xh;
         }
-        launch_gemm(EPI_BF16, hmb, e->p_h0, e->head0, xin, H, e->V0_pad, e->V0, nullptr, (uint16_t*)e->logits0, st);
-        launch_gemm(EPI_BF16, hmb, e->p_h17, e->heads17, xin, H, 7 * e->Vs_pad, 7 * e->Vs_pad, nullptr, (uint16_t*)e->logits17, st);
+        launch_gemm_heads(hmb, e->p_h0, e->p_h17, e->head0, e->heads17, xin, H, e->V0_pad, e->V0, 7 * e->Vs_pad, 7 * e->Vs_pad,
+                          (uint16_t*)e->logits0, (uint16_t*)e->logits17, st);
     }
     HIPCHK(hipGetLastError());
     return MTTS_OK;
@@ -986,9 +987,10 @@
 
 static int step_graph(MttsEngine* e, int pages, hipGraphExec_t* out) {
     const int forced = e->has_forced ? 1 : 0, row = attn_row_shape(e, pages) ? 1 : 0, lora = rows_carry_adapters(e) ? 1 : 0;
+    const int noseal = e->skip_seal ? 1 : 0;
     for (auto& g : e->graphs)
         if (g.B == e->B && g.pages == pages && g.forced == forced && g.ch0 == e->ch0_sampled && g.scores == e->scores_on && g.row == row &&
-            g.lora == lora) {
+            g.lora == lora && g.noseal == noseal) {
             *out = g.exec;
             return MTTS_OK;
         }
@@ -1004,7 +1006,7 @@
     hipError_t ie = hipGraphInstantiate(&exec, g, nullptr, nullptr, 0);
     hipGraphDestroy(g);
     HIPCHK(ie);
-    e->graphs.push_back({e->B, pages, forced, e->ch0_sampled, e->scores_on, row, lora, exec});
+    e->graphs.push_back({e->B, pages, forced, e->ch0_sampled, e->scores_on, row, lora, noseal, exec});
     *out = exec;
     return MTTS_OK;
 }
@@ -1013,13 +1015,18 @@
     for (int i = 0; i < n; ++i) {
         if (e->steps_issued >= e->max_steps) break;
         int len_bound = 1;
+        bool completes = false;
         for (int b = 0; b < e->B; ++b) {
             if (!e->slot_live[b]) continue;
             const int len = e->n_real[b] + e->steps_issued + 1;
             len_bound = std::max(len_bound, len);
+            completes |= len % MTTS_PAGE == 0;
             TRY(pool_grow(e, b, (len + MTTS_PAGE - 1) / MTTS_PAGE, st));
         }
         TRY(pool_flush(e, st));
+        e->skip_seal = e->step_noseal && e->kpack && !e->continuous && !completes;
+        if (e->kpack) ++(e->skip_seal ? e->steps_noseal : e->steps_sealing);
+        struct Reset { bool& f; ~Reset() { f = false; } } reset{e->skip_seal};
         const int pages_bound = (len_bound + MTTS_PAGE - 1) / MTTS_PAGE;
         if (e->use_graphs && !e->prof) {
             hipGraphExec_t exec = nullptr;
@@ -1541,8 +1548,8 @@
     } else {
     HIPCHK(hipMemsetAsync(e->xh, 0, (size_t)MTTS_MAXR * e->H * 2, st));
     launch_pack_rows((const uint16_t*)e->hlast + (size_t)slot * e->H, e->xh, 1, e->H, 1, st);
-    launch_gemm(EPI_BF16, 1, e->p_h0, e->head0, e->xh, e->H, e->V0_pad, e->V0, nullptr, (uint16_t*)e->join_logits0, st);
-    launch_gemm(EPI_BF16, 1, e->p_h17, e->heads17, e->xh, e->H, 7 * e->Vs_pad, 7 * e->Vs_pad, nullptr, (uint16_t*)e->join_logits17, st);
+    launch_gemm_heads(1, e->p_h0, e->p_h17, e->head0, e->heads17, e->xh, e->H, e->V0_pad, e->V0, 7 * e->Vs_pad, 7 * e->Vs_pad,
+                      (uint16_t*)e->join_logits0, (uint16_t*)e->join_logits17, st);
     HIPCHK(hipMemcpyAsync((uint16_t*)e->logits0 + (size_t)slot * e->V0_pad, e->join_logits0, (size_t)e->V0 * 2, hipMemcpyDeviceToDevice, st));
     HIPCHK(hipMemcpyAsync((uint16_t*)e->logits17 + (size_t)slot * 7 * e->Vs_pad, e->join_logits17, (size_t)7 * e->Vs_pad * 2, hipMemcpyDeviceToDevice, st));
     }
diff --git a/moss-ttsd_amd/csrc/gemm.hip b/moss-ttsd_amd/csrc/gemm.hip
--- a/moss-ttsd_amd/csrc/gemm.hip
+++ b/moss-ttsd_amd/csrc/gemm.hip
@@ -1,3 +1,5 @@
+#include <stdlib.h>
+
 #include "launch.h"
 
 
@@ -81,6 +83,79 @@
                     int idx = (n0 >> 1) + j;
                     out[xpack_off(row, idx, Npad >> 1)] = f2bf(a * u);
                 }
+            }
+        }
+    }
+}
+
+template <int WAVES, int MB>
+__global__ __launch_bounds__(WAVES * 64) void gemm_heads_kernel(
+    const u32x4_t* __restrict__ Wp0, const u32x4_t* __restrict__ Wp1, const u32x4_t* __restrict__ Xp, int KT, int kt_per_wave,
+    uint16_t* __restrict__ out0, uint16_t* __restrict__ out1, int tiles0, int Npad0, int n_valid0, int Npad1, int n_valid1) {
+    __shared__ float red[WAVES][16][64];
+    const bool h0 = (int)blockIdx.x < tiles0;
+    const int nt = h0 ? blockIdx.x : blockIdx.x - tiles0;
+    const u32x4_t* Wp = h0 ? Wp0 : Wp1;
+    uint16_t* out = h0 ? out0 : out1;
+    const int Npad = h0 ? Npad0 : Npad1, n_valid = h0 ? n_valid0 : n_valid1;
+    const int wave = threadIdx.x >> 6, lane = threadIdx.x & 63;
+    const int kt0 = wave * kt_per_wave, kt1 = min(kt0 + kt_per_wave, KT);
+    f32x16_t acc[MB];
+#pragma unroll
+    for (int mb = 0; mb < MB; ++mb)
+#pragma unroll
+        for (int i = 0; i < 16; ++i) acc[mb][i] = 0.f;
+    const u32x4_t* wp = Wp + ((size_t)nt * KT + kt0) * 64 + lane;
+    const u32x4_t* xp = Xp + (size_t)kt0 * 64 + lane;
+    const size_t xtile = (size_t)KT * 64;
+    constexpr int U = (MB == 1) ? 8 : 4;
+    const int n = kt1 - kt0;
+    int i = 0;
+    for (; i + U <= n; i += U) {
+        u32x4_t a[U], b[U][MB];
+#pragma unroll
+        for (int u = 0; u < U; ++u) a[u] = __builtin_nontemporal_load(wp + (size_t)(i + u) * 64);
+#pragma unroll
+        for (int u = 0; u < U; ++u)
+#pragma unroll
+            for (int mb = 0; mb < MB; ++mb) b[u][mb] = xp[(size_t)(i + u) * 64 + mb * xtile];
+#pragma unroll
+        for (int u = 0; u < U; ++u)
+#pragma unroll
+            for (int mb = 0; mb < MB; ++mb)
+                acc[mb] = __builtin_amdgcn_mfma_f32_32x32x16_bf16(*(bf16x8_t*)&a[u], *(bf16x8_t*)&b[u][mb], acc[mb], 0, 0, 0);
+    }
+    for (; i < n; ++i) {
+        u32x4_t a = __builtin_nontemporal_load(wp + (size_t)i * 64);
+#pragma unroll
+        for (int mb = 0; mb < MB; ++mb) {
+            u32x4_t b = xp[(size_t)i * 64 + mb * xtile];
+            acc[mb] = __builtin_amdgcn_mfma_f32_32x32x16_bf16(*(bf16x8_t*)&a, *(bf16x8_t*)&b, acc[mb], 0, 0, 0);
+        }
+    }
+#pragma unroll
+    for (int mb = 0; mb < MB; ++mb) {
+        if (mb) __syncthreads();
+#pragma unroll
+        for (int r = 0; r < 16; ++r) red[wave][r][lane] = acc[mb][r];
+        __syncthreads();
+        for (int q = wave; q < 4; q += WAVES) {
+            float v[4];
+#pragma unroll
+            for (int j = 0; j < 4; ++j) {
+                float s = red[0][4 * q + j][lane];
+#pragma unroll
+                for (int w = 1; w < WAVES; ++w) s += red[w][4 * q + j][lane];
+                v[j] = s;
+            }
+            const int row = mb * 32 + (lane & 31);
+            const int n0 = nt * 32 + 8 * q + 4 * (lane >> 5);
+            uint16_t* o = out + (size_t)row * Npad + n0;
+            if (n0 + 3 < n_valid) *(u32x2_t*)o = u32x2_t{pack2(v[0], v[1]), pack2(v[2], v[3])};
+            else {
+#pragma unroll
+                for (int j = 0; j < 4; ++j)
+                    if (n0 + j < n_valid) o[j] = f2bf(v[j]);
             }
         }
     }
@@ -581,6 +656,37 @@
     else launch_gemm_mb<EPI_SILU>(mb, p, Wp, Xp, K, Npad, n_valid, partial, out, st);
 }
 
+template <int MB>
+static void launch_heads_mb(const GemmPlan& p, const void* W0, const void* W1, const void* Xp, int K, int Npad0, int n_valid0,
+                            int Npad1, int n_valid1, uint16_t* out0, uint16_t* out1, hipStream_t st) {
+    const dim3 grid((Npad0 + Npad1) / 32);
+#define MTTS_HEADS_CASE(WV)                                                                                              \
+    case WV:                                                                                                             \
+        hipLaunchKernelGGL((gemm_heads_kernel<WV, MB>), grid, dim3(WV * 64), 0, st, (const u32x4_t*)W0, (const u32x4_t*)W1, \
+                           (const u32x4_t*)Xp, K / 16, p.kt_per_wave, out0, out1, Npad0 / 32, Npad0, n_valid0, Npad1, n_valid1); \
+        break;
+    switch (p.waves) {
+        MTTS_HEADS_CASE(8)
+        MTTS_HEADS_CASE(4)
+        MTTS_HEADS_CASE(2)
+        MTTS_HEADS_CASE(1)
+    }
+#undef MTTS_HEADS_CASE
+}
+void launch_gemm_heads(int mb, const GemmPlan& p0, const GemmPlan& p1, const void* W0, const void* W1, const void* Xp, int K,
+                       int Npad0, int n_valid0, int Npad1, int n_valid1, uint16_t* out0, uint16_t* out1, hipStream_t st) {
+    const char* g = getenv("MTTS_HEADS_ONE");
+    const bool same = p0.ksplit == 1 && p1.ksplit == 1 && p0.waves == p1.waves && p0.kt_per_wave == p1.kt_per_wave;
+    if ((g && atoi(g) == 0) || !same) {
+        launch_gemm(EPI_BF16, mb, p0, W0, Xp, K, Npad0, n_valid0, nullptr, out0, st);
+        launch_gemm(EPI_BF16, mb, p1, W1, Xp, K, Npad1, n_valid1, nullptr, out1, st);
+        return;
+    }
+    if (mb <= 1) launch_heads_mb<1>(p0, W0, W1, Xp, K, Npad0, n_valid0, Npad1, n_valid1, out0, out1, st);
+    else if (mb == 2) launch_heads_mb<2>(p0, W0, W1, Xp, K, Npad0, n_valid0, Npad1, n_valid1, out0, out1, st);
+    else launch_heads_mb<4>(p0, W0, W1, Xp, K, Npad0, n_valid0, Npad1, n_valid1, out0, out1, st);
+}
+
 
 int mtts_small_lds_bytes(const GemmPlan& p, int K, int pro) {
     const int kts = pro == PRO_NORM ? K / 16 : p.kt_per_split;
diff --git a/moss-ttsd_amd/csrc/hooks.hip b/moss-ttsd_amd/csrc/hooks.hip
--- a/moss-ttsd_amd/csrc/hooks.hip
+++ b/moss-ttsd_amd/csrc/hooks.hip
@@ -682,6 +682,25 @@
     return MTTS_OK;
 }
 
+int32_t mtts_debug_read_kv_pack(MttsEngine* e, int32_t which, void* host_out, int64_t cap_bytes, int64_t* bytes) {
+    if (!e || !bytes || which < 0 || which > 1) return fail(MTTS_EINVAL, "read_kv_pack: bad argument");
+    if (!e->kpack) return fail(MTTS_ESTATE, "the engine keeps no sealed pages (fp32 / fp16 engine, or MTTS_KV_PACK=0)");
+    const size_t size = e->pk_layer_stride * e->L;
+    *bytes = (int64_t)size;
+    if (!host_out) return MTTS_OK;
+    HIPCHK(hipSetDevice(e->device));
+    HIPCHK(hipDeviceSynchronize());
+    HIPCHK(hipMemcpy(host_out, which ? e->vpack : e->kpack, std::min(size, (size_t)std::max<int64_t>(cap_bytes, 0)), hipMemcpyDeviceToHost));
+    return MTTS_OK;
+}
+
+int32_t mtts_debug_step_counts(MttsEngine* e, int64_t* out2) {
+    if (!e || !out2) return fail(MTTS_EINVAL, "null argument");
+    out2[0] = e->steps_sealing;
+    out2[1] = e->steps_noseal;
+    return MTTS_OK;
+}
+
 int32_t mtts_debug_set_kv_len(MttsEngine* e, int32_t kv_len) {
     if (!e || !e->began) return fail(MTTS_ESTATE, "mtts_begin has not run");
     if (e->f32) return fail(MTTS_EINVAL, "measurement hook of the bf16 engine");
diff --git a/moss-ttsd_amd/csrc/launch.h b/moss-ttsd_amd/csrc/launch.h
--- a/moss-ttsd_amd/csrc/launch.h
+++ b/moss-ttsd_amd/csrc/launch.h
@@ -14,6 +14,8 @@
 GemmPlan mtts_plan_gemm_forced(int Npad, int K, int ksplit, int waves);
 void launch_gemm(int epi, int mb, const GemmPlan& p, const void* Wp, const void* Xp, int K, int Npad, int n_valid,
                  float* partial, uint16_t* out, hipStream_t st);
+void launch_gemm_heads(int mb, const GemmPlan& p0, const GemmPlan& p1, const void* W0, const void* W1, const void* Xp, int K,
+                       int Npad0, int n_valid0, int Npad1, int n_valid1, uint16_t* out0, uint16_t* out1, hipStream_t st);
 int mtts_tile_ksplit(int Npad, int K, int R);
 void launch_gemm_tile(int epi, int R, int ksplit, const void* Wp, const void* Xp, int K, int Npad, int n_valid,
                       float* partial, uint16_t* out, hipStream_t st);
diff --git a/moss-ttsd_amd/csrc/sampler.hip b/moss-ttsd_amd/csrc/sampler.hip
--- a/moss-ttsd_amd/csrc/sampler.hip
+++ b/moss-ttsd_amd/csrc/sampler.hip
@@ -1,3 +1,5 @@
+#include <stdlib.h>
+
 #include "launch.h"
 
 __device__ __forceinline__ void philox4x32_10(uint32_t c0, uint32_t c1, uint32_t c2, uint32_t c3, uint32_t k0,
@@ -111,7 +113,63 @@
     return base + inc - v;
 }
 
-template <bool LP>
+__device__ __forceinline__ float proc_score_bits(uint32_t bits, int i, int mask_id, uint32_t bm_word, float penalty, float temperature) {
+    if (i == mask_id) return -INFINITY;
+    float s = bf2f((uint16_t)bits);
+    if (penalty > 0.f && (bm_word >> (i & 31)) & 1u) s = (s < 0.f) ? s * penalty : s / penalty;
+    if (temperature > 0.f) s = s / temperature;
+    return s;
+}
+
+template <bool VEC, typename F>
+__device__ __forceinline__ void slice_walk(const SampleCtx& x, int i0, int i1, F f) {
+    const int tid = threadIdx.x;
+    if (!VEC || x.lg.f32 || ((uintptr_t)x.lg.p & 15)) {
+        for (int i = i0 + tid; i < i1; i += SAMP_T) f(proc_score(x.lg, i, x.mask_id, x.bm, x.penalty, x.temp), i);
+        return;
+    }
+    const u32x4_t* row = (const u32x4_t*)x.lg.p;
+    const uint16_t* tok = (const uint16_t*)x.lg.p;
+    const int gfull = x.V >> 3, g1 = (i1 + 7) >> 3;
+    for (int g0 = (i0 >> 3) + tid; g0 < g1; g0 += 3 * SAMP_T) {
+        u32x4_t w[3];
+        uint32_t bw[3];
+#pragma unroll
+        for (int u = 0; u < 3; ++u) {
+            const int g = g0 + u * SAMP_T;
+            w[u] = u32x4_t{0u, 0u, 0u, 0u};
+            bw[u] = 0u;
+            if (g >= g1) continue;
+            if (g < gfull) w[u] = row[g];
+            else {
+                uint32_t t[4] = {0u, 0u, 0u, 0u};
+#pragma unroll
+                for (int k = 0; k < 8; ++k)
+                    if (8 * g + k < x.V) t[k >> 1] |= (uint32_t)tok[8 * g + k] << (16 * (k & 1));
+                w[u] = u32x4_t{t[0], t[1], t[2], t[3]};
+            }
+            if (x.penalty > 0.f) bw[u] = x.bm[g >> 2];
+        }
+#pragma unroll
+        for (int u = 0; u < 3; ++u) {
+            const int g = g0 + u * SAMP_T;
+            if (g >= g1) continue;
+            const uint32_t t[4] = {w[u].x, w[u].y, w[u].z, w[u].w};
+#pragma unroll
+            for (int k = 0; k < 8; ++k) {
+                const int i = 8 * g + k;
+                if (i >= i0 && i < i1) f(proc_score_bits(t[k >> 1] >> (16 * (k & 1)), i, x.mask_id, bw[u], x.penalty, x.temp), i);
+            }
+        }
+    }
+}
+
+static bool sampler_vec() {
+    const char* g = getenv("MTTS_SAMPLER_VEC");
+    return !(g && atoi(g) == 0);
+}
+
+template <bool LP, bool VEC>
 __global__ __launch_bounds__(SAMP_T) void sample_scan_kernel(
     const uint16_t* __restrict__ logits0, int V0, const uint32_t* __restrict__ bitmaps, int bm_words,
     const MttsSamplerCfg* __restrict__ cfgs, const LoopState* __restrict__ ls, const SeqState* __restrict__ seqs,
@@ -133,11 +191,10 @@
     const int i0 = slice * per, i1 = min(x.V, i0 + per);
     float bv = -INFINITY;
     int bi = 0x7fffffff;
-    for (int i = i0 + tid; i < i1; i += SAMP_T) {
-        float s = proc_score(x.lg, i, x.mask_id, x.bm, x.penalty, x.temp);
+    slice_walk<VEC>(x, i0, i1, [&](float s, int i) {
         argmax_merge(bv, bi, s, i);
         if (want_hist) atomicAdd(&hist[fkey(s) >> 21], 1u);
-    }
+    });
     block_argmax(bv, bi, shf, shi);
     if (tid == 0) { sc.slice_val[b * SAMP_NS + slice] = bv; sc.slice_idx[b * SAMP_NS + slice] = bi; }
     if (LP && !cfg.do_sample) {
@@ -222,6 +279,7 @@
     return *sh_b0;
 }
 
+template <bool VEC>
 __global__ __launch_bounds__(SAMP_T) void sample_collect_kernel(
     const uint16_t* __restrict__ logits0, int V0, const uint32_t* __restrict__ bitmaps, int bm_words,
     const MttsSamplerCfg* __restrict__ cfgs, const LoopState* __restrict__ ls, const SeqState* __restrict__ seqs,
@@ -256,14 +314,36 @@
     const uint32_t ninf_key = fkey(-INFINITY);
     const int per = (x.V + SAMP_NS - 1) / SAMP_NS;
     const int i0 = slice * per, i1 = min(x.V, i0 + per);
-    for (int i = i0 + tid; i < i1; i += SAMP_T) {
-        float s = proc_score(x.lg, i, x.mask_id, x.bm, x.penalty, x.temp);
-        uint32_t key = fkey(s);
-        if ((int)(key >> 21) >= b0 && key > ninf_key) {
-            uint32_t slot = atomicAdd(&sc.cand_n[b], 1u);
+    auto is_cand = [&](float s) { const uint32_t key = fkey(s); return (int)(key >> 21) >= b0 && key > ninf_key; };
+    if (!VEC) {
+        slice_walk<false>(x, i0, i1, [&](float s, int i) {
+            if (is_cand(s)) {
+                uint32_t slot = atomicAdd(&sc.cand_n[b], 1u);
+                if (slot < SAMP_CAND) { sc.cand_val[(size_t)b * SAMP_CAND + slot] = s; sc.cand_idx[(size_t)b * SAMP_CAND + slot] = i; }
+            }
+        });
+        return;
+    }
+    int cnt = 0;
+    slice_walk<true>(x, i0, i1, [&](float s, int) { cnt += is_cand(s) ? 1 : 0; });
+    int inc = cnt;
+#pragma unroll
+    for (int o = 1; o < 64; o <<= 1) {
+        const int t = __shfl_up(inc, o, 64);
+        if (lane >= o) inc += t;
+    }
+    const int total = __shfl(inc, 63, 64);
+    if (!total) return;
+    uint32_t base = 0u;
+    if (lane == 63) base = atomicAdd(&sc.cand_n[b], (uint32_t)total);
+    uint32_t slot = (uint32_t)__shfl((int)base, 63, 64) + (uint32_t)(inc - cnt);
+    if (!cnt) return;
+    slice_walk<true>(x, i0, i1, [&](float s, int i) {
+        if (is_cand(s)) {
             if (slot < SAMP_CAND) { sc.cand_val[(size_t)b * SAMP_CAND + slot] = s; sc.cand_idx[(size_t)b * SAMP_CAND + slot] = i; }
-        }
-    }
+            ++slot;
+        }
+    });
 }
 
 template <int NT>
@@ -800,11 +880,14 @@
                    const MttsSamplerCfg* cfgs, const LoopState* ls, const SeqState* seqs, uint64_t seed, int32_t* decisions,
                    int32_t* err, int B, const SampleScratch& sc, int ch0_sampled, int full_cap, int emit_lp, hipStream_t st) {
     const int big0 = V0 > SAMP_CAND ? 1 : 0;
+    const bool vec = sampler_vec();
+    const auto scan = emit_lp ? (vec ? sample_scan_kernel<true, true> : sample_scan_kernel<true, false>)
+                              : (vec ? sample_scan_kernel<false, true> : sample_scan_kernel<false, false>);
     if (big0) {
-        hipLaunchKernelGGL(emit_lp ? sample_scan_kernel<true> : sample_scan_kernel<false>, dim3(SAMP_NS, B), dim3(SAMP_T), 0, st,
+        hipLaunchKernelGGL(scan, dim3(SAMP_NS, B), dim3(SAMP_T), 0, st,
                            (const uint16_t*)logits0, V0, bitmaps, bm_words, cfgs, ls, seqs, sc, 0, 0, 0, 0);
         if (ch0_sampled)
-            hipLaunchKernelGGL(sample_collect_kernel, dim3(SAMP_NS, B), dim3(SAMP_T), 0, st, (const uint16_t*)logits0, V0,
+            hipLaunchKernelGGL(vec ? sample_collect_kernel<true> : sample_collect_kernel<false>, dim3(SAMP_NS, B), dim3(SAMP_T), 0, st, (const uint16_t*)logits0, V0,
                                bitmaps, bm_words, cfgs, ls, seqs, sc, full_cap, 0, 0, 0, 0);
     }
     hipLaunchKernelGGL(emit_lp ? sample_final_kernel<true> : sample_final_kernel<false>, dim3(8, B), dim3(SAMP_T), 0, st,
@@ -817,11 +900,14 @@
 void launch_sample_single(const void* logits, int rows, int vocab, const uint32_t* bitmap, int bm_words,
                           const MttsSamplerCfg* cfgs8, int mask_id, uint64_t seed, int step, int channel,
                           int32_t* decisions, int32_t* err, const SampleScratch& sc, int full_cap, int emit_lp, hipStream_t st) {
+    const bool vec = sampler_vec();
+    const auto scan = emit_lp ? (vec ? sample_scan_kernel<true, true> : sample_scan_kernel<true, false>)
+                              : (vec ? sample_scan_kernel<false, true> : sample_scan_kernel<false, false>);
     if (vocab > SAMP_CAND) {
-        hipLaunchKernelGGL(emit_lp ? sample_scan_kernel<true> : sample_scan_kernel<false>, dim3(SAMP_NS, rows), dim3(SAMP_T), 0, st,
+        hipLaunchKernelGGL(scan, dim3(SAMP_NS, rows), dim3(SAMP_T), 0, st,
                            (const uint16_t*)logits, vocab, bitmap, bm_words, cfgs8, (const LoopState*)nullptr,
                            (const SeqState*)nullptr, sc, vocab, mask_id, step, channel);
-        hipLaunchKernelGGL(sample_collect_kernel, dim3(SAMP_NS, rows), dim3(SAMP_T), 0, st, (const uint16_t*)logits, vocab,
+        hipLaunchKernelGGL(vec ? sample_collect_kernel<true> : sample_collect_kernel<false>, dim3(SAMP_NS, rows), dim3(SAMP_T), 0, st, (const uint16_t*)logits, vocab,
                            bitmap, bm_words, cfgs8, (const LoopState*)nullptr, (const SeqState*)nullptr, sc, full_cap, vocab, mask_id, step, channel);
     }
     hipLaunchKernelGGL(emit_lp ? sample_final_kernel<true> : sample_final_kernel<false>, dim3(1, rows), dim3(SAMP_T), 0, st,
diff --git a/moss-ttsd_amd/mtts/capi.py b/moss-ttsd_amd/mtts/capi.py
--- a/moss-ttsd_amd/mtts/capi.py
+++ b/moss-ttsd_amd/mtts/capi.py
@@ -99,6 +99,8 @@
                                       C.POINTER(C.c_int64)]),
     "mtts_debug_set_kv_len": (C.c_int32, [C.c_void_p, C.c_int32]),
     "mtts_debug_kv_pack_stats": (C.c_int32, [C.c_void_p, C.c_void_p]),
+    "mtts_debug_step_counts": (C.c_int32, [C.c_void_p, C.c_void_p]),
+    "mtts_debug_read_kv_pack": (C.c_int32, [C.c_void_p, C.c_int32, C.c_void_p, C.c_int64, C.POINTER(C.c_int64)]),
     "mtts_k_kv_seal": (C.c_int32, [C.c_void_p, C.c_int32, C.c_void_p, C.c_int32, C.c_void_p]),
     "mtts_k_attn_bench": (C.c_int32, [C.c_void_p, C.c_int32, C.c_int32, C.POINTER(C.c_float), C.POINTER(C.c_int64)]),
     "mtts_k_gemm_bench": (C.c_int32, [C.c_int32] * 7 + [C.POINTER(C.c_float)]),
diff --git a/moss-ttsd_amd/mtts/engine.py b/moss-ttsd_amd/mtts/engine.py
--- a/moss-ttsd_amd/mtts/engine.py
+++ b/moss-ttsd_amd/mtts/engine.py
@@ -315,6 +315,18 @@
         capi.check(self.lib.mtts_debug_kv_pack_stats(self._h, o.ctypes.data))
         return dict(zip(("k_pages", "k_unsealed", "v_pages", "v_unsealed", "k_layers_on", "v_layers_on"), (int(x) for x in o)))
 
+    def read_kv_pack(self, which):
+        n = C.c_int64(0)
+        capi.check(self.lib.mtts_debug_read_kv_pack(self._h, int(which), None, 0, C.byref(n)))
+        buf = np.zeros(n.value, dtype=np.uint8)
+        capi.check(self.lib.mtts_debug_read_kv_pack(self._h, int(which), buf.ctypes.data, n.value, C.byref(n)))
+        return buf.reshape(self.cfg["num_hidden_layers"], self.cfg["num_key_value_heads"], -1, 13 * 1024)
+
+    def step_counts(self):
+        o = np.zeros(2, dtype=np.int64)
+        capi.check(self.lib.mtts_debug_step_counts(self._h, o.ctypes.data))
+        return int(o[0]), int(o[1])
+
     def debug_set_kv_len(self, n):
         capi.check(self.lib.mtts_debug_set_kv_len(self._h, int(n)))
 
```
